# mfathulkr/MA-CJD-Cooperative-Jamming-Decision-Making-via-MARL

Measured on AMD Instinct MI355X. Metric: env-steps/sec (all GPUs; batch_envs=4096/GPU, 3j/4r), higher is better.
Workload: dtype f64; 1 GPU; 3 jammers / 4 radars, batch_envs=4096 per GPU, GRU hidden=64; mode=train, hidden=64, train_batch_episodes=32, updates_per_graph=20, hip_graphs=True, gemm_tuning=True, replay_capacity_episodes=8192, mixer_dtype=fp32, mixer=one MFMA launch per direction (f32)

## Files before the change

include/macjd.h:

```cpp
#ifndef MACJD_H
#define MACJD_H

#include <stddef.h>
#include <stdint.h>

#ifdef __cplusplus
extern "C" {
#endif

#define MACJD_ABI_VERSION 8
#define MACJD_PE_ROWS(R, J) (6 * (R) + 3 * (J) + (J) * (R))
#define MACJD_PE_SCAN_ROWS(R, J) (10 * (R) + (J) * (R))

#define MACJD_OK          0
#define MACJD_EINVAL     -1
#define MACJD_ENOMEM     -2
#define MACJD_EDEVICE    -3
#define MACJD_EUNSUPPORTED -4

#define MACJD_MAX_RADARS  32
#define MACJD_MAX_JAMMERS 32
#define MACJD_MAX_PATTERN_LEVELS 6

#define MACJD_JR_WEAK_DENOM 1u

#define MACJD_STEP_ARITH_F64 1u
#define MACJD_STEP_LANE_KERNEL 2u
#define MACJD_STEP_SLOT_KERNEL 4u

typedef struct macjd_scenario_desc {
    int32_t n_radars;
    int32_t n_jammers;
    int32_t episode_limit;
    int32_t reserved;
    double rp_min, rp_max;
    double pd_A, pd_c1, pd_denB;
    const double* radar_GaPs;
    const double* radar_Pn;
    const double* radar_D;
    const double* radar_pd_no;
    const double* radar_snr_no;
    const double* radar_rd_pen;
    const double* radar_gr;
    const double* jam_pmin;
    const double* jam_pmax;
    const double* jam_gj;
    const double* jr_denom;
    const uint8_t* jr_flags;
} macjd_scenario_desc;

typedef struct macjd_scenario macjd_scenario;

typedef struct macjd_step_io {
    int64_t n_envs;
    int64_t env_offset;
    uint64_t seed;
    uint32_t flags;
    uint32_t reserved;

    const int32_t* T;    int64_t T_se, T_sx;
    const float*   P32;
    const double*  P64;  int64_t P_se, P_sx;

    const double* u;     int64_t u_se, u_sx;
    const int32_t* episode;

    uint8_t* track;      int64_t k_se, k_sx;
    int32_t* step;

    float*   reward;
    float*   r_dpj;
    uint8_t* terminated;
    float*   pd;         int64_t pd_se, pd_sx;
    float*   snr_with;   int64_t sw_se, sw_sx;
    double*  out64;
    double*  pd64;
    double*  snr64;
    double*  prj64;
    const double*  pe_tables;
    const uint8_t* pe_flags;
    int64_t        pe_stride;
    int32_t        pe_tile;
    int32_t        reserved_pe;
    float*   r_dpj_sum;
} macjd_step_io;

typedef struct macjd_scan_desc {
    int32_t n_radars, n_jammers;
    const double* half_beam;
    const double* sweep;
    const double* sweep_mod;
    const uint8_t* full;
    const double* az0;
    const double* bear_tgt;
    const double* bear_jam;
    const double* GaPs_side;
    const double* snr_no;
    const double* snr_no_side;
    const double* pd_no_side;
    const double* gr_side;
} macjd_scan_desc;

typedef struct macjd_scan_pattern_desc {
    int32_t n_radars;
    int32_t n_levels;
    const double* inv_width;
    const double* GaPs_lvl;
    const double* snr_no_lvl;
    const double* pd_no_lvl;
    const double* gr_lvl;
} macjd_scan_pattern_desc;

typedef struct macjd_scan_io {
    double* theta_a;  int64_t a_se, a_sx;
    float*  state;    int64_t st_se;
    int32_t st_col0, st_col_step;
    float*  snr_no;   int64_t sn_se, sn_sx;
} macjd_scan_io;

typedef struct macjd_scan_pe_io {
    const double* tables;
    int64_t stride;
} macjd_scan_pe_io;

int         macjd_abi_version(void);
const char* macjd_last_error(void);
void        macjd_reload_options(void);
int         macjd_device_count(void);

int  macjd_scenario_create(const macjd_scenario_desc* host_desc, macjd_scenario** out);
void macjd_scenario_destroy(macjd_scenario* s);
int  macjd_scenario_dims(const macjd_scenario* s, int32_t* n_radars, int32_t* n_jammers,
                         int32_t* episode_limit);
int  macjd_scenario_is_regular(const macjd_scenario* s);

int macjd_env_reset(const macjd_scenario* s, int64_t n_envs, uint8_t* track, int64_t k_se,
                    int64_t k_sx, int32_t* step, const uint8_t* mask, int32_t* episode,
                    void* hip_stream);

int macjd_env_step(const macjd_scenario* s, const macjd_step_io* io, void* hip_stream);

int macjd_scenario_set_scan(macjd_scenario* s, const macjd_scan_desc* d);
int macjd_scenario_set_scan_pattern(macjd_scenario* s, const macjd_scan_pattern_desc* d);
int macjd_env_step_scan(const macjd_scenario* s, const macjd_step_io* io, const macjd_scan_io* scan, void* hip_stream);
int macjd_env_reset_scan(const macjd_scenario* s, int64_t n_envs, const macjd_scan_io* scan, const uint8_t* mask,
                         void* hip_stream);

int macjd_env_step_scan_pe(const macjd_scenario* s, const macjd_step_io* io, const macjd_scan_io* scan,
                           const macjd_scan_pe_io* scan_pe, void* hip_stream);
int macjd_env_reset_scan_pe(const macjd_scenario* s, int64_t n_envs, const macjd_scan_io* scan, const macjd_scan_pe_io* scan_pe,
                            int32_t pe_tile, const uint8_t* mask, void* hip_stream);

int macjd_env_step_many(const macjd_scenario* s, const macjd_step_io* io, int32_t n_steps, int64_t t_stride,
                        void* hip_stream);

int macjd_env_step_timed(const macjd_scenario* s, const macjd_step_io* io, int iters,
                         void* hip_stream, float* ms_per_launch);

int macjd_env_step_many_timed(const macjd_scenario* s, const macjd_step_io* io, int32_t n_steps, int64_t t_stride,
                              int iters, void* hip_stream, float* ms_per_launch);

#ifdef __cplusplus
}
// ... 3 lines not shown
```

include/macjd_nets.h:

```cpp
#ifndef MACJD_NETS_H
#define MACJD_NETS_H

#include <stdint.h>

#include "macjd.h"

#ifdef __cplusplus
extern "C" {
#endif

typedef struct macjd_qhead_io {
    int64_t n_rows;
    int32_t H, A, n_agents, greedy_only;
    const float* base;  int64_t base_ld;
    const float* P_all; int64_t p_ld;
    const float* W1;    int64_t w1_ld;
    const float* w2;
    const float* b2;
    float* Q;           int64_t q_ld;
    const void* avail;  int32_t avail_elem_size, reserved;
    int64_t av_se, av_sj, av_sa;
    float epsilon;      float reserved2;
    uint64_t seed, counter;
    const float* eps_dev;
    const uint64_t* counter_dev;
    int32_t* T_out32;
    int64_t* T_out64;
    int64_t t32_se, t32_sj, t64_se, t64_sj;
    float* P_out;       int64_t po_se, po_sj;
    int64_t* argmax_out;
    const int64_t* gather_idx;
    float* q_gather_out;
} macjd_qhead_io;

int macjd_qhead_select(const macjd_qhead_io* io, void* hip_stream);

typedef struct macjd_gru_io {
    int32_t n_nets, B, T, J, H, reserved;
    const float* gi[2];
    const float* w_hh[2];
    const float* b_hh[2];
    const float* h0[2];
    float* h_out[2];
    int64_t h0_sb[2];
    const float* obs;      int64_t obs_sb, obs_sj;   int32_t S, reserved2;
    const int64_t* obs_index;
    const float* fc1_w[2]; const float* fc1_b[2];
    const float* w_ih[2];  const float* b_ih[2];
    float* p_out[2];
    const float* act_w[2][3]; const float* act_b[2][3];
    int32_t Ah, A;
} macjd_gru_io;

int macjd_gru_sequence(const macjd_gru_io* io, void* hip_stream);

typedef struct macjd_mixer_io {
    int64_t M;
    int32_t J, Em;
    const float* q;
    const float* w1_raw;
    const float* b1_raw;
    const float* wf_raw;
    const float* v_raw;
    float* y;
    const float* gy;
    float* gq;
    float* gw1_raw;
    float* gb1_raw;
    float* gwf_raw;
    float* gv_raw;
    int64_t b1_ld;
} macjd_mixer_io;

int macjd_mixer_tail_forward(const macjd_mixer_io* io, void* hip_stream);
int macjd_mixer_tail_backward(const macjd_mixer_io* io, void* hip_stream);

typedef struct macjd_tdloss_io {
    int32_t B, Tm1;
    float gamma, reserved;
    const float* y;
    const float* tq;
    int64_t y_sb, tq_sb;
    int64_t gy_sb, gy_cols;
    const float* reward;       int64_t r_sb, r_st;
    const uint8_t* terminated; int64_t t_sb, t_st;
    const uint8_t* filled;     int64_t f_sb, f_st;
    float* stats;
    float* gy;
} macjd_tdloss_io;

int macjd_td_loss(const macjd_tdloss_io* io, void* hip_stream);
int macjd_td_mask_sum(const macjd_tdloss_io* io, float* out, void* hip_stream);

typedef struct macjd_adam_io {
    int64_t n;
    float lr, beta1, beta2, eps, max_norm, reserved;
    float* param; float* grad ; float* exp_avg; float* exp_avg_sq;
    float* step; float* grad_norm; float* partials;
} macjd_adam_io;

int macjd_clip_adam_step(const macjd_adam_io* io, void* hip_stream);

typedef struct macjd_sampler_io {
    int64_t* idx_out;
    int32_t n, reserved;
    const int32_t* n_stored;
    int64_t* counter;
    uint64_t seed;
} macjd_sampler_io;

int macjd_sample_episodes(const macjd_sampler_io* io, void* hip_stream);
int macjd_clip_adam_step_sample(const macjd_adam_io* io, const macjd_sampler_io* next, void* hip_stream);

typedef struct macjd_wgrad_io {
    int64_t K;
    int32_t M, N;
    const float* gout; int64_t gout_ld;
    const float* inp;  int64_t inp_ld;
    float* dW;         int64_t dw_ld;
    float* db;
    float* workspace;
    const float* outer_vec;
    const float* outer_w;
} macjd_wgrad_io;

int64_t macjd_linear_wgrad_workspace_floats(int64_t K, int32_t M, int32_t N);
int macjd_linear_wgrad(const macjd_wgrad_io* io, void* hip_stream);
#define MACJD_WGRAD_MAX_BATCH 8
int macjd_linear_wgrad_many(const macjd_wgrad_io* ios, int32_t n, void* hip_stream);

typedef struct macjd_gather_io {
    int32_t n_tensors, n_rows;
    const int64_t* idx;
    const void* src[8]; void* dst[8]; int64_t row_bytes[8];
    int64_t dst_row_bytes[8];
} macjd_gather_io;

int macjd_gather_rows(const macjd_gather_io* io, void* hip_stream);

typedef struct macjd_prefetch_io {
    macjd_gru_io gru;
    macjd_gather_io gather;
    macjd_sampler_io sampler;
    macjd_tdloss_io mask;
    float* tot_m;
    int32_t no_draw, gather_blocks;
} macjd_prefetch_io;

int macjd_prefetch_batch_supported(int32_t n_nets, int32_t H, int32_t B);
int macjd_prefetch_batch(const macjd_prefetch_io* io, void* hip_stream);

typedef struct macjd_qinput_io {
    int64_t n_rows;
    int32_t H, A;
    const float* h;   int64_t h_ld;
    const void* idx;  int32_t idx_elem_size, reserved;
    const float* P;
    float* out;       int64_t out_ld;
} macjd_qinput_io;

int macjd_qhead_input(const macjd_qinput_io* io, void* hip_stream);

typedef struct macjd_qtaken_io {
    int64_t n_rows;
    int32_t H, A;
    const float* h;   int64_t h_ld;
    const void* idx;  int32_t idx_elem_size, reserved;
    const float* P;
    const float* W1;  int64_t w1_ld;
    const float* b1;  const float* w2;  const float* b2;
    float* x;         int64_t x_ld;
    float* act;       int64_t act_ld;
    float* q;
} macjd_qtaken_io;

int macjd_qhead_taken_supported(int32_t H, int32_t A);
int macjd_qhead_taken(const macjd_qtaken_io* io, void* hip_stream);

typedef struct macjd_layernorm_io {
    int64_t M;
    int32_t S, reserved;
    float eps, reserved2;
    const float* x;  int64_t x_ld;
    const float* gamma;
    const float* beta;
    float* y;        int64_t y_ld;
    float* mean;
    float* rstd;
    float* xhat;     int64_t xhat_ld;
} macjd_layernorm_io;

int macjd_layernorm_forward(const macjd_layernorm_io* io, void* hip_stream);

typedef struct macjd_lnparam_io {
    int32_t C, K;
    const float* W;   int64_t w_ld;
    const float* G;   int64_t g_ld;
    const float* gb;
    float* dgamma;
    float* dbeta;
} macjd_lnparam_io;

int macjd_layernorm_param_grad(const macjd_lnparam_io* io, void* hip_stream);
int macjd_clip_adam_step_ln(const macjd_adam_io* io, const macjd_sampler_io* next, const macjd_lnparam_io* ln,
                            int64_t gamma_off, int64_t beta_off, void* hip_stream);

#define MACJD_ACT_NONE 0
#define MACJD_ACT_RELU 1
#define MACJD_ACT_SIGMOID 2
typedef struct macjd_mlp_io {
    int64_t n_rows;
    int32_t n_layers;
    int32_t dims[4];
    int32_t act[3];
    const float* W[3];
    const float* b[3];
    const float* x;  int64_t x_ld;
    float* y;        int64_t y_ld;
} macjd_mlp_io;

int macjd_mlp_forward(const macjd_mlp_io* io, void* hip_stream);
int macjd_mlp_forward_pair(const macjd_mlp_io* io0, const macjd_mlp_io* io1, void* hip_stream);

typedef struct macjd_splitrelu_bwd_io {
    int64_t M;
    int32_t n_blocks, Cp;
    int32_t width[4];
    const float* g[4];  int64_t g_ld[4];
    const float* g_pass; int64_t gp_ld;
    const float* act;   int64_t act_ld;
    float* gout;        int64_t gout_ld;
    const float* outer_w[4];
} macjd_splitrelu_bwd_io;

int macjd_splitrelu_backward(const macjd_splitrelu_bwd_io* io, void* hip_stream);

typedef struct macjd_rowdot_io {
    int64_t n_rows;
    int32_t K, reserved;
    const float* x;  int64_t x_ld;
    const float* w;
    const float* b;
    float* y;
} macjd_rowdot_io;

int macjd_rowdot(const macjd_rowdot_io* io, void* hip_stream);

typedef struct macjd_grugates_io {
    int64_t n_rows;
    int32_t H, reserved;
    const float* gi;  int64_t gi_ld;
    const float* gh;  int64_t gh_ld;
    const float* h;   int64_t h_ld;
    float* h_out;     int64_t ho_ld;
    float* h_out2;    int64_t ho2_ld;
} macjd_grugates_io;

int macjd_gru_gates(const macjd_grugates_io* io, void* hip_stream);

typedef struct macjd_mixerf_io {
    int64_t M;
    int32_t J, S, Hh, Em;
    int32_t save;
    int32_t operand_dtype;
    float ln_eps;  float reserved_f;
    const float* s;   int64_t s_ld;
    const float* q;
    const float* ln_w; const float* ln_b;
    const float* W1; const float* b1;
    const float* W2; const float* b2;
    const float* Wf2; const float* bf2;
    const float* wV2; const float* bV2;
    float* y;
    float* sn; float* xhat;
    float* act;
    const float* gy;
    float* gq;
    float* gout1;
    float* g_w1raw;
    float* g_wfraw;
    float* g_v;
} macjd_mixerf_io;
// ... 139 lines not shown
```

ma-cjd-cooperative-jamming-decision-making-via-marl_amd/_native.py:

```python
from __future__ import annotations

import ctypes
import os
from typing import Optional

_PKG_DIR = os.path.dirname(os.path.abspath(__file__))
LIB_NAME = "libmacjd_hip.so"
LIB_PATH = os.environ.get("MACJD_LIB") or os.path.join(_PKG_DIR, LIB_NAME)

ABI_VERSION = 8
STEP_ARITH_F64 = 1
STEP_LANE_KERNEL = 2
STEP_SLOT_KERNEL = 4

EXPORTS = [
    "macjd_abi_version", "macjd_last_error", "macjd_reload_options", "macjd_device_count",
    "macjd_scenario_create", "macjd_scenario_destroy", "macjd_scenario_dims", "macjd_scenario_is_regular",
    "macjd_env_reset", "macjd_env_step", "macjd_env_step_timed",
    "macjd_qhead_select", "macjd_gru_sequence", "macjd_mixer_tail_forward", "macjd_mixer_tail_backward",
    "macjd_mlp_forward", "macjd_mlp_forward_pair", "macjd_td_loss", "macjd_clip_adam_step", "macjd_clip_adam_step_sample", "macjd_clip_adam_step_ln", "macjd_sample_episodes", "macjd_gather_rows",
    "macjd_linear_wgrad", "macjd_linear_wgrad_workspace_floats", "macjd_linear_wgrad_many", "macjd_qhead_input", "macjd_layernorm_forward", "macjd_layernorm_param_grad", "macjd_gru_gates", "macjd_rowdot", "macjd_splitrelu_backward",
    "macjd_mixer_fused_supported", "macjd_mixer_fused_forward", "macjd_mixer_fused_backward", "macjd_mixer_fused_backward_td", "macjd_td_mask_sum",
    "macjd_agent_episode_supported", "macjd_agent_episode", "macjd_env_step_many", "macjd_env_step_many_timed",
    "macjd_qhead_double_q_supported", "macjd_qhead_double_q", "macjd_qhead_taken_supported", "macjd_qhead_taken",
    "macjd_qheads_pair", "macjd_mixer_fused_forward_pair", "macjd_mixer_fused_train", "macjd_mixer_fused_train_static",
    "macjd_scenario_set_scan", "macjd_env_step_scan", "macjd_env_reset_scan",
    "macjd_env_step_scan_pe", "macjd_env_reset_scan_pe",
    "macjd_agent_env_episode_scan_supported", "macjd_agent_env_episode_scan",
    "macjd_scenario_set_scan_pattern",
    "macjd_gru_sequence_backward_supported", "macjd_gru_sequence_backward",
    "macjd_prefetch_batch_supported", "macjd_prefetch_batch",
    "macjd_actor_gradient_supported", "macjd_actor_gradient",
]


class NativeLibraryError(RuntimeError):
    pass


class StepIO(ctypes.Structure):
    _fields_ = [
        ("n_envs", ctypes.c_int64), ("env_offset", ctypes.c_int64), ("seed", ctypes.c_uint64),
        ("flags", ctypes.c_uint32), ("reserved", ctypes.c_uint32),
        ("T", ctypes.c_void_p), ("T_se", ctypes.c_int64), ("T_sx", ctypes.c_int64),
        ("P32", ctypes.c_void_p), ("P64", ctypes.c_void_p), ("P_se", ctypes.c_int64), ("P_sx", ctypes.c_int64),
        ("u", ctypes.c_void_p), ("u_se", ctypes.c_int64), ("u_sx", ctypes.c_int64),
        ("episode", ctypes.c_void_p),
        ("track", ctypes.c_void_p), ("k_se", ctypes.c_int64), ("k_sx", ctypes.c_int64),
        ("step", ctypes.c_void_p),
        ("reward", ctypes.c_void_p), ("r_dpj", ctypes.c_void_p), ("terminated", ctypes.c_void_p),
        ("pd", ctypes.c_void_p), ("pd_se", ctypes.c_int64), ("pd_sx", ctypes.c_int64),
        ("snr_with", ctypes.c_void_p), ("sw_se", ctypes.c_int64), ("sw_sx", ctypes.c_int64),
        ("out64", ctypes.c_void_p), ("pd64", ctypes.c_void_p), ("snr64", ctypes.c_void_p),
        ("prj64", ctypes.c_void_p),
        ("pe_tables", ctypes.c_void_p), ("pe_flags", ctypes.c_void_p), ("pe_stride", ctypes.c_int64),
        ("pe_tile", ctypes.c_int32), ("reserved_pe", ctypes.c_int32),
        ("r_dpj_sum", ctypes.c_void_p),
    ]


class ScanDesc(ctypes.Structure):
    _fields_ = [
        ("n_radars", ctypes.c_int32), ("n_jammers", ctypes.c_int32),
        ("half_beam", ctypes.c_void_p), ("sweep", ctypes.c_void_p), ("sweep_mod", ctypes.c_void_p),
        ("full", ctypes.c_void_p), ("az0", ctypes.c_void_p), ("bear_tgt", ctypes.c_void_p), ("bear_jam", ctypes.c_void_p),
        ("GaPs_side", ctypes.c_void_p), ("snr_no", ctypes.c_void_p), ("snr_no_side", ctypes.c_void_p),
        ("pd_no_side", ctypes.c_void_p), ("gr_side", ctypes.c_void_p),
    ]


class ScanPatternDesc(ctypes.Structure):
    _fields_ = [
        ("n_radars", ctypes.c_int32), ("n_levels", ctypes.c_int32),
        ("inv_width", ctypes.c_void_p), ("GaPs_lvl", ctypes.c_void_p), ("snr_no_lvl", ctypes.c_void_p),
        ("pd_no_lvl", ctypes.c_void_p), ("gr_lvl", ctypes.c_void_p),
    ]


class ScanIO(ctypes.Structure):
    _fields_ = [
        ("theta_a", ctypes.c_void_p), ("a_se", ctypes.c_int64), ("a_sx", ctypes.c_int64),
        ("state", ctypes.c_void_p), ("st_se", ctypes.c_int64), ("st_col0", ctypes.c_int32), ("st_col_step", ctypes.c_int32),
        ("snr_no", ctypes.c_void_p), ("sn_se", ctypes.c_int64), ("sn_sx", ctypes.c_int64),
    ]


class ScanPeIO(ctypes.Structure):
    _fields_ = [("tables", ctypes.c_void_p), ("stride", ctypes.c_int64)]


class QheadIO(ctypes.Structure):
    _fields_ = [
        ("n_rows", ctypes.c_int64),
        ("H", ctypes.c_int32), ("A", ctypes.c_int32), ("n_agents", ctypes.c_int32), ("greedy_only", ctypes.c_int32),
        ("base", ctypes.c_void_p), ("base_ld", ctypes.c_int64),
        ("P_all", ctypes.c_void_p), ("p_ld", ctypes.c_int64),
        ("W1", ctypes.c_void_p), ("w1_ld", ctypes.c_int64),
        ("w2", ctypes.c_void_p), ("b2", ctypes.c_void_p),
        ("Q", ctypes.c_void_p), ("q_ld", ctypes.c_int64),
        ("avail", ctypes.c_void_p), ("avail_elem_size", ctypes.c_int32), ("reserved", ctypes.c_int32),
        ("av_se", ctypes.c_int64), ("av_sj", ctypes.c_int64), ("av_sa", ctypes.c_int64),
        ("epsilon", ctypes.c_float), ("reserved2", ctypes.c_float),
        ("seed", ctypes.c_uint64), ("counter", ctypes.c_uint64),
        ("eps_dev", ctypes.c_void_p), ("counter_dev", ctypes.c_void_p),
        ("T_out32", ctypes.c_void_p), ("T_out64", ctypes.c_void_p),
        ("t32_se", ctypes.c_int64), ("t32_sj", ctypes.c_int64), ("t64_se", ctypes.c_int64), ("t64_sj", ctypes.c_int64),
        ("P_out", ctypes.c_void_p), ("po_se", ctypes.c_int64), ("po_sj", ctypes.c_int64),
        ("argmax_out", ctypes.c_void_p), ("gather_idx", ctypes.c_void_p), ("q_gather_out", ctypes.c_void_p),
    ]


class GruIO(ctypes.Structure):
    _fields_ = [
        ("n_nets", ctypes.c_int32), ("B", ctypes.c_int32), ("T", ctypes.c_int32), ("J", ctypes.c_int32),
        ("H", ctypes.c_int32), ("reserved", ctypes.c_int32),
        ("gi", ctypes.c_void_p * 2), ("w_hh", ctypes.c_void_p * 2), ("b_hh", ctypes.c_void_p * 2),
        ("h0", ctypes.c_void_p * 2), ("h_out", ctypes.c_void_p * 2), ("h0_sb", ctypes.c_int64 * 2),
        ("obs", ctypes.c_void_p), ("obs_sb", ctypes.c_int64), ("obs_sj", ctypes.c_int64), ("S", ctypes.c_int32), ("reserved2", ctypes.c_int32),
        ("obs_index", ctypes.c_void_p),
        ("fc1_w", ctypes.c_void_p * 2), ("fc1_b", ctypes.c_void_p * 2), ("w_ih", ctypes.c_void_p * 2), ("b_ih", ctypes.c_void_p * 2),
        ("p_out", ctypes.c_void_p * 2), ("act_w", (ctypes.c_void_p * 3) * 2), ("act_b", (ctypes.c_void_p * 3) * 2),
        ("Ah", ctypes.c_int32), ("A", ctypes.c_int32),
    ]


class GruBwdIO(ctypes.Structure):
    _fields_ = [
        ("B", ctypes.c_int32), ("T", ctypes.c_int32), ("J", ctypes.c_int32), ("H", ctypes.c_int32),
        ("gi", ctypes.c_void_p), ("gh", ctypes.c_void_p), ("h_all", ctypes.c_void_p),
        ("h0", ctypes.c_void_p), ("h0_sb", ctypes.c_int64),
        ("w_hh", ctypes.c_void_p), ("dh_all", ctypes.c_void_p),
        ("dgi", ctypes.c_void_p), ("dgh", ctypes.c_void_p), ("dh0", ctypes.c_void_p),
    ]


class ActorGradIO(ctypes.Structure):
    _fields_ = [
        ("n_rows", ctypes.c_int64),
        ("S", ctypes.c_int32), ("Ha", ctypes.c_int32), ("H", ctypes.c_int32), ("A", ctypes.c_int32),
        ("x", ctypes.c_void_p), ("x_ld", ctypes.c_int64), ("base", ctypes.c_void_p), ("base_ld", ctypes.c_int64),
        ("m", ctypes.c_void_p),
        ("W1a", ctypes.c_void_p), ("b1a", ctypes.c_void_p), ("W2a", ctypes.c_void_p), ("b2a", ctypes.c_void_p),
        ("W3a", ctypes.c_void_p), ("b3a", ctypes.c_void_p),
        ("W1q", ctypes.c_void_p), ("w1_ld", ctypes.c_int64), ("w2q", ctypes.c_void_p), ("b2q", ctypes.c_void_p),
        ("a1", ctypes.c_void_p), ("a2", ctypes.c_void_p), ("g3", ctypes.c_void_p), ("g2", ctypes.c_void_p),
        ("g1", ctypes.c_void_p), ("qsum", ctypes.c_void_p),
    ]


class MixerIO(ctypes.Structure):
    _fields_ = [
        ("M", ctypes.c_int64), ("J", ctypes.c_int32), ("Em", ctypes.c_int32),
        ("q", ctypes.c_void_p), ("w1_raw", ctypes.c_void_p), ("b1_raw", ctypes.c_void_p),
        ("wf_raw", ctypes.c_void_p), ("v_raw", ctypes.c_void_p), ("y", ctypes.c_void_p),
        ("gy", ctypes.c_void_p), ("gq", ctypes.c_void_p), ("gw1_raw", ctypes.c_void_p),
        ("gb1_raw", ctypes.c_void_p), ("gwf_raw", ctypes.c_void_p), ("gv_raw", ctypes.c_void_p),
        ("b1_ld", ctypes.c_int64),
    ]


class MixerFusedIO(ctypes.Structure):
    _fields_ = [
        ("M", ctypes.c_int64), ("J", ctypes.c_int32), ("S", ctypes.c_int32), ("Hh", ctypes.c_int32), ("Em", ctypes.c_int32),
        ("save", ctypes.c_int32), ("operand_dtype", ctypes.c_int32), ("ln_eps", ctypes.c_float), ("reserved_f", ctypes.c_float),
        ("s", ctypes.c_void_p), ("s_ld", ctypes.c_int64), ("q", ctypes.c_void_p),
        ("ln_w", ctypes.c_void_p), ("ln_b", ctypes.c_void_p), ("W1", ctypes.c_void_p), ("b1", ctypes.c_void_p),
        ("W2", ctypes.c_void_p), ("b2", ctypes.c_void_p), ("Wf2", ctypes.c_void_p), ("bf2", ctypes.c_void_p),
        ("wV2", ctypes.c_void_p), ("bV2", ctypes.c_void_p),
        ("y", ctypes.c_void_p), ("sn", ctypes.c_void_p), ("xhat", ctypes.c_void_p), ("act", ctypes.c_void_p),
        ("gy", ctypes.c_void_p), ("gq", ctypes.c_void_p), ("gout1", ctypes.c_void_p), ("g_w1raw", ctypes.c_void_p),
        ("g_wfraw", ctypes.c_void_p), ("g_v", ctypes.c_void_p),
    ]


class MixerStaticIO(ctypes.Structure):
    _fields_ = [
        ("n_tiles", ctypes.c_int64), ("sn", ctypes.c_void_p), ("xhat", ctypes.c_void_p), ("act", ctypes.c_void_p),
        ("gout1_sum", ctypes.c_void_p), ("g_w1raw_sum", ctypes.c_void_p), ("g_wfraw_sum", ctypes.c_void_p),
        ("g_v_sum", ctypes.c_void_p),
    ]


class AgentEpisodeIO(ctypes.Structure):
    _fields_ = [
        ("n_envs", ctypes.c_int64), ("T", ctypes.c_int32), ("J", ctypes.c_int32), ("H", ctypes.c_int32), ("A", ctypes.c_int32),
# ... 18 lines not shown
        ("a1_w", ctypes.c_void_p), ("a1_b", ctypes.c_void_p), ("a2_w", ctypes.c_void_p), ("a2_b", ctypes.c_void_p),
        ("a3_w", ctypes.c_void_p), ("a3_b", ctypes.c_void_p),
        ("W1", ctypes.c_void_p), ("w1_ld", ctypes.c_int64), ("b1", ctypes.c_void_p), ("w2", ctypes.c_void_p), ("b2", ctypes.c_void_p),
        ("avail", ctypes.c_void_p), ("avail_elem_size", ctypes.c_int32), ("reserved", ctypes.c_int32),
        ("av_se", ctypes.c_int64), ("av_sj", ctypes.c_int64), ("av_sa", ctypes.c_int64),
        ("eps", ctypes.c_void_p), ("seed", ctypes.c_uint64), ("counter_base", ctypes.c_void_p),
        ("env_seed", ctypes.c_uint64), ("episode", ctypes.c_void_p),
        ("track", ctypes.c_void_p), ("k_se", ctypes.c_int64), ("k_sx", ctypes.c_int64), ("step", ctypes.c_void_p),
        ("scan", ScanIO), ("pe_tables", ctypes.c_void_p),
        ("hidden", ctypes.c_void_p), ("T_out", ctypes.c_void_p), ("P_out", ctypes.c_void_p), ("h_final", ctypes.c_void_p),
        ("st_state", ctypes.c_void_p), ("st_obs", ctypes.c_void_p), ("reward", ctypes.c_void_p), ("terminated", ctypes.c_void_p),
        ("rdpj_sum", ctypes.c_void_p),
    ]


class DoubleQIO(ctypes.Structure):
    _fields_ = [
        ("n_rows", ctypes.c_int64), ("H", ctypes.c_int32), ("A", ctypes.c_int32),
        ("h_e", ctypes.c_void_p), ("he_ld", ctypes.c_int64), ("h_t", ctypes.c_void_p), ("ht_ld", ctypes.c_int64),
        ("P_e", ctypes.c_void_p), ("pe_ld", ctypes.c_int64), ("P_t", ctypes.c_void_p), ("pt_ld", ctypes.c_int64),
        ("W1_e", ctypes.c_void_p), ("w1e_ld", ctypes.c_int64), ("b1_e", ctypes.c_void_p), ("w2_e", ctypes.c_void_p), ("b2_e", ctypes.c_void_p),
        ("W1_t", ctypes.c_void_p), ("w1t_ld", ctypes.c_int64), ("b1_t", ctypes.c_void_p), ("w2_t", ctypes.c_void_p), ("b2_t", ctypes.c_void_p),
        ("out", ctypes.c_void_p), ("argmax_out", ctypes.c_void_p), ("p_group", ctypes.c_int64), ("p_inner", ctypes.c_int64),
    ]


class QinputIO(ctypes.Structure):
    _fields_ = [
        ("n_rows", ctypes.c_int64), ("H", ctypes.c_int32), ("A", ctypes.c_int32),
        ("h", ctypes.c_void_p), ("h_ld", ctypes.c_int64),
        ("idx", ctypes.c_void_p), ("idx_elem_size", ctypes.c_int32), ("reserved", ctypes.c_int32),
        ("P", ctypes.c_void_p), ("out", ctypes.c_void_p), ("out_ld", ctypes.c_int64),
    ]


class GruGatesIO(ctypes.Structure):
    _fields_ = [
        ("n_rows", ctypes.c_int64), ("H", ctypes.c_int32), ("reserved", ctypes.c_int32),
        ("gi", ctypes.c_void_p), ("gi_ld", ctypes.c_int64), ("gh", ctypes.c_void_p), ("gh_ld", ctypes.c_int64),
        ("h", ctypes.c_void_p), ("h_ld", ctypes.c_int64),
        ("h_out", ctypes.c_void_p), ("ho_ld", ctypes.c_int64), ("h_out2", ctypes.c_void_p), ("ho2_ld", ctypes.c_int64),
    ]


class RowdotIO(ctypes.Structure):
    _fields_ = [
        ("n_rows", ctypes.c_int64), ("K", ctypes.c_int32), ("reserved", ctypes.c_int32),
        ("x", ctypes.c_void_p), ("x_ld", ctypes.c_int64), ("w", ctypes.c_void_p), ("b", ctypes.c_void_p),
        ("y", ctypes.c_void_p),
    ]


class SplitReluBwdIO(ctypes.Structure):
    _fields_ = [
        ("M", ctypes.c_int64), ("n_blocks", ctypes.c_int32), ("Cp", ctypes.c_int32), ("width", ctypes.c_int32 * 4),
        ("g0", ctypes.c_void_p), ("g1", ctypes.c_void_p), ("g2", ctypes.c_void_p), ("g3", ctypes.c_void_p),
        ("g_ld", ctypes.c_int64 * 4),
        ("g_pass", ctypes.c_void_p), ("gp_ld", ctypes.c_int64),
        ("act", ctypes.c_void_p), ("act_ld", ctypes.c_int64), ("gout", ctypes.c_void_p), ("gout_ld", ctypes.c_int64),
        ("ow0", ctypes.c_void_p), ("ow1", ctypes.c_void_p), ("ow2", ctypes.c_void_p), ("ow3", ctypes.c_void_p),
    ]


class LayerNormIO(ctypes.Structure):
    _fields_ = [
        ("M", ctypes.c_int64), ("S", ctypes.c_int32), ("reserved", ctypes.c_int32),
        ("eps", ctypes.c_float), ("reserved2", ctypes.c_float),
        ("x", ctypes.c_void_p), ("x_ld", ctypes.c_int64), ("gamma", ctypes.c_void_p), ("beta", ctypes.c_void_p),
        ("y", ctypes.c_void_p), ("y_ld", ctypes.c_int64), ("mean", ctypes.c_void_p), ("rstd", ctypes.c_void_p),
        ("xhat", ctypes.c_void_p), ("xhat_ld", ctypes.c_int64),
    ]


class LnParamIO(ctypes.Structure):
    _fields_ = [
        ("C", ctypes.c_int32), ("K", ctypes.c_int32),
        ("W", ctypes.c_void_p), ("w_ld", ctypes.c_int64), ("G", ctypes.c_void_p), ("g_ld", ctypes.c_int64),
        ("gb", ctypes.c_void_p), ("dgamma", ctypes.c_void_p), ("dbeta", ctypes.c_void_p),
    ]


class MlpIO(ctypes.Structure):
    _fields_ = [
        ("n_rows", ctypes.c_int64), ("n_layers", ctypes.c_int32), ("dims", ctypes.c_int32 * 4),
        ("act", ctypes.c_int32 * 3), ("W", ctypes.c_void_p * 3), ("b", ctypes.c_void_p * 3),
        ("x", ctypes.c_void_p), ("x_ld", ctypes.c_int64), ("y", ctypes.c_void_p), ("y_ld", ctypes.c_int64),
    ]


class TdLossIO(ctypes.Structure):
    _fields_ = [
        ("B", ctypes.c_int32), ("Tm1", ctypes.c_int32), ("gamma", ctypes.c_float), ("reserved", ctypes.c_float),
        ("y", ctypes.c_void_p), ("tq", ctypes.c_void_p),
        ("y_sb", ctypes.c_int64), ("tq_sb", ctypes.c_int64), ("gy_sb", ctypes.c_int64), ("gy_cols", ctypes.c_int64),
        ("reward", ctypes.c_void_p), ("r_sb", ctypes.c_int64), ("r_st", ctypes.c_int64),
        ("terminated", ctypes.c_void_p), ("t_sb", ctypes.c_int64), ("t_st", ctypes.c_int64),
        ("filled", ctypes.c_void_p), ("f_sb", ctypes.c_int64), ("f_st", ctypes.c_int64),
        ("stats", ctypes.c_void_p), ("gy", ctypes.c_void_p),
    ]


class AdamIO(ctypes.Structure):
    _fields_ = [
        ("n", ctypes.c_int64), ("lr", ctypes.c_float), ("beta1", ctypes.c_float), ("beta2", ctypes.c_float),
        ("eps", ctypes.c_float), ("max_norm", ctypes.c_float), ("reserved", ctypes.c_float),
        ("param", ctypes.c_void_p), ("grad", ctypes.c_void_p), ("exp_avg", ctypes.c_void_p),
        ("exp_avg_sq", ctypes.c_void_p), ("step", ctypes.c_void_p), ("grad_norm", ctypes.c_void_p),
        ("partials", ctypes.c_void_p),
    ]


class QtakenIO(ctypes.Structure):
    _fields_ = [
        ("n_rows", ctypes.c_int64), ("H", ctypes.c_int32), ("A", ctypes.c_int32),
        ("h", ctypes.c_void_p), ("h_ld", ctypes.c_int64),
        ("idx", ctypes.c_void_p), ("idx_elem_size", ctypes.c_int32), ("reserved", ctypes.c_int32),
        ("P", ctypes.c_void_p),
        ("W1", ctypes.c_void_p), ("w1_ld", ctypes.c_int64),
        ("b1", ctypes.c_void_p), ("w2", ctypes.c_void_p), ("b2", ctypes.c_void_p),
        ("x", ctypes.c_void_p), ("x_ld", ctypes.c_int64),
        ("act", ctypes.c_void_p), ("act_ld", ctypes.c_int64),
        ("q", ctypes.c_void_p),
    ]


class SamplerIO(ctypes.Structure):
    _fields_ = [
        ("idx_out", ctypes.c_void_p), ("n", ctypes.c_int32), ("reserved", ctypes.c_int32),
        ("n_stored", ctypes.c_void_p), ("counter", ctypes.c_void_p), ("seed", ctypes.c_uint64),
    ]


class GatherIO(ctypes.Structure):
    _fields_ = [
        ("n_tensors", ctypes.c_int32), ("n_rows", ctypes.c_int32), ("idx", ctypes.c_void_p),
        ("src", ctypes.c_void_p * 8), ("dst", ctypes.c_void_p * 8), ("row_bytes", ctypes.c_int64 * 8),
        ("dst_row_bytes", ctypes.c_int64 * 8),
    ]


class PrefetchIO(ctypes.Structure):
    _fields_ = [
        ("gru", GruIO), ("gather", GatherIO), ("sampler", SamplerIO), ("mask", TdLossIO),
        ("tot_m", ctypes.c_void_p), ("no_draw", ctypes.c_int32), ("gather_blocks", ctypes.c_int32),
    ]


class WgradIO(ctypes.Structure):
    _fields_ = [
        ("K", ctypes.c_int64), ("M", ctypes.c_int32), ("N", ctypes.c_int32),
        ("gout", ctypes.c_void_p), ("gout_ld", ctypes.c_int64), ("inp", ctypes.c_void_p), ("inp_ld", ctypes.c_int64),
        ("dW", ctypes.c_void_p), ("dw_ld", ctypes.c_int64), ("db", ctypes.c_void_p), ("workspace", ctypes.c_void_p),
        ("outer_vec", ctypes.c_void_p), ("outer_w", ctypes.c_void_p),
    ]


_lib: Optional[ctypes.CDLL] = None


def load() -> ctypes.CDLL:
    global _lib
    if _lib is not None:
        return _lib
    if not os.path.exists(LIB_PATH):
        raise NativeLibraryError(
            f"{LIB_PATH} not found. Build it with `python -c 'import __graft_entry__ as g; g.build()'` "
            f"(hipcc --offload-arch=gfx950). There is no CPU fallback for the environment step.")
    try:
        lib = ctypes.CDLL(LIB_PATH)
    except OSError as e:
        raise NativeLibraryError(f"cannot load {LIB_PATH}: {e}") from e
    lib.macjd_abi_version.restype = ctypes.c_int
    lib.macjd_last_error.restype = ctypes.c_char_p
    lib.macjd_device_count.restype = ctypes.c_int
    lib.macjd_reload_options.restype = None
    lib.macjd_scenario_create.restype = ctypes.c_int
    lib.macjd_scenario_create.argtypes = [ctypes.c_void_p, ctypes.POINTER(ctypes.c_void_p)]
    lib.macjd_scenario_destroy.restype = None
    lib.macjd_scenario_destroy.argtypes = [ctypes.c_void_p]
    lib.macjd_scenario_is_regular.restype = ctypes.c_int
    lib.macjd_scenario_is_regular.argtypes = [ctypes.c_void_p]
    lib.macjd_scenario_dims.restype = ctypes.c_int
    lib.macjd_scenario_dims.argtypes = [ctypes.c_void_p] + [ctypes.POINTER(ctypes.c_int32)] * 3
    lib.macjd_env_reset.restype = ctypes.c_int
    lib.macjd_env_reset.argtypes = [ctypes.c_void_p, ctypes.c_int64, ctypes.c_void_p, ctypes.c_int64, ctypes.c_int64,
                                    ctypes.c_void_p, ctypes.c_void_p, ctypes.c_void_p, ctypes.c_void_p]
    lib.macjd_env_step.restype = ctypes.c_int
    lib.macjd_scenario_set_scan.restype = ctypes.c_int
    lib.macjd_scenario_set_scan.argtypes = [ctypes.c_void_p, ctypes.POINTER(ScanDesc)]
    lib.macjd_scenario_set_scan_pattern.restype = ctypes.c_int
    lib.macjd_scenario_set_scan_pattern.argtypes = [ctypes.c_void_p, ctypes.POINTER(ScanPatternDesc)]
    lib.macjd_env_step_scan.restype = ctypes.c_int
    lib.macjd_env_step_scan.argtypes = [ctypes.c_void_p, ctypes.POINTER(StepIO), ctypes.POINTER(ScanIO), ctypes.c_void_p]
    lib.macjd_env_reset_scan.restype = ctypes.c_int
    lib.macjd_env_reset_scan.argtypes = [ctypes.c_void_p, ctypes.c_int64, ctypes.POINTER(ScanIO), ctypes.c_void_p, ctypes.c_void_p]
    lib.macjd_env_step_scan_pe.restype = ctypes.c_int
    lib.macjd_env_step_scan_pe.argtypes = [ctypes.c_void_p, ctypes.POINTER(StepIO), ctypes.POINTER(ScanIO),
                                           ctypes.POINTER(ScanPeIO), ctypes.c_void_p]
    lib.macjd_env_reset_scan_pe.restype = ctypes.c_int
    lib.macjd_env_reset_scan_pe.argtypes = [ctypes.c_void_p, ctypes.c_int64, ctypes.POINTER(ScanIO), ctypes.POINTER(ScanPeIO),
                                            ctypes.c_int32, ctypes.c_void_p, ctypes.c_void_p]
    lib.macjd_env_step.argtypes = [ctypes.c_void_p, ctypes.POINTER(StepIO), ctypes.c_void_p]
    lib.macjd_env_step_timed.restype = ctypes.c_int
    lib.macjd_env_step_timed.argtypes = [ctypes.c_void_p, ctypes.POINTER(StepIO), ctypes.c_int, ctypes.c_void_p,
                                         ctypes.POINTER(ctypes.c_float)]
    lib.macjd_qhead_select.restype = ctypes.c_int
    lib.macjd_qhead_select.argtypes = [ctypes.POINTER(QheadIO), ctypes.c_void_p]
    lib.macjd_gru_sequence.restype = ctypes.c_int
    lib.macjd_gru_sequence.argtypes = [ctypes.POINTER(GruIO), ctypes.c_void_p]
    lib.macjd_gru_sequence_backward_supported.restype = ctypes.c_int
    lib.macjd_gru_sequence_backward_supported.argtypes = [ctypes.c_int32]
    lib.macjd_gru_sequence_backward.restype = ctypes.c_int
    lib.macjd_gru_sequence_backward.argtypes = [ctypes.POINTER(GruBwdIO), ctypes.c_void_p]
    lib.macjd_actor_gradient_supported.restype = ctypes.c_int
    lib.macjd_actor_gradient_supported.argtypes = [ctypes.c_int32] * 4
    lib.macjd_actor_gradient.restype = ctypes.c_int
    lib.macjd_actor_gradient.argtypes = [ctypes.POINTER(ActorGradIO), ctypes.c_void_p]
    for name in ("macjd_mixer_tail_forward", "macjd_mixer_tail_backward"):
        getattr(lib, name).restype = ctypes.c_int
        getattr(lib, name).argtypes = [ctypes.POINTER(MixerIO), ctypes.c_void_p]
    lib.macjd_qhead_double_q_supported.restype = ctypes.c_int
    lib.macjd_qhead_double_q_supported.argtypes = [ctypes.c_int32] * 2
    lib.macjd_qhead_double_q.restype = ctypes.c_int
    lib.macjd_qhead_double_q.argtypes = [ctypes.POINTER(DoubleQIO), ctypes.c_void_p]
    lib.macjd_agent_episode_supported.restype = ctypes.c_int
    lib.macjd_agent_episode_supported.argtypes = [ctypes.c_int32] * 3
    lib.macjd_agent_episode.restype = ctypes.c_int
    lib.macjd_agent_episode.argtypes = [ctypes.POINTER(AgentEpisodeIO), ctypes.c_void_p]
    lib.macjd_agent_env_episode_scan_supported.restype = ctypes.c_int
    lib.macjd_agent_env_episode_scan_supported.argtypes = [ctypes.c_int32] * 4
    lib.macjd_agent_env_episode_scan.restype = ctypes.c_int
    lib.macjd_agent_env_episode_scan.argtypes = [ctypes.c_void_p, ctypes.POINTER(AgentEnvEpisodeScanIO), ctypes.c_void_p]
    lib.macjd_env_step_many.restype = ctypes.c_int
    lib.macjd_env_step_many.argtypes = [ctypes.c_void_p, ctypes.POINTER(StepIO), ctypes.c_int32, ctypes.c_int64, ctypes.c_void_p]
    lib.macjd_env_step_many_timed.restype = ctypes.c_int
    lib.macjd_env_step_many_timed.argtypes = [ctypes.c_void_p, ctypes.POINTER(StepIO), ctypes.c_int32, ctypes.c_int64, ctypes.c_int,
                                              ctypes.c_void_p, ctypes.POINTER(ctypes.c_float)]
    lib.macjd_mixer_fused_supported.restype = ctypes.c_int
    lib.macjd_mixer_fused_supported.argtypes = [ctypes.c_int32] * 4
    for name in ("macjd_mixer_fused_forward", "macjd_mixer_fused_backward"):
        getattr(lib, name).restype = ctypes.c_int
        getattr(lib, name).argtypes = [ctypes.POINTER(MixerFusedIO), ctypes.c_void_p]
    lib.macjd_mixer_fused_backward_td.restype = ctypes.c_int
    lib.macjd_mixer_fused_backward_td.argtypes = [ctypes.POINTER(MixerFusedIO), ctypes.POINTER(TdLossIO), ctypes.c_void_p, ctypes.c_void_p]
    lib.macjd_mixer_fused_train.restype = ctypes.c_int
    lib.macjd_mixer_fused_train.argtypes = [ctypes.POINTER(MixerFusedIO), ctypes.POINTER(MixerFusedIO), ctypes.POINTER(TdLossIO),
                                            ctypes.c_void_p, ctypes.c_void_p]
    lib.macjd_mixer_fused_train_static.restype = ctypes.c_int
    lib.macjd_mixer_fused_train_static.argtypes = [ctypes.POINTER(MixerFusedIO), ctypes.POINTER(MixerFusedIO), ctypes.POINTER(TdLossIO),
                                                   ctypes.c_void_p, ctypes.POINTER(MixerStaticIO), ctypes.c_void_p]
    lib.macjd_td_mask_sum.restype = ctypes.c_int
    lib.macjd_td_mask_sum.argtypes = [ctypes.POINTER(TdLossIO), ctypes.c_void_p, ctypes.c_void_p]
    lib.macjd_qhead_taken_supported.restype = ctypes.c_int
    lib.macjd_qhead_taken_supported.argtypes = [ctypes.c_int32, ctypes.c_int32]
    lib.macjd_qhead_taken.restype = ctypes.c_int
    lib.macjd_qhead_taken.argtypes = [ctypes.POINTER(QtakenIO), ctypes.c_void_p]
    lib.macjd_qheads_pair.restype = ctypes.c_int
    lib.macjd_qheads_pair.argtypes = [ctypes.POINTER(QtakenIO), ctypes.POINTER(DoubleQIO), ctypes.c_void_p]
    lib.macjd_mixer_fused_forward_pair.restype = ctypes.c_int
    lib.macjd_mixer_fused_forward_pair.argtypes = [ctypes.POINTER(MixerFusedIO), ctypes.POINTER(MixerFusedIO), ctypes.c_void_p]
    lib.macjd_qhead_input.restype = ctypes.c_int
    lib.macjd_qhead_input.argtypes = [ctypes.POINTER(QinputIO), ctypes.c_void_p]
    lib.macjd_layernorm_forward.restype = ctypes.c_int
    lib.macjd_layernorm_forward.argtypes = [ctypes.POINTER(LayerNormIO), ctypes.c_void_p]
    lib.macjd_gru_gates.restype = ctypes.c_int
    lib.macjd_gru_gates.argtypes = [ctypes.POINTER(GruGatesIO), ctypes.c_void_p]
    lib.macjd_splitrelu_backward.restype = ctypes.c_int
    lib.macjd_splitrelu_backward.argtypes = [ctypes.POINTER(SplitReluBwdIO), ctypes.c_void_p]
    lib.macjd_layernorm_param_grad.restype = ctypes.c_int
    lib.macjd_layernorm_param_grad.argtypes = [ctypes.POINTER(LnParamIO), ctypes.c_void_p]
    lib.macjd_rowdot.restype = ctypes.c_int
    lib.macjd_rowdot.argtypes = [ctypes.POINTER(RowdotIO), ctypes.c_void_p]
    lib.macjd_mlp_forward_pair.restype = ctypes.c_int
    lib.macjd_mlp_forward_pair.argtypes = [ctypes.POINTER(MlpIO), ctypes.POINTER(MlpIO), ctypes.c_void_p]
    lib.macjd_mlp_forward.restype = ctypes.c_int
    lib.macjd_mlp_forward.argtypes = [ctypes.POINTER(MlpIO), ctypes.c_void_p]
    lib.macjd_td_loss.restype = ctypes.c_int
    lib.macjd_td_loss.argtypes = [ctypes.POINTER(TdLossIO), ctypes.c_void_p]
    lib.macjd_clip_adam_step.restype = ctypes.c_int
    lib.macjd_clip_adam_step.argtypes = [ctypes.POINTER(AdamIO), ctypes.c_void_p]
    lib.macjd_clip_adam_step_sample.restype = ctypes.c_int
    lib.macjd_clip_adam_step_sample.argtypes = [ctypes.POINTER(AdamIO), ctypes.POINTER(SamplerIO), ctypes.c_void_p]
    lib.macjd_clip_adam_step_ln.restype = ctypes.c_int
    lib.macjd_clip_adam_step_ln.argtypes = [ctypes.POINTER(AdamIO), ctypes.POINTER(SamplerIO), ctypes.POINTER(LnParamIO),
                                            ctypes.c_int64, ctypes.c_int64, ctypes.c_void_p]
    lib.macjd_sample_episodes.restype = ctypes.c_int
    lib.macjd_sample_episodes.argtypes = [ctypes.POINTER(SamplerIO), ctypes.c_void_p]
    lib.macjd_prefetch_batch_supported.restype = ctypes.c_int
    lib.macjd_prefetch_batch_supported.argtypes = [ctypes.c_int32] * 3
    lib.macjd_prefetch_batch.restype = ctypes.c_int
    lib.macjd_prefetch_batch.argtypes = [ctypes.POINTER(PrefetchIO), ctypes.c_void_p]
    lib.macjd_gather_rows.restype = ctypes.c_int
    lib.macjd_gather_rows.argtypes = [ctypes.POINTER(GatherIO), ctypes.c_void_p]
    lib.macjd_linear_wgrad.restype = ctypes.c_int
    lib.macjd_linear_wgrad.argtypes = [ctypes.POINTER(WgradIO), ctypes.c_void_p]
    lib.macjd_linear_wgrad_many.restype = ctypes.c_int
    lib.macjd_linear_wgrad_many.argtypes = [ctypes.POINTER(WgradIO), ctypes.c_int32, ctypes.c_void_p]
    lib.macjd_linear_wgrad_workspace_floats.restype = ctypes.c_int64
    lib.macjd_linear_wgrad_workspace_floats.argtypes = [ctypes.c_int64, ctypes.c_int32, ctypes.c_int32]
    if lib.macjd_abi_version() != ABI_VERSION:
        raise NativeLibraryError(f"{LIB_NAME}: ABI version {lib.macjd_abi_version()} != expected {ABI_VERSION}")
    _lib = lib
    return lib


def reload_options() -> None:
    load().macjd_reload_options()


def check(rc: int, what: str) -> None:
    if rc != 0:
        msg = load().macjd_last_error()
        raise NativeLibraryError(f"{what} failed ({rc}): {msg.decode() if msg else ''}")


class ScenarioHandle:

    def __init__(self, scenario):
        lib = load()
        desc, keep = scenario.c_desc()
        h = ctypes.c_void_p()
        check(lib.macjd_scenario_create(ctypes.addressof(desc), ctypes.byref(h)), "macjd_scenario_create")
        del keep
        self._h = h
        self._lib = lib
        if getattr(scenario, "scanning", False):
            sdesc, skeep = scenario.c_scan_desc()
            check(lib.macjd_scenario_set_scan(h, ctypes.byref(sdesc)), "macjd_scenario_set_scan")
            del skeep
            if getattr(scenario, "scan_pattern_levels", 0):
                pdesc, pkeep = scenario.c_scan_pattern_desc()
                check(lib.macjd_scenario_set_scan_pattern(h, ctypes.byref(pdesc)), "macjd_scenario_set_scan_pattern")
                del pkeep

    @property
    def ptr(self):
        return self._h

    def close(self):
        if getattr(self, "_h", None):
            self._lib.macjd_scenario_destroy(self._h)
            self._h = None

    def __del__(self):
        try:
            self.close()
        except Exception:
            pass
```

ma-cjd-cooperative-jamming-decision-making-via-marl_amd/core/qmix.py:

```python
from __future__ import annotations

import copy
import os

import numpy as np
import torch
import torch.nn.functional as F
import torch.optim as optim

from .. import hipgraph, ops, options
from .networks import QMixer


def _to(x, dtype, device):
    if isinstance(x, torch.Tensor):
        return x.to(device=device, dtype=dtype)
    return torch.as_tensor(np.asarray(x), device=device).to(dtype)


class QMixLearner:
    def __init__(self, mac, args):
        self.args = args
        self.mac = mac
        self.n_agents = args.n_agents
        self.n_actions = args.n_actions
        self.state_shape = args.state_shape
        self.obs_shape = args.obs_shape
        self.device = torch.device(args.device if torch.cuda.is_available() and args.use_cuda else "cpu")
        self.train_agent_body = bool(getattr(args, "train_agent_body", False))
        self.train_actor = bool(getattr(args, "train_actor", False))
        self.actor_loss_coef = float(getattr(args, "actor_loss_coef", 1.0))
        self._last_actor_q = None

        self.eval_qmix_net = QMixer(args)
        self.target_mac = copy.deepcopy(mac)
        self.target_qmix_net = QMixer(args)
        self.target_qmix_net.load_state_dict(self.eval_qmix_net.state_dict())
        if args.use_cuda:
            self.cuda()
        print(f"QMix Learner Initialized on device: {self.device}")

        self.agent_params = list(self.mac.parameters())
        self.qmix_params = list(self.eval_qmix_net.parameters())
        self.params = self.agent_params + self.qmix_params
        self.optimizer = optim.Adam(params=self.params, lr=args.lr, capturable=(self.device.type == "cuda"))
        self.last_target_update_step = 0
        self.train_step = 0
        self._flat_grad = None
        self._sample_rng = np.random.default_rng(int(getattr(args, "seed", 0) or 0))
        self.grad_pack_launches = 0
        self._flat_param = None
        if self.device.type == "cuda":
            self._flatten_trainable()
        self._body_versions = None
        self._mark_body_shared()

    @staticmethod
    def _body_params(agent):
        return list(agent.fc1.parameters()) + list(agent.rnn.parameters()) + list(agent.actor.parameters())

    def _mark_body_shared(self):
        pe, pt = self._body_params(self.mac.agent), self._body_params(self.target_mac.agent)
        self._body_versions = [(p, p._version, q, q._version) for p, q in zip(pe, pt)]

    def _verify_body_shared(self):
        pe, pt = self._body_params(self.mac.agent), self._body_params(self.target_mac.agent)
        same = len(pe) == len(pt) and all(p.shape == q.shape and torch.equal(p.detach(), q.detach()) for p, q in zip(pe, pt))
        if same:
            self._mark_body_shared()
        else:
            self._body_versions = None
        return same and self._body_is_shared()

    def _body_is_shared(self):
        if self.train_agent_body or self.train_actor:
            return False
        if not options.on("SHARED_BODY") or not self._body_versions:
            return False
        pe = self._body_params(self.mac.agent)
        if len(pe) != len(self._body_versions):
            return False
        return all(p is p0 and p._version == vp and q._version == vq
                   for p, (p0, vp, q, vq) in zip(pe, self._body_versions))

    def _trainable(self):
        first = self.eval_qmix_net.first_layer_params()
        ids = {id(p) for p in first}
        rest = [p for p in list(self.mac.agent.fc2_q_head.parameters()) + self.qmix_params if id(p) not in ids]
        body = list(self.mac.agent.fc1.parameters()) + list(self.mac.agent.rnn.parameters()) if self.train_agent_body else []
        actor = list(self.mac.agent.actor.parameters()) if self.train_actor else []
        return first + rest + body + actor

    @staticmethod
    def _world_size():
        import torch.distributed as dist
        return dist.get_world_size() if (dist.is_available() and dist.is_initialized()) else 1

    def _flatten_trainable(self):
        tr = self._trainable()
        self._flat_offsets, off = [], 0
        for p in tr:
            self._flat_offsets.append(off)
            off += (p.numel() + 3) // 4 * 4
        flat = torch.zeros(off, dtype=tr[0].dtype, device=tr[0].device)
        for p, o in zip(tr, self._flat_offsets):
            flat[o:o + p.numel()].copy_(p.detach().reshape(-1))
        self._flat_param = flat
        self._flat_exp_avg = torch.zeros_like(flat)
        self._flat_exp_avg_sq = torch.zeros_like(flat)
        self._adam_step = torch.zeros((), dtype=torch.float32, device=flat.device)
        self._grad_norm = torch.zeros((), dtype=torch.float32, device=flat.device)
        self._adam_partials = torch.zeros(256 + 1024, dtype=torch.float32, device=flat.device)
        for p, off in zip(tr, self._flat_offsets):
            n = p.numel()
            p.data = flat[off:off + n].view_as(p)
            self.optimizer.state[p] = {"step": self._adam_step, "exp_avg": self._flat_exp_avg[off:off + n].view_as(p),
                                       "exp_avg_sq": self._flat_exp_avg_sq[off:off + n].view_as(p)}
        self._flat_grad = torch.zeros_like(flat)
        self._grad_dst = {}
        for p, off in zip(tr, self._flat_offsets):
            n = p.numel()
            self._grad_dst[ops.grad_key(p)] = self._flat_grad[off:off + n].view_as(p)
        mx = self.eval_qmix_net
        first = mx.first_layer_params()
        rows, S = sum(p.shape[0] for p in first[:4]), first[0].shape[1]
        assert self._flat_offsets[8] == rows * S + rows, "merged first layer must be contiguous in the flat vector"
        mx._merged_views = (flat[:rows * S].view(rows, S), flat[rows * S:rows * S + rows])
        self._grad_dst[ops.grad_key(mx._merged_views[0])] = self._flat_grad[:rows * S].view(rows, S)
        self._grad_dst[ops.grad_key(mx._merged_views[1])] = self._flat_grad[rows * S:rows * S + rows]
        self.target_qmix_net.enable_first_layer_cache()

    def load_optimizer_state(self, state_dict):
        self.optimizer.load_state_dict(state_dict)
        if self._flat_param is None:
            return
        for p, off in zip(self._trainable(), self._flat_offsets):
            n = p.numel()
            st = self.optimizer.state.get(p, {})
            if "exp_avg" in st:
                self._flat_exp_avg[off:off + n].copy_(st["exp_avg"].reshape(-1))
                self._flat_exp_avg_sq[off:off + n].copy_(st["exp_avg_sq"].reshape(-1))
                self._adam_step.copy_(torch.as_tensor(st["step"], dtype=torch.float32).reshape(()))
            self.optimizer.state[p] = {"step": self._adam_step, "exp_avg": self._flat_exp_avg[off:off + n].view_as(p),
                                       "exp_avg_sq": self._flat_exp_avg_sq[off:off + n].view_as(p)}

    def grad_vector(self):
        if self._flat_grad is not None:
            return self._flat_grad
        return torch.cat([p.grad.reshape(-1) for p in self._trainable()])

    def _flatten_grads(self):
        tr = self._trainable()
        if self._flat_grad is None:
            self._flat_grad = torch.empty(sum(p.numel() for p in tr), dtype=tr[0].dtype, device=tr[0].device)
        for p in tr:
            if p.grad is None:
                p.grad = torch.zeros_like(p)
        offs = getattr(self, "_flat_offsets", None)
        padded = offs is not None
        if not padded:
            offs, off = [], 0
            for p in tr:
                offs.append(off)
                off += p.numel()
        base, esz = self._flat_grad.data_ptr(), self._flat_grad.element_size()
        in_place = sum(int(p.grad.data_ptr() == base + off * esz and p.grad.is_contiguous()) for p, off in zip(tr, offs))
        if in_place == len(tr):
            return
        self.grad_pack_launches += 1
        if padded:
            packed = [p.grad.reshape(-1).clone() for p in tr]
            for g_, off in zip(packed, offs):
                self._flat_grad[off:off + g_.numel()].copy_(g_)
        elif in_place == 0:
            torch.cat([p.grad.reshape(-1) for p in tr], out=self._flat_grad)
        else:
            self._flat_grad.copy_(torch.cat([p.grad.reshape(-1) for p in tr]))
        for p, off in zip(tr, offs):
            p.grad = self._flat_grad[off:off + p.numel()].view_as(p)

    def _ar_capturable(self):
        import torch.distributed as dist
        return dist.is_available() and dist.is_initialized() and dist.get_backend() == "nccl"

    def _allreduce_grads(self, force=False):
        import torch.distributed as dist
        if self._world_size() <= 1 and not (force and self._ar_capturable()):
            return
        if dist.get_backend() == "nccl":
            dist.all_reduce(self._flat_grad, op=dist.ReduceOp.AVG)
        else:
            dist.all_reduce(self._flat_grad, op=dist.ReduceOp.SUM)
            self._flat_grad.div_(dist.get_world_size())

    def _forward_backward(self, batch, T, validate_actions=True):
        dev = self.device
        states = _to(batch["state"], torch.float32, dev)[:, :T]
        obs = _to(batch["obs"], torch.float32, dev)[:, :T]
        actions_discrete = _to(batch["actions_discrete"], torch.long, dev)[:, :T]
        actions_continuous = _to(batch["actions_continuous"], torch.float32, dev)[:, :T]
        rewards = _to(batch["reward"], torch.float32, dev)[:, :T]
        terminated = _to(batch["terminated"], torch.bool, dev)[:, :T]
        filled = _to(batch["filled"], torch.bool, dev)[:, :T]
        hidden_states = _to(batch["hidden_state"], torch.float32, dev)[:, :T + 1]
        B = states.shape[0]

        rollout_hidden = self.mac.hidden_states
        h_eval = self._unroll_eval_body(obs) if self.train_agent_body else None
        with torch.no_grad():
            if h_eval is not None:
                target_q_all = self._all_action_q_multi([self.target_mac], obs)[0]
                eval_q_all = self._all_action_q_from_hidden(self.mac, h_eval.detach(), obs)
            else:
                target_q_all, eval_q_all = self._all_action_q_multi([self.target_mac, self.mac], obs)
            self.mac.hidden_states = rollout_hidden
            next_actions = eval_q_all[:, 1:].argmax(dim=3, keepdim=True)
            target_q_taken = torch.gather(target_q_all[:, 1:], 3, next_actions).squeeze(3)
            target_q_mixer = self.target_qmix_net(target_q_taken, states[:, 1:])

        if T <= 1:
            q_taken = torch.empty((B, 0, self.n_agents), device=dev)
        else:
            n_eff = B * (T - 1) * self.n_agents
            h_taken = hidden_states if h_eval is None else h_eval
            q_taken = self.mac.agent.get_q_value_for_action(
                h_taken[:, :T - 1].reshape(n_eff, self.args.rnn_hidden_dim),
                actions_discrete[:, :T - 1].reshape(n_eff, 1),
                actions_continuous[:, :T - 1].reshape(n_eff, 1), validate=validate_actions).view(B, T - 1, self.n_agents)
        eval_q_mixer = self.eval_qmix_net(q_taken, states[:, :-1])

        loss, eval_mean, target_mean = ops.td_loss(eval_q_mixer, target_q_mixer, rewards[:, :-1], terminated[:, :-1],
                                                   filled[:, :-1], self.args.gamma)

        for p in self.params:
            p.grad = None
        if self.train_actor:
            with ops.deferred_wgrad(grad_dst=getattr(self, "_grad_dst", None)):
                loss.backward()
                self._last_actor_q = self._actor_backward(obs, hidden_states if h_eval is None else h_eval.detach(), filled, T)
        else:
            loss.backward()
        if self._world_size() > 1 or self._flat_param is not None:
            self._flatten_grads()
        return loss.detach(), eval_mean.detach(), target_mean.detach()

    def _actor_backward(self, obs, h_taken, filled, T):
        a = self.mac.agent
        params = list(a.actor.parameters())
        B, J, H, A = obs.shape[0], self.n_agents, self.args.rnn_hidden_dim, self.n_actions
        if T <= 1:
            for p in params:
                p.grad = torch.zeros_like(p)
            return torch.zeros((), dtype=torch.float32, device=obs.device)
        n = B * (T - 1) * J
        with torch.no_grad():
            f = filled[:, :T - 1].reshape(B, T - 1).to(torch.float32)
            tot = f.sum()
            w = torch.where(tot > 0, f / (J * tot), torch.zeros_like(f))
            w = w.unsqueeze(2).expand(B, T - 1, J).reshape(n)
            x = obs[:, :T - 1].reshape(n, -1)
            l1, l2 = a.fc2_q_head[0], a.fc2_q_head[2]
            base = F.linear(h_taken[:, :T - 1].reshape(n, H), l1.weight[:, :H], l1.bias)
            a1, a2, g3, g2, g1, qsum = ops.actor_gradient(x, base, self.actor_loss_coef * w, a.actor_layers(), l1.weight,
                                                           l2.weight, l2.bias, H, A)
            for p, g in zip(params, ops.actor_weight_grads(x, a1, a2, g3, g2, g1, params=params)):
                p.grad = g
            return (w * qsum).sum()

    def _unroll_eval_body(self, obs):
        B, T, J, S = obs.shape
        a = self.mac.agent
        H = a.rnn_hidden_dim
# ... 106 lines not shown
            mixer_static = (mixer_train and obs_static and bool(getattr(self, "_g_state_static", False))
                            and options.on("MIXER_STATIC_STATE"))
            self._g_mixer_static = mixer_static
            train_gy = None
            try:
                with torch.no_grad():
                    bases = scan_chain()
                    p_eval = pre_actor[1]
                    params = [p_eval if shared else pre_actor[0], p_eval]
                    for t_ in list(bases) + [p for p in params if p is not None]:
                        t_.record_stream(origin)
                    tq_agents = double_q(bases, params, paired=True)
                q_taken = self.mac.agent.get_q_value_for_action(
                    st["hidden_state"].view(n, H), st["actions_discrete"].view(n, 1), st["actions_continuous"].view(n, 1),
                    validate=False).view(B, T1, J)
                if after_join is not None:
                    fork_at.record(origin)
                with torch.no_grad():
                    if mixer_train:
                        target_q_tot, train_gy = self.target_qmix_net.forward_paired_with_next_fused(
                            tq_agents, st["state"], td=dict(reward=st["reward"], terminated=st["terminated"], filled=st["filled"],
                                                            gamma=self.args.gamma, Tm1=T - 1, tot_m=tot_m,
                                                            static_rows=mixer_static))
                    else:
                        target_q_tot = self.target_qmix_net.forward_paired_with_next_fused(tq_agents, st["state"])
                eval_q_tot = self.eval_qmix_net(q_taken, st["state"])
                ops.assert_pairs_launched()
            finally:
                ops.clear_pending_pairs()
            return self._finish_update(st, T, eval_q_tot, target_q_tot, tot_m=tot_m, side_work=side_work, sums_in_backward=True,
                                       train_gy=train_gy)
        elif target_beside_head:
            origin = torch.cuda.current_stream(dev)
            ts = self._target_stream
            ts.wait_stream(origin)
            with torch.cuda.stream(ts), torch.no_grad():
                bases = scan_chain()
                p_eval = pre_actor[1]
                params = [p_eval if shared else pre_actor[0], p_eval]
                target_q_tot = self.target_qmix_net(double_q(bases, params), st["state"])
                target_done = torch.cuda.Event()
                target_done.record(ts)
            if after_join is not None:
                after_join(False)
            origin.wait_event(prefetched[0])
            eval_q_tot = eval_forward()
            origin.wait_event(target_done)
            target_q_tot.record_stream(origin)
            return self._finish_update(st, T, eval_q_tot, target_q_tot, tot_m=prefetched[2] if len(prefetched) > 2 else None)
        elif two_streams:
            origin = torch.cuda.current_stream(dev)
            if getattr(self, "_target_stream", None) is None:
                self._target_stream = torch.cuda.Stream(device=dev)
            ts = self._target_stream
            if prefetched is None:
                ts.wait_stream(origin)
                with torch.cuda.stream(ts), torch.no_grad():
                    bases = scan_chain()
                    p_target = None if (shared or pre_actor is not None) else actor_all(macs[0].agent)
            else:
                assert pre_scan is not None and pre_actor is not None
                origin.wait_event(prefetched[0])
                bases, p_target = scan_chain(), None
            if pre_actor is not None:
                p_target, p_eval = (None if shared else pre_actor[0]), pre_actor[1]
            eval_q_tot = eval_forward()
            if pre_actor is None:
                with torch.no_grad():
                    p_eval = actor_all(body)
            with torch.no_grad():
                hyper = None if self.target_qmix_net.fused_available(st["state"]) else self.target_qmix_net.hyper_outputs(st["state"])
                if prefetched is None:
                    origin.wait_stream(ts)
                else:
                    origin.wait_event(prefetched[1])
                if after_join is not None:
                    after_join()
                for t_ in list(bases) + ([p_target] if p_target is not None else []) + ([p_eval] if pre_actor is not None else []):
                    t_.record_stream(origin)
                if pre_actor is not None and not fused_dq:
                    ex = lambda p_: p_.view(B, 1, J, A).expand(B, T1, J, A).reshape(n, A)
                    p_target, p_eval = (None if p_target is None else ex(p_target)), ex(p_eval)
                params = [p_eval if shared else p_target, p_eval]
                target_q_tot = self.target_qmix_net(double_q(bases, params), st["state"], hyper=hyper)
        else:
            with torch.no_grad():
                bases = scan_chain()
                p_eval = actor_all(body)
                params = [p_eval if shared else actor_all(macs[0].agent), p_eval]
                hyper = None if self.target_qmix_net.fused_available(st["state"]) else self.target_qmix_net.hyper_outputs(st["state"])
                target_q_tot = self.target_qmix_net(double_q(bases, params), st["state"], hyper=hyper)
            eval_q_tot = eval_forward()
        return self._finish_update(st, T, eval_q_tot, target_q_tot)

    def _paired_heads_ok(self, st, T):
        B, T1 = st["state"].shape[0], T + 1
        J, H, A = self.n_agents, self.args.rnn_hidden_dim, self.n_actions
        n = B * T1 * J
        head = self.mac.agent.fc2_q_head
        return (st["state"].is_cuda and options.get("UPDATE_STREAMS") != "1" and options.on("PAIRED_HEADS")
                and ops.qhead_double_q_fused_supported(st["obs"].reshape(n, -1), H, A)
                and self.target_qmix_net.fused_available(st["state"]) and self.eval_qmix_net.fused_available(st["state"])
                and ops.qhead_taken_supported(st["hidden_state"].view(n, H), head[0].weight, head[2].weight, A))

    def _finish_update(self, st, T, eval_q_tot, target_q_tot, tot_m=None, side_work=None, sums_in_backward=False,
                       train_gy=None):
        for p in self.params:
            p.grad = None
        if eval_q_tot.is_cuda:
            stats_done = stats_branch = sums_late = None
            if train_gy is not None:
                origin = torch.cuda.current_stream(eval_q_tot.device)
                ts = self._target_stream
                head_done = torch.cuda.Event()
                head_done.record(origin)
                row = self._last_stats4 = torch.empty(4, dtype=torch.float32, device=eval_q_tot.device)
                loss, eval_mean, target_mean = row[0], row[1], row[2]
                gy = train_gy

                def sums_late():
                    ts.wait_event(head_done)
                    with torch.cuda.stream(ts):
                        ops.td_loss_sums_into(row, eval_q_tot, target_q_tot, st["reward"], st["terminated"], st["filled"],
                                              self.args.gamma, T - 1, 1)
                    for t_ in (row, eval_q_tot, target_q_tot):
                        t_.record_stream(ts)
            elif tot_m is not None and ops.fused_mixer_backward_will_run(eval_q_tot):
                origin = torch.cuda.current_stream(eval_q_tot.device)
                ts = self._target_stream
                head_done = torch.cuda.Event()
                if not sums_in_backward:
                    head_done.record(origin)

                def stats_branch():
                    with torch.cuda.stream(ts):
                        ts.wait_event(head_done)
                        out = ops.td_loss_and_grad(eval_q_tot, target_q_tot, st["reward"], st["terminated"], st["filled"],
                                                   self.args.gamma, T - 1, 1)
                        done = torch.cuda.Event()
                        done.record(ts)
                    return out, done

                if not sums_in_backward:
                    (loss, eval_mean, target_mean, _, self._last_stats4), stats_done = stats_branch()
                else:
                    row = self._last_stats4 = torch.empty(4, dtype=torch.float32, device=eval_q_tot.device)
                    loss, eval_mean, target_mean = row[0], row[1], row[2]
                gy = ops.td_grad_in_mixer_backward(eval_q_tot, target_q_tot, st["reward"], st["terminated"], st["filled"],
                                                   self.args.gamma, T - 1, 1, tot_m, stats_row=row if sums_in_backward else None)
            else:
                loss, eval_mean, target_mean, gy, self._last_stats4 = ops.td_loss_and_grad(
                    eval_q_tot, target_q_tot, st["reward"], st["terminated"], st["filled"], self.args.gamma, T - 1, 1)
            hold = self._flat_param is not None and self._world_size() <= 1 and options.on("LN_IN_SQNORM")
            with ops.deferred_wgrad(grad_dst=getattr(self, "_grad_dst", None), hold_lnparam=hold) as dw:
                eval_q_tot.backward(gy)
            assert ops._PENDING_TD is None, "the fused mixer's backward did not take the TD loss's inputs"
            self._held_ln = dw.held
            if side_work is not None:
                side_work()
            if sums_late is not None:
                sums_late()
            if stats_done is not None:
                torch.cuda.current_stream(eval_q_tot.device).wait_event(stats_done)
                for t_ in (self._last_stats4,):
                    t_.record_stream(torch.cuda.current_stream(eval_q_tot.device))
        else:
            loss, eval_mean, target_mean = ops.td_loss_full(eval_q_tot, target_q_tot, st["reward"], st["terminated"],
                                                            st["filled"], self.args.gamma, T - 1, 1)
            loss.backward()
        if self._world_size() > 1 or self._flat_param is not None:
            self._flatten_grads()
        return loss.detach(), eval_mean.detach(), target_mean.detach()

    def _clip_and_step(self, sample_next=None):
        if self._flat_param is not None:
            g = self.optimizer.param_groups[0]
            held, self._held_ln = getattr(self, "_held_ln", None), None
            ops.clip_adam_step(self._flat_param, self._flat_grad, self._flat_exp_avg, self._flat_exp_avg_sq,
                               self._adam_step, self._grad_norm, self._adam_partials, g["lr"], g["betas"], g["eps"],
                               self.args.grad_norm_clip, sample_next=sample_next, lnparam=held)
            return self._grad_norm
        grad_norm = torch.nn.utils.clip_grad_norm_(self.params, self.args.grad_norm_clip)
        self.optimizer.step()
        return grad_norm.detach() if torch.is_tensor(grad_norm) else torch.as_tensor(grad_norm)

    def _after_step(self):
        if (self.train_step - self.last_target_update_step) >= self.args.target_update_interval:
            self._update_targets()
            self.last_target_update_step = self.train_step

    def _pack_stats(self, loss, grad_norm, ev, tg, sync_stats, actor_q=None):
        stats = {"loss": loss, "grad_norm": grad_norm, "eval_qtot_avg": ev, "target_qtot_avg": tg}
        if actor_q is not None:
            stats["actor_q_avg"] = actor_q
        if sync_stats:
            stacked = torch.stack([torch.as_tensor(v, device=self.device, dtype=torch.float32).reshape(())
                                   for v in stats.values()])
            stats = dict(zip(stats.keys(), stacked.tolist()))
        return stats

    def train(self, batch, train_info=None, sync_stats=True):
        self.train_step += 1
        loss, ev, tg = self._forward_backward(batch, int(batch["max_seq_len"]))
        self._allreduce_grads()
        grad_norm = self._clip_and_step()
        if self.train_agent_body or self.train_actor:
            for m in (self.mac, self.target_mac):
                m.invalidate_static_inputs()
        self._after_step()
        if not sync_stats and torch.is_tensor(grad_norm) and grad_norm is self._grad_norm_tensor():
            grad_norm = grad_norm.clone()
        return self._pack_stats(loss, grad_norm, ev, tg, sync_stats, actor_q=self._last_actor_q if self.train_actor else None)

    def _grad_norm_tensor(self):
        return getattr(self, "_grad_norm", None)

    def enable_graphs(self, buffer, batch_size, warmup_iters=3, force_two_graphs=False, updates_per_graph=None,
                      graphed_allreduce=None, prime=True):
        if self.device.type != "cuda":
            raise RuntimeError("enable_graphs needs the learner on a HIP device")
        if self.train_agent_body:
            raise RuntimeError("enable_graphs: train_agent_body is an eager-mode option (the captured, static-observation "
                               "and shared-body updates are built on the frozen agent body); use train()")
        if self.train_actor:
            raise RuntimeError("enable_graphs: train_actor is an eager-mode option (the captured, static-observation and "
                               "shared-body updates are built on the frozen actor); use train()")
        self.release_graphs()
        self._verify_body_shared()
        same_buffer = getattr(self, "_g_buffer", None) is buffer
        self._g_buffer, self._g_B, self._g_T = buffer, int(batch_size), int(buffer.episode_limit)
        self._g_obs_static = bool(getattr(buffer, "obs_static", False)) and options.on("LEARNER_STATIC_OBS")
        self._g_state_static = self._g_obs_static and bool(getattr(buffer, "state_static", False))
        self._g_mixer_static = False
        self._g_actor_in_scan = options.on("ACTOR_IN_SCAN")
        self._g_scan_from_ring = self._g_obs_static and int(buffer.buffers["obs"].shape[-1]) <= 3 * int(self.args.rnn_hidden_dim)
        prev_idx = getattr(self, "_g_idx", None)
        keep_idx = same_buffer and prev_idx is not None and prev_idx.numel() == self._g_B and prev_idx.device == self.device
        self._g_idx = prev_idx if keep_idx else torch.zeros(self._g_B, dtype=torch.int64, device=self.device)
        self._g_dev_sampler = self._flat_param is not None and options.on("DEVICE_SAMPLER")
        if not keep_idx:
            self._g_n_stored = torch.zeros(1, dtype=torch.int32, device=self.device)
        if getattr(self, "_g_draws", None) is None:
            self._g_draws = torch.full((1,), int(getattr(self, "_resume_draws", 0)), dtype=torch.int64, device=self.device)
        if not keep_idx:
            self._g_pop_seen = None
            self._g_idx_fresh = False
        self._g_idx_ring = [(torch.zeros(self._g_B, dtype=torch.int64).pin_memory(), torch.cuda.Event()) for _ in range(8)]
        if buffer.current_size < 1:
            raise RuntimeError("enable_graphs: the replay buffer is empty")

        keys = [k for k in buffer.buffers if k != "avail_actions"]
        srcs = [buffer.buffers[k] for k in keys]
        fused = ops.gather_rows_supported(srcs) and self._g_T >= 2
        if fused:
            T1 = self._g_T + 1
            padded = ("actions_discrete", "actions_continuous")
            stage = {k: torch.zeros((self._g_B, T1 if k in padded else v.shape[1]) + tuple(v.shape[2:]), dtype=v.dtype,
                                    device=v.device) for k, v in zip(keys, srcs)}

        def body_a():
            if fused:
                pre = (None, None)
                if self._g_scan_from_ring and options.get("UPDATE_STREAMS") != "1":
                    pre = self._scan_from_ring_early()
                ops.gather_rows(self._g_idx, srcs, [stage[k] for k in keys])
                return self._forward_backward_full(stage, self._g_T, pre_scan=pre[0], pre_actor=pre[1])
            b = {k: v.index_select(0, self._g_idx) for k, v in zip(keys, srcs)}
            return self._forward_backward(b, self._g_T, validate_actions=False)

        self._graph_body_a = body_a

        was_shared = self._body_is_shared()
        snap_p = [p.detach().clone() for p in self.params]
        snap_o = {id(p): {k: v.clone() for k, v in st.items() if torch.is_tensor(v)}
                  for p, st in self.optimizer.state.items()}
        s = torch.cuda.Stream(device=self.device)
        s.wait_stream(torch.cuda.current_stream(self.device))
        with torch.cuda.stream(s):
            for _ in range(max(1, warmup_iters)):
                body_a()
                self._clip_and_step()
        torch.cuda.current_stream(self.device).wait_stream(s)
        def restore_training_state():
            with torch.no_grad():
                for p, sp in zip(self.params, snap_p):
                    p.copy_(sp)
                for p, st in self.optimizer.state.items():
                    for k, v in st.items():
                        if torch.is_tensor(v):
                            old = snap_o.get(id(p), {}).get(k)
                            v.copy_(old) if old is not None else v.zero_()
            if was_shared:
                self._mark_body_shared()

        restore_training_state()
        self._graph_a, self._graph_b = torch.cuda.CUDAGraph(), torch.cuda.CUDAGraph()
        self._g_graphed_ar = bool(graphed_allreduce if graphed_allreduce is not None
                                  else options.get("GRAPHED_ALLREDUCE") == "1") and self._ar_capturable()
        self._g_single = (self._world_size() <= 1 and not force_two_graphs) or self._g_graphed_ar
        with hipgraph.capture(self._graph_a):
            self._g_out_a = body_a()
            st4 = getattr(self, "_last_stats4", None) if fused else None
            if st4 is not None and st4.numel() == 4:
                self._grad_norm = st4[3]
            self._g_stats4 = st4 if (st4 is not None and st4.numel() == 4) else None
            nxt = (self._g_idx, self._g_n_stored, self._g_draws, self._sampler_seed()) if self._g_dev_sampler else None
            if self._g_single:
                if self._g_graphed_ar:
                    self._allreduce_grads(force=True)
                self._g_out_b = self._clip_and_step(sample_next=nxt)
        if not self._g_single:
            with hipgraph.capture(self._graph_b, pool=self._graph_a.pool()):
                self._g_out_b = self._clip_and_step(sample_next=nxt)
        K = int(updates_per_graph if updates_per_graph is not None else options.get("UPDATES_PER_GRAPH"))
        self._g_multi = None
        self._g_prefetch_launch = False
        if K > 1 and self._g_single and self._g_dev_sampler and fused and self._g_stats4 is not None:
            gm, rows, single_norm = torch.cuda.CUDAGraph(), [], self._grad_norm
            pipelined = (self._g_scan_from_ring and self._g_actor_in_scan and options.get("UPDATE_STREAMS") != "1"
                         and options.on("PIPELINED_GROUP"))
            launch_agents = [self.mac.agent] if self._body_is_shared() else [self.target_mac.agent, self.mac.agent]
            self._g_prefetch_launch = bool(pipelined and options.on("PREFETCH_LAUNCH") and "filled" in keys
                                           and ops.prefetch_batch_supported(launch_agents, self._g_B, srcs))
            stage2 = {k: torch.zeros_like(v) for k, v in stage.items()} if pipelined else None
            stages = [stage, stage2]
            self._g_stages = stages
            origin_dev = self.device

            unwritten = [0]

            def prefetch(dst, fork=True, draw=True):
                origin = torch.cuda.current_stream(origin_dev)
                ts = self._target_stream
                if isinstance(fork, torch.cuda.Event):
                    ts.wait_event(fork)
                elif fork:
                    ts.wait_stream(origin)
                shared = self._body_is_shared()
                agents = [self.mac.agent] if shared else [self.target_mac.agent, self.mac.agent]
                if self._g_prefetch_launch:
                    with torch.cuda.stream(ts), torch.no_grad():
                        h, ps, tot_m = ops.prefetch_batch(
                            buffer.buffers["obs"], agents, self._g_B, self.n_agents, self._g_T + 1,
                            (self._g_idx, self._g_n_stored, self._g_draws, self._sampler_seed()), srcs, [dst[k] for k in keys],
                            buffer.buffers["filled"], self._g_T - 1, offset=unwritten[0], draw=draw)
                        unwritten[0] += 1 if draw else 0
                        ev = torch.cuda.Event()
                        ev.record(ts)
                    return [h[0], h[0]], [ps[0], ps[0]], (ev, ev, tot_m)
                with torch.cuda.stream(ts), torch.no_grad():
                    if draw:
                        ops.sample_episodes(self._g_idx, self._g_n_stored, self._g_draws, self._sampler_seed())
                    ops.gather_rows(self._g_idx, srcs, [dst[k] for k in keys])
                    tot_m = ops.td_mask_sum(dst["filled"], self._g_T - 1)
                    ev_g = torch.cuda.Event()
                    ev_g.record(ts)
                    h, ps = ops.gru_sequence_from_obs(buffer.buffers["obs"], self._g_idx, agents, self._g_B, self.n_agents,
                                                      self._g_T + 1, with_actor=True)
                    ev_s = torch.cuda.Event()
                    ev_s.record(ts)
                return (([h[0], h[0]] if shared else h), ([ps[0], ps[0]] if shared else ps), (ev_g, ev_s, tot_m))

            with hipgraph.capture(gm, pool=self._graph_a.pool()):
                nxt_batch = None
                for k_upd in range(K):
                    last = k_upd == K - 1
                    box = {}
                    hook = (lambda fork=True: box.__setitem__("next", prefetch(stages[(k_upd + 1) % 2], fork))) if (pipelined and not last) else None
                    if pipelined and nxt_batch is not None:
                        h_pre, p_pre, evs = nxt_batch
                        self._forward_backward_full(stages[k_upd % 2], self._g_T, pre_scan=h_pre, pre_actor=p_pre,
                                                    prefetched=evs, after_join=hook)
                    elif pipelined:
                        pre = self._scan_from_ring_early()
                        ops.gather_rows(self._g_idx, srcs, [stage[k] for k in keys])
                        if self._paired_heads_ok(stage, self._g_T):
                            tot_m0 = ops.td_mask_sum(stage["filled"], self._g_T - 1)
                            scan_done = torch.cuda.Event()
                            scan_done.record(self._target_stream)
                            self._forward_backward_full(stage, self._g_T, pre_scan=pre[0], pre_actor=pre[1],
                                                        prefetched=(None, scan_done, tot_m0), after_join=hook)
                        else:
                            self._forward_backward_full(stage, self._g_T, pre_scan=pre[0], pre_actor=pre[1], after_join=hook)
                    else:
                        body_a()
                    nxt_batch = box.get("next")
                    rows.append(self._last_stats4)
                    self._grad_norm = rows[-1][3]
                    if self._g_graphed_ar:
                        self._allreduce_grads(force=True)
                    if nxt_batch is not None:
                        self._clip_and_step(sample_next=None)
                    else:
                        self._clip_and_step(sample_next=nxt + (unwritten[0],))
                        unwritten[0] = 0
                if pipelined:
                    torch.cuda.current_stream(self.device).wait_stream(self._target_stream)
            self._grad_norm = single_norm
            self._g_multi = (K, gm, rows)
            self._g_pipelined = pipelined
        self._g_shared_body = self._body_is_shared()
        assert self._g_obs_static == (bool(getattr(buffer, "obs_static", False)) and options.on("LEARNER_STATIC_OBS"))
        if prime:
            keep = (self._g_draws.clone(), self._g_idx.clone(), self._g_n_stored.clone())
            self._g_n_stored.fill_(int(buffer.current_size))
            self._g_idx.clamp_(0, max(0, int(buffer.current_size) - 1))
            hipgraph.replay(self._graph_a, self.device)
            if not self._g_single:
                self._allreduce_grads()
                hipgraph.replay(self._graph_b, self.device)
            if self._g_multi is not None:
                self._g_idx.clamp_(0, max(0, int(buffer.current_size) - 1))
                hipgraph.replay(self._g_multi[1], self.device)
            torch.cuda.synchronize(self.device)
            restore_training_state()
            self._g_draws.copy_(keep[0]); self._g_idx.copy_(keep[1]); self._g_n_stored.copy_(keep[2])
        self._graphs_ready = True

    def release_graphs(self):
        graphs = []
        m = getattr(self, "_g_multi", None)
        if m is not None:
            graphs.append(m[1])
        graphs += [getattr(self, "_graph_b", None), getattr(self, "_graph_a", None)]
        self._graphs_ready = False
        self._g_multi = self._g_stages = None
        self._graph_a = self._graph_b = None
        self._graph_body_a = None
        self._g_out_a = self._g_out_b = self._g_stats4 = self._last_stats4 = self._held_ln = None
        if self._flat_param is not None and any(g is not None for g in graphs):
            self._grad_norm = torch.zeros((), dtype=torch.float32, device=self._flat_param.device)
        hipgraph.destroy(graphs, self.device)

    def train_from_buffer(self, indices=None, sync_stats=True, stats_row=None):
        buf = self._g_buffer if getattr(self, "_graphs_ready", False) else None
        if buf is None:
            raise RuntimeError("call enable_graphs(buffer, batch_size) first")
        device_draw = False
        if indices is None:
            if buf.current_size < self._g_B:
                return self._snap(self.train(buf.sample(self._g_B), None, sync_stats=sync_stats), stats_row)
            device_draw = self._g_dev_sampler and self._population_full_length(buf)
            if not device_draw:
                indices = self._sample_rng.choice(buf.current_size, self._g_B, replace=False)
        if not device_draw:
            indices = np.asarray(indices, dtype=np.int64)
            if len(indices) != self._g_B or int(buf.episode_lengths[indices].min()) != self._g_T:
                return self._snap(self.train(buf.sample(len(indices), indices=indices), None, sync_stats=sync_stats), stats_row)
        if self._g_obs_static and not buf.obs_static:
            raise RuntimeError("an episode with unknown / changing observations was stored after enable_graphs() captured "
                               "the static-observation update: call enable_graphs() again")
        if self._g_shared_body and not self._body_is_shared():
            raise RuntimeError("the agent body (fc1 / GRU / actor) of one controller changed after enable_graphs() captured "
                               "the shared-body update: call enable_graphs() again")
        self.train_step += 1
        if device_draw:
            self._device_draw_ready(buf)
        else:
            k = self.train_step % len(self._g_idx_ring)
            slot, ev = self._g_idx_ring[k]
            ev.synchronize()
            slot.numpy()[:] = indices
            self._g_idx.copy_(slot, non_blocking=True)
            ev.record()
        hipgraph.replay(self._graph_a, self.device)
        self._g_idx_fresh = self._g_dev_sampler and (buf.store_count, buf.current_size) == self._g_pop_seen
        if not self._g_single:
            self._allreduce_grads()
            hipgraph.replay(self._graph_b, self.device)
        self._after_step()
        loss, ev, tg = self._g_out_a
        if stats_row is not None and not sync_stats and self._g_stats4 is not None:
            stats_row.copy_(self._g_stats4, non_blocking=True)
            return {"loss": stats_row[0], "grad_norm": stats_row[3], "eval_qtot_avg": stats_row[1], "target_qtot_avg": stats_row[2]}
        return self._snap(self._pack_stats(loss, self._g_out_b, ev, tg, sync_stats), stats_row)

    def _device_draw_ready(self, buf):
        pop = (buf.store_count, buf.current_size)
        if pop != self._g_pop_seen:
            self._g_n_stored.fill_(buf.current_size)
            self._g_pop_seen, self._g_idx_fresh = pop, False
        if not self._g_idx_fresh:
            ops.sample_episodes(self._g_idx, self._g_n_stored, self._g_draws, self._sampler_seed())

    def train_from_buffer_many(self, n, stats_out=None):
        buf = self._g_buffer if getattr(self, "_graphs_ready", False) else None
        if buf is None:
            raise RuntimeError("call enable_graphs(buffer, batch_size) first")
        out, done = [], 0
        while done < n:
            m = self._g_multi
            until_sync = self.args.target_update_interval - (self.train_step - self.last_target_update_step)
            if (m is not None and n - done >= m[0] and until_sync >= m[0] and buf.current_size >= self._g_B
                    and self._population_full_length(buf) and (not self._g_obs_static or buf.obs_static)
                    and (not self._g_shared_body or self._body_is_shared())):
                self._device_draw_ready(buf)
                self.train_step += m[0]
                hipgraph.replay(m[1], self.device)
                self._g_idx_fresh = (buf.store_count, buf.current_size) == self._g_pop_seen
                self._after_step()
                if stats_out is not None:
                    torch.stack(m[2], out=stats_out[done:done + m[0]])
                out += m[2]
                done += m[0]
            else:
                row = stats_out[done] if stats_out is not None else torch.empty(4, dtype=torch.float32, device=self.device)
                self.train_from_buffer(sync_stats=False, stats_row=row)
                out.append(row)
                done += 1
        return out if stats_out is None else stats_out

    def _sampler_seed(self):
        return getattr(self, "_sampler_seed_value", int(getattr(self.args, "seed", 0) or 0))

    def _population_full_length(self, buf):
        key = (buf.store_count, buf.current_size)
        if getattr(self, "_g_full_key", None) != key:
            self._g_full_key = key
            self._g_full = bool((buf.episode_lengths[:buf.current_size] == self._g_T).all())
        return self._g_full

    @staticmethod
    def _snap(stats, stats_row):
        if stats_row is None or not torch.is_tensor(stats["loss"]):
            return stats
        order = ("loss", "eval_qtot_avg", "target_qtot_avg", "grad_norm")
        torch.stack([torch.as_tensor(stats[k], device=stats_row.device, dtype=torch.float32).reshape(()) for k in order],
                    out=stats_row)
        return {k: stats_row[i] for i, k in enumerate(order)}

    def _all_action_q_multi(self, macs, obs, keep_final_hidden=True):
        B, T, J, S = obs.shape
        rows = obs.reshape(B * T * J, S)
        shared = len(macs) == 2 and self._body_is_shared() and {id(m) for m in macs} == {id(self.mac), id(self.target_mac)}
        body_macs = [self.mac] if shared else list(macs)
        side = None
        if rows.is_cuda:
            if getattr(self, "_side_stream", None) is None:
                self._side_stream = torch.cuda.Stream(device=rows.device)
            side, main = self._side_stream, torch.cuda.current_stream(rows.device)
            side.wait_stream(main)
            with torch.cuda.stream(side):
                params = [m.agent.actor_forward(rows) for m in body_macs]
        else:
            params = [m.agent.actor_forward(rows) for m in body_macs]
        gis = [m.agent.gru_input_transform(rows).view(B, T, J, 3 * m.agent.rnn_hidden_dim) for m in body_macs]
        h_alls = ops.gru_sequence_multi(gis, [m.agent.rnn.weight_hh for m in body_macs],
                                        [m.agent.rnn.bias_hh for m in body_macs])
        if shared:
            params, h_alls = params * 2, h_alls * 2
        bases = []
        for m, h_all in zip(macs, h_alls):
            a = m.agent
            H = a.rnn_hidden_dim
            if keep_final_hidden:
                m.hidden_states = h_all[:, T - 1].reshape(B * J, H) if T > 0 else None
            l1 = a.fc2_q_head[0]
            bases.append(F.linear(h_all.reshape(B * T * J, H), l1.weight[:, :H], l1.bias))
        if side is not None:
            torch.cuda.current_stream(rows.device).wait_stream(side)
            for p in params:
                p.record_stream(torch.cuda.current_stream(rows.device))
        out = []
        for m, base, params_all in zip(macs, bases, params):
            a = m.agent
            l1, l2 = a.fc2_q_head[0], a.fc2_q_head[2]
            out.append(ops.qhead_all_actions(base, params_all, l1.weight, l2.weight, l2.bias, a.rnn_hidden_dim,
                                             a.n_actions).view(B, T, J, a.n_actions))
        return out

    def _all_action_q(self, mac_controller, obs):
        return self._all_action_q_multi([mac_controller], obs)[0]

    def _get_all_action_q_values_and_params(self, mac_controller, batch, max_seq_len):
        obs = _to(batch["obs"], torch.float32, self.device)[:, :max_seq_len]
        with torch.no_grad():
            q = self._all_action_q(mac_controller, obs)
            B, T, J, S = obs.shape
            params = mac_controller.agent.actor(obs.reshape(-1, S)).view(B, T, J, -1)
        return q, params

    def _update_targets(self):
# ... 25 lines not shown
```

ma-cjd-cooperative-jamming-decision-making-via-marl_amd/csrc/macjd_nets.hip:

```cpp
#include <hip/hip_runtime.h>
#include <math.h>
#include <stdint.h>
#include <stdio.h>
#include <stdlib.h>
#include <string.h>
#include <type_traits>

#include "../../include/macjd.h"
#include "../../include/macjd_nets.h"
#include "macjd_err.h"
#include "macjd_tdloss.h"
#include "macjd_philox.h"
#include "macjd_gru_math.h"

namespace macjd {

static int set_nets_err(int code, const char* msg) { return set_err(code, "%s", msg); }

__device__ __forceinline__ bool avail_at(const macjd_qhead_io& io, int64_t e, int j, int a) {
    if (!io.avail) return true;
    const int64_t off = e * io.av_se + (int64_t)j * io.av_sj + (int64_t)a * io.av_sa;
    return (io.avail_elem_size == 8) ? (((const int64_t*)io.avail)[off] != 0)
                                     : (((const int32_t*)io.avail)[off] != 0);
}
// ... 691 lines not shown
    if (err != hipSuccess) return set_nets_err(MACJD_EDEVICE, hipGetErrorString(err));
    return MACJD_OK;
}

extern "C" int macjd_td_loss(const macjd_tdloss_io* io, void* hip_stream) {
    using namespace macjd;
    if (!io || io->B < 1 || io->Tm1 < 1) return set_nets_err(MACJD_EINVAL, "macjd_td_loss: bad B / Tm1");
    if (!io->y || !io->tq || !io->reward || !io->terminated || !io->filled || !io->stats)
        return set_nets_err(MACJD_EINVAL, "macjd_td_loss: NULL pointer");
    if (io->y_sb < io->Tm1 || io->tq_sb < io->Tm1 || (io->gy && (io->gy_cols < io->Tm1 || io->gy_sb < io->gy_cols)))
        return set_nets_err(MACJD_EINVAL, "macjd_td_loss: bad strides");
    hipLaunchKernelGGL(td_loss_kernel, dim3(1), dim3(1024), 0, (hipStream_t)hip_stream, *io);
    hipError_t err = hipGetLastError();
    if (err != hipSuccess) return set_nets_err(MACJD_EDEVICE, hipGetErrorString(err));
    return MACJD_OK;
}

namespace macjd {

constexpr int ADAM_BLOCKS = 256;

__global__ void __launch_bounds__(256) adam_sqnorm_kernel(const macjd_adam_io io) {
    __shared__ float smem[4];
    float s = 0.0f;
    for (int64_t i = (int64_t)blockIdx.x * blockDim.x + threadIdx.x; i < io.n; i += (int64_t)gridDim.x * blockDim.x) {
        const float g = io.grad[i];
        s = fmaf(g, g, s);
    }
    s = wave_sum(s);
    if ((threadIdx.x & 63) == 0) smem[threadIdx.x >> 6] = s;
    __syncthreads();
    if (threadIdx.x == 0) {
        io.partials[blockIdx.x] = (smem[0] + smem[1]) + (smem[2] + smem[3]);
        if (blockIdx.x == 0) io.step[0] += 1.0f;
    }
}

__global__ void __launch_bounds__(256) adam_sqnorm_ln_kernel(const macjd_adam_io io, const macjd_lnparam_io ln, const int64_t g_off,
                                                             const int64_t b_off, const int nb) {
    __shared__ float smem[8];
    if ((int)blockIdx.x < nb) {
        float s = 0.0f;
        for (int64_t i = (int64_t)blockIdx.x * blockDim.x + threadIdx.x; i < io.n; i += (int64_t)nb * blockDim.x) {
            const bool is_ln = (i >= g_off && i < g_off + ln.K) || (i >= b_off && i < b_off + ln.K);
            const float g = is_ln ? 0.0f : io.grad[i];
            s = fmaf(g, g, s);
        }
        s = wave_sum(s);
        if ((threadIdx.x & 63) == 0) smem[threadIdx.x >> 6] = s;
        __syncthreads();
        if (threadIdx.x == 0) {
            io.partials[blockIdx.x] = (smem[0] + smem[1]) + (smem[2] + smem[3]);
            if (blockIdx.x == 0) io.step[0] += 1.0f;
        }
        return;
    }
    const int k = (int)blockIdx.x - nb;
    float sg = 0.0f, sb = 0.0f;
    for (int c = threadIdx.x; c < ln.C; c += blockDim.x) {
        const float w = ln.W[(int64_t)c * ln.w_ld + k];
        sg = fmaf(w, ln.G[(int64_t)c * ln.g_ld + k], sg);
        sb = fmaf(w, ln.gb[c], sb);
    }
    sg = wave_sum(sg);
    sb = wave_sum(sb);
    if ((threadIdx.x & 63) == 0) { smem[threadIdx.x >> 6] = sg; smem[4 + (threadIdx.x >> 6)] = sb; }
    __syncthreads();
    if (threadIdx.x == 0) {
        const float dg = (smem[0] + smem[1]) + (smem[2] + smem[3]), db = (smem[4] + smem[5]) + (smem[6] + smem[7]);
        ln.dgamma[k] = dg;
        ln.dbeta[k] = db;
        io.partials[nb + k] = fmaf(db, db, dg * dg);
    }
}

__device__ __forceinline__ uint32_t fmix32(uint32_t h) {
    h ^= h >> 16; h *= 0x85ebca6bu; h ^= h >> 13; h *= 0xc2b2ae35u; h ^= h >> 16;
    return h;
}
struct SamplerPerm { uint32_t key[8]; int rb; uint32_t rmask, lmask; };
__device__ __forceinline__ SamplerPerm sampler_perm(const int64_t c, const uint64_t seed, const int64_t N) {
    const Philox4 ka = philox4x32_10((uint32_t)c, (uint32_t)((uint64_t)c >> 32), 0x53414d50u, 0u, (uint32_t)seed, (uint32_t)(seed >> 32));
    const Philox4 kb = philox4x32_10((uint32_t)c, (uint32_t)((uint64_t)c >> 32), 0x53414d50u, 1u, (uint32_t)seed, (uint32_t)(seed >> 32));
    SamplerPerm p;
    p.key[0] = ka.v[0]; p.key[1] = ka.v[1]; p.key[2] = ka.v[2]; p.key[3] = ka.v[3];
    p.key[4] = kb.v[0]; p.key[5] = kb.v[1]; p.key[6] = kb.v[2]; p.key[7] = kb.v[3];
    int k = 2;
    while (((int64_t)1 << k) < N) ++k;
    const int lb = k / 2;
    p.rb = k - k / 2;
    p.rmask = (1u << p.rb) - 1u; p.lmask = (1u << lb) - 1u;
    return p;
}
__device__ __forceinline__ int64_t sampler_index(const SamplerPerm& p, const int64_t N, const int n, const int t) {
    if (N < n) return t % N;
    uint32_t x = (uint32_t)t;
    for (int walk = 0; walk < 64; ++walk) {
        uint32_t L = x >> p.rb, R = x & p.rmask;
#pragma unroll
        for (int r = 0; r < 8; r += 2) {
            L = (L ^ fmix32(R ^ p.key[r])) & p.lmask;
            R = (R ^ fmix32(L ^ p.key[r + 1])) & p.rmask;
        }
        x = (L << p.rb) | R;
        if ((int64_t)x < N) break;
    }
    return ((int64_t)x < N) ? (int64_t)x : (int64_t)(x % (uint32_t)N);
}
__device__ __forceinline__ void sample_episodes_block(const macjd_sampler_io& sp) {
    const int64_t c = *sp.counter + (int64_t)sp.reserved;
    const int64_t N = (int64_t)*sp.n_stored;
    __syncthreads();
    if (threadIdx.x == 0) *sp.counter = c + 1;
    if (N < 1) return;
    const SamplerPerm perm = sampler_perm(c, sp.seed, N);
    for (int t = threadIdx.x; t < sp.n; t += blockDim.x) sp.idx_out[t] = sampler_index(perm, N, sp.n, t);
}

__global__ void __launch_bounds__(256) sample_episodes_kernel(const macjd_sampler_io sp) { sample_episodes_block(sp); }

template <bool SAMPLE>
__global__ void __launch_bounds__(256) adam_update_kernel(const macjd_adam_io io, const int n_partials, const macjd_sampler_io next) {
    __shared__ float s_tot;
    if (threadIdx.x < 64) {
        float s = 0.0f;
        for (int i = threadIdx.x; i < n_partials; i += 64) s += io.partials[i];
        s = wave_sum(s);
        if (threadIdx.x == 0) s_tot = s;
    }
    __syncthreads();
    const float total_norm = sqrtf(s_tot);
    float coef = io.max_norm / (total_norm + 1e-6f);
    coef = coef < 1.0f ? coef : 1.0f;
    const float step = io.step[0];
    const float bc1 = 1.0f - powf(io.beta1, step);
    const float bc2 = 1.0f - powf(io.beta2, step);
    const float step_size = io.lr / bc1;
    const float bc2_sqrt = sqrtf(bc2);
    for (int64_t i = (int64_t)blockIdx.x * blockDim.x + threadIdx.x; i < io.n; i += (int64_t)gridDim.x * blockDim.x) {
        const float g = io.grad[i] * coef;
        io.grad[i] = g;
        float m = io.exp_avg[i], v = io.exp_avg_sq[i];
        m = m + (1.0f - io.beta1) * (g - m);
        v = v * io.beta2 + (1.0f - io.beta2) * g * g;
        io.exp_avg[i] = m;
        io.exp_avg_sq[i] = v;
        const float denom = sqrtf(v) / bc2_sqrt + io.eps;
        io.param[i] -= step_size * (m / denom);
    }
    if (blockIdx.x == 0 && threadIdx.x == 0) io.grad_norm[0] = total_norm;
    if (SAMPLE && blockIdx.x == 0) sample_episodes_block(next);
}

__device__ __forceinline__ void gather_rows_body(const macjd_gather_io& io, const int k, const int row, const int64_t src_row,
                                                 const int part, const int parts) {
    const int64_t words = io.row_bytes[k] >> 2;
    const uint32_t* __restrict__ src = (const uint32_t*)((const char*)io.src[k] + src_row * io.row_bytes[k]);
    const int64_t dpitch = io.dst_row_bytes[k] ? io.dst_row_bytes[k] : io.row_bytes[k];
    uint32_t* __restrict__ dst = (uint32_t*)((char*)io.dst[k] + (int64_t)row * dpitch);
    const bool vec = ((io.row_bytes[k] & 15) == 0) && ((dpitch & 15) == 0) && ((((uintptr_t)io.src[k]) & 15) == 0) &&
                     ((((uintptr_t)io.dst[k]) & 15) == 0);
    if (vec) {
        const int64_t n4 = words >> 2;
        for (int64_t i = (int64_t)part * blockDim.x + threadIdx.x; i < n4; i += (int64_t)parts * blockDim.x)
            ((uint4*)dst)[i] = ((const uint4*)src)[i];
    } else {
        for (int64_t i = (int64_t)part * blockDim.x + threadIdx.x; i < words; i += (int64_t)parts * blockDim.x)
            dst[i] = src[i];
    }
}

__global__ void __launch_bounds__(256) gather_rows_kernel(const macjd_gather_io io) {
    gather_rows_body(io, blockIdx.y, blockIdx.z, io.idx[blockIdx.z], blockIdx.x, gridDim.x);
}

constexpr int PREFETCH_MAX_B = 1024;
constexpr int PREFETCH_ROW_PARTS = 8;

__global__ void __launch_bounds__(256) prefetch_batch_kernel(const macjd_prefetch_io io) {
    __shared__ __attribute__((aligned(16))) float s_h[2][64];
    __shared__ float s_gi[3 * 64];
    __shared__ float s_pro[768];
    __shared__ int64_t s_idx[PREFETCH_MAX_B];
    __shared__ float s_w[16];
    const int B = io.gru.B, BJ = B * io.gru.J, G = io.gather_blocks;
    const int wg = blockIdx.x;
    const int64_t N = (int64_t)*io.sampler.n_stored;
    const bool draw = !io.no_draw && N >= 1;
    SamplerPerm perm = {};
    if (draw) perm = sampler_perm(*io.sampler.counter + (int64_t)io.sampler.reserved, io.sampler.seed, N);
    auto index_of = [&](int t) -> int64_t { return draw ? sampler_index(perm, N, io.sampler.n, t) : io.sampler.idx_out[t]; };
    if (wg < 2 * BJ) {
        const bool actor_only = wg >= BJ;
        const int seq = actor_only ? wg - BJ : wg;
        gru_units_body<true>(io.gru, 0, seq, index_of(seq / io.gru.J), actor_only, false, s_h, s_gi, s_pro);
    } else if (wg < 2 * BJ + G) {
        const int n_parts = PREFETCH_ROW_PARTS * io.gather.n_tensors * B;
        for (int v = wg - 2 * BJ; v < n_parts; v += G) {
            const int part = v % PREFETCH_ROW_PARTS, kr = v / PREFETCH_ROW_PARTS;
            const int k = kr % io.gather.n_tensors, row = kr / io.gather.n_tensors;
            gather_rows_body(io.gather, k, row, index_of(row), part, PREFETCH_ROW_PARTS);
        }
    } else {
        for (int t = threadIdx.x; t < B; t += blockDim.x) {
            const int64_t e = index_of(t);
            s_idx[t] = e;
            if (draw) io.sampler.idx_out[t] = e;
        }
        __syncthreads();
        td_mask_sum_body(io.mask, io.tot_m, s_w, [&](int b) { return s_idx[b]; });
    }
}

}

static int sampler_args_ok(const macjd_sampler_io* sp) {
    return sp && sp->idx_out && sp->n >= 1 && sp->n_stored && sp->counter && sp->reserved >= 0;
}

extern "C" int macjd_sample_episodes(const macjd_sampler_io* io, void* hip_stream) {
    using namespace macjd;
    if (!sampler_args_ok(io)) return set_nets_err(MACJD_EINVAL, "macjd_sample_episodes: bad argument");
    hipLaunchKernelGGL(sample_episodes_kernel, dim3(1), dim3(256), 0, (hipStream_t)hip_stream, *io);
    hipError_t err = hipGetLastError();
    if (err != hipSuccess) return set_nets_err(MACJD_EDEVICE, hipGetErrorString(err));
    return MACJD_OK;
}

extern "C" int macjd_clip_adam_step_sample(const macjd_adam_io* io, const macjd_sampler_io* next, void* hip_stream) {
    using namespace macjd;
    if (!io || io->n < 1 || !io->param || !io->grad || !io->exp_avg || !io->exp_avg_sq || !io->step || !io->grad_norm ||
        !io->partials)
        return set_nets_err(MACJD_EINVAL, "macjd_clip_adam_step: bad argument");
    if (next && !sampler_args_ok(next)) return set_nets_err(MACJD_EINVAL, "macjd_clip_adam_step_sample: bad sampler argument");
    hipStream_t s = (hipStream_t)hip_stream;
    int blocks = (int)((io->n + 255) / 256);
    if (blocks > ADAM_BLOCKS) blocks = ADAM_BLOCKS;
    hipLaunchKernelGGL(adam_sqnorm_kernel, dim3(blocks), dim3(256), 0, s, *io);
    if (next) hipLaunchKernelGGL(adam_update_kernel<true>, dim3(blocks), dim3(256), 0, s, *io, blocks, *next);
    else hipLaunchKernelGGL(adam_update_kernel<false>, dim3(blocks), dim3(256), 0, s, *io, blocks, macjd_sampler_io{});
    hipError_t err = hipGetLastError();
    if (err != hipSuccess) return set_nets_err(MACJD_EDEVICE, hipGetErrorString(err));
    return MACJD_OK;
}

extern "C" int macjd_clip_adam_step(const macjd_adam_io* io, void* hip_stream) {
    return macjd_clip_adam_step_sample(io, nullptr, hip_stream);
}

extern "C" int macjd_clip_adam_step_ln(const macjd_adam_io* io, const macjd_sampler_io* next, const macjd_lnparam_io* ln,
                                       int64_t gamma_off, int64_t beta_off, void* hip_stream) {
    using namespace macjd;
    if (!io || io->n < 1 || !io->param || !io->grad || !io->exp_avg || !io->exp_avg_sq || !io->step || !io->grad_norm ||
        !io->partials)
        return set_nets_err(MACJD_EINVAL, "macjd_clip_adam_step_ln: bad argument");
    if (next && !sampler_args_ok(next)) return set_nets_err(MACJD_EINVAL, "macjd_clip_adam_step_ln: bad sampler argument");
    if (!ln || ln->C < 1 || ln->K < 1 || ln->K > 1024 || !ln->W || !ln->G || !ln->gb || ln->w_ld < ln->K || ln->g_ld < ln->K)
        return set_nets_err(MACJD_EINVAL, "macjd_clip_adam_step_ln: bad LayerNorm argument");
    if (gamma_off < 0 || beta_off < 0 || gamma_off + ln->K > io->n || beta_off + ln->K > io->n ||
        ln->dgamma != io->grad + gamma_off || ln->dbeta != io->grad + beta_off)
        return set_nets_err(MACJD_EINVAL, "macjd_clip_adam_step_ln: dgamma / dbeta must be the named ranges of the gradient vector");
    hipStream_t s = (hipStream_t)hip_stream;
    int blocks = (int)((io->n + 255) / 256);
    if (blocks > ADAM_BLOCKS) blocks = ADAM_BLOCKS;
    hipLaunchKernelGGL(adam_sqnorm_ln_kernel, dim3(blocks + ln->K), dim3(256), 0, s, *io, *ln, gamma_off, beta_off, blocks);
    if (next) hipLaunchKernelGGL(adam_update_kernel<true>, dim3(blocks), dim3(256), 0, s, *io, blocks + ln->K, *next);
    else hipLaunchKernelGGL(adam_update_kernel<false>, dim3(blocks), dim3(256), 0, s, *io, blocks + ln->K, macjd_sampler_io{});
    hipError_t err = hipGetLastError();
    if (err != hipSuccess) return set_nets_err(MACJD_EDEVICE, hipGetErrorString(err));
    return MACJD_OK;
}

static int gather_tensors_ok(const macjd_gather_io* io) {
    if (io->n_tensors < 1 || io->n_tensors > 8) return 0;
    for (int k = 0; k < io->n_tensors; ++k)
        if (!io->src[k] || !io->dst[k] || io->row_bytes[k] < 4 || (io->row_bytes[k] & 3) || (io->dst_row_bytes[k] & 3) ||
            (io->dst_row_bytes[k] && io->dst_row_bytes[k] < io->row_bytes[k]))
            return 0;
    return 1;
}

extern "C" int macjd_gather_rows(const macjd_gather_io* io, void* hip_stream) {
    using namespace macjd;
    if (!io || io->n_tensors < 1 || io->n_tensors > 8 || io->n_rows < 0 || !io->idx)
        return set_nets_err(MACJD_EINVAL, "macjd_gather_rows: bad argument");
    if (!gather_tensors_ok(io))
        return set_nets_err(MACJD_EINVAL, "macjd_gather_rows: bad tensor (row bytes must be a positive multiple of 4)");
    if (io->n_rows == 0) return MACJD_OK;
    hipLaunchKernelGGL(gather_rows_kernel, dim3(8, io->n_tensors, io->n_rows), dim3(256), 0, (hipStream_t)hip_stream, *io);
    hipError_t err = hipGetLastError();
    if (err != hipSuccess) return set_nets_err(MACJD_EDEVICE, hipGetErrorString(err));
    return MACJD_OK;
}

extern "C" int macjd_prefetch_batch_supported(int32_t n_nets, int32_t H, int32_t B) {
    return n_nets == 1 && H == 64 && B >= 1 && B <= macjd::PREFETCH_MAX_B && !macjd::env_options().gru_ksplit;
}

extern "C" int macjd_prefetch_batch(const macjd_prefetch_io* io, void* hip_stream) {
    using namespace macjd;
    if (!io) return set_nets_err(MACJD_EINVAL, "macjd_prefetch_batch: NULL io");
    const macjd_gru_io& g = io->gru;
    if (!macjd_prefetch_batch_supported(g.n_nets, g.H, g.B))
        return set_nets_err(MACJD_EUNSUPPORTED, "macjd_prefetch_batch: needs one network, H = 64, 1 <= B <= 1024, the unit-split scan");
    if (g.T < 1 || g.J < 1 || !g.obs || g.S < 1 || g.S > 256 || !g.w_hh[0] || !g.b_hh[0] || !g.h_out[0] || !g.fc1_w[0] ||
        !g.fc1_b[0] || !g.w_ih[0] || !g.b_ih[0])
        return set_nets_err(MACJD_EINVAL, "macjd_prefetch_batch: bad scan argument");
    if (!g.p_out[0] || g.Ah < 1 || g.Ah > 256 || g.A < 1 || g.A > 64)
        return set_nets_err(MACJD_EINVAL, "macjd_prefetch_batch: needs the in-kernel actor (Ah <= 256, A <= 64)");
    for (int l = 0; l < 3; ++l)
        if (!g.act_w[0][l] || !g.act_b[0][l]) return set_nets_err(MACJD_EINVAL, "macjd_prefetch_batch: needs the actor's three layers");
    if (!sampler_args_ok(&io->sampler) || io->sampler.n != g.B)
        return set_nets_err(MACJD_EINVAL, "macjd_prefetch_batch: bad sampler argument (n must be the batch size)");
    if (io->gather.n_rows != g.B || !gather_tensors_ok(&io->gather))
        return set_nets_err(MACJD_EINVAL, "macjd_prefetch_batch: bad gather argument (n_rows must be the batch size, row bytes "
                                          "positive multiples of 4)");
    if (io->mask.B != g.B || io->mask.Tm1 < 1 || !io->mask.filled || !io->tot_m)
        return set_nets_err(MACJD_EINVAL, "macjd_prefetch_batch: bad mask-sum argument");
    if (io->gather_blocks < 0) return set_nets_err(MACJD_EINVAL, "macjd_prefetch_batch: bad gather_blocks");
    macjd_prefetch_io a = *io;
    const int n_parts = PREFETCH_ROW_PARTS * a.gather.n_tensors * g.B;
    if (a.gather_blocks == 0) a.gather_blocks = 256;
    if (a.gather_blocks > n_parts) a.gather_blocks = n_parts;
    const unsigned grid = 2u * (unsigned)(g.B * g.J) + (unsigned)a.gather_blocks + 1u;
    hipLaunchKernelGGL(prefetch_batch_kernel, dim3(grid), dim3(256), 0, (hipStream_t)hip_stream, a);
    hipError_t err = hipGetLastError();
    if (err != hipSuccess) return set_nets_err(MACJD_EDEVICE, hipGetErrorString(err));
    return MACJD_OK;
}

namespace macjd {

__global__ void __launch_bounds__(256) qhead_input_kernel(const macjd_qinput_io io) {
    const int W = io.H + io.A + 1;
    const int64_t total = io.n_rows * W;
    for (int64_t i = (int64_t)blockIdx.x * blockDim.x + threadIdx.x; i < total; i += (int64_t)gridDim.x * blockDim.x) {
        const int64_t n = i / W;
        const int c = (int)(i - n * W);
        float v;
        if (c < io.H) {
            v = io.h[n * io.h_ld + c];
        } else if (c < io.H + io.A) {
            const int64_t a = (io.idx_elem_size == 8) ? ((const int64_t*)io.idx)[n] : (int64_t)((const int32_t*)io.idx)[n];
            v = (a == (int64_t)(c - io.H)) ? 1.0f : 0.0f;
        } else {
            v = io.P[n];
        }
        io.out[n * io.out_ld + c] = v;
    }
}

__global__ void __launch_bounds__(256) layernorm_forward_kernel(const macjd_layernorm_io io) {
    const int lane = threadIdx.x & 63;
    const int64_t wave = (int64_t)blockIdx.x * (blockDim.x >> 6) + (threadIdx.x >> 6);
    const int64_t n_waves = (int64_t)gridDim.x * (blockDim.x >> 6);
    const int S = io.S;
    const float inv_s = 1.0f / (float)S;
    for (int64_t m = wave; m < io.M; m += n_waves) {
        const float* __restrict__ x = io.x + m * io.x_ld;
        float v[16];
        float sum = 0.0f;
#pragma unroll
        for (int i = 0; i < 16; ++i) {
            const int c = lane + 64 * i;
            v[i] = (c < S) ? x[c] : 0.0f;
            sum += v[i];
        }
#pragma unroll
        for (int o = 32; o > 0; o >>= 1) sum += __shfl_xor(sum, o);
        const float mean = sum * inv_s;
        float sq = 0.0f;
#pragma unroll
        for (int i = 0; i < 16; ++i) {
            const int c = lane + 64 * i;
            const float d = (c < S) ? v[i] - mean : 0.0f;
            sq = fmaf(d, d, sq);
        }
#pragma unroll
        for (int o = 32; o > 0; o >>= 1) sq += __shfl_xor(sq, o);
        const float rstd = rsqrtf(sq * inv_s + io.eps);
        float* __restrict__ y = io.y + m * io.y_ld;
#pragma unroll
        for (int i = 0; i < 16; ++i) {
            const int c = lane + 64 * i;
            if (c < S) {
                const float g = io.gamma ? io.gamma[c] : 1.0f, b = io.beta ? io.beta[c] : 0.0f;
                y[c] = (v[i] - mean) * rstd * g + b;
                if (io.xhat) io.xhat[m * io.xhat_ld + c] = (v[i] - mean) * rstd;
            }
        }
        if (lane == 0) {
            if (io.mean) io.mean[m] = mean;
            if (io.rstd) io.rstd[m] = rstd;
// ... 244 lines not shown
```

ma-cjd-cooperative-jamming-decision-making-via-marl_amd/csrc/macjd_wgrad.hip:

```cpp
#include <hip/hip_runtime.h>
#include <stdint.h>

#include "../../include/macjd.h"
#include "../../include/macjd_nets.h"
#include "macjd_err.h"

namespace macjd {

typedef float f32x4 __attribute__((ext_vector_type(4)));
#ifndef MACJD_WG_KC
#define MACJD_WG_KC 64
#endif
#ifndef MACJD_WG_ABLATE
#define MACJD_WG_ABLATE 0
#endif
#ifndef MACJD_WG_SUB
#define MACJD_WG_SUB 1
#endif
constexpr int WG_BM = 64, WG_BN = 64, WG_KC = MACJD_WG_KC, WG_PITCH = 80, WG_SUB = MACJD_WG_SUB;
constexpr int WG_ROWS = WG_KC * WG_SUB;

__host__ __device__ inline int64_t wg_pad(int64_t v, int64_t m) { return (v + m - 1) / m * m; }

struct WgradProb {
    int64_t K, gout_ld, inp_ld;
    int M, N, Mp, Np, n_chunks;
    const float* gout;
    const float* inp;
    float* workspace;
    bool want_db;
    const float* outer_vec;
    const float* outer_w;
};

__device__ __forceinline__ void wgrad_partial_body(const WgradProb& io, const int tn, const int tm, const int chunk,
                                                   float* __restrict__ sA, float* __restrict__ sB) {
    const int Mp = io.Mp, Np = io.Np;
    const int m0 = tm * WG_BM, n0 = tn * WG_BN;
    const int64_t k0 = (int64_t)chunk * WG_ROWS;
    const int tid = threadIdx.x;
    constexpr int NIT = (WG_KC * 16) / 256;
    float4 va[NIT], vb[NIT];
    auto load_operand = [&](const float* __restrict__ base, const int64_t ld, const int cols, const int c0, const int piece,
                            float4* __restrict__ out) {
        const bool al16 = ((ld & 3) == 0) && ((((uintptr_t)base) & 15) == 0) && (c0 + 64 <= cols);
        const bool al8 = ((ld & 1) == 0) && ((cols & 1) == 0) && ((((uintptr_t)base) & 7) == 0) && cols >= 2;
        const int c4 = (tid & 15) * 4;
        int64_t roff[NIT];
        bool rok[NIT];
#pragma unroll
        for (int it = 0; it < NIT; ++it) {
            const int64_t k = k0 + (int64_t)piece * WG_KC + ((it * 256 + tid) >> 4);
            rok[it] = k < io.K && !(MACJD_WG_ABLATE & 2);
            roff[it] = (k < io.K ? k : io.K - 1) * ld;
        }
        if (al16) {
#pragma unroll
            for (int it = 0; it < NIT; ++it) out[it] = *reinterpret_cast<const float4*>(base + roff[it] + c0 + c4);
        } else if (al8) {
            const int ca = c0 + c4 < cols ? c0 + c4 : cols - 2, cb = c0 + c4 + 2 < cols ? c0 + c4 + 2 : cols - 2;
#pragma unroll
            for (int it = 0; it < NIT; ++it) {
                const float2 lo = *reinterpret_cast<const float2*>(base + roff[it] + ca);
                const float2 hi = *reinterpret_cast<const float2*>(base + roff[it] + cb);
                out[it] = float4{lo.x, lo.y, hi.x, hi.y};
            }
        } else {
            int cc[4];
#pragma unroll
            for (int e = 0; e < 4; ++e) cc[e] = c0 + c4 + e < cols ? c0 + c4 + e : cols - 1;
#pragma unroll
            for (int it = 0; it < NIT; ++it)
                out[it] = float4{base[roff[it] + cc[0]], base[roff[it] + cc[1]], base[roff[it] + cc[2]], base[roff[it] + cc[3]]};
        }
#pragma unroll
        for (int it = 0; it < NIT; ++it) {
            out[it].x = (rok[it] && c0 + c4 + 0 < cols) ? out[it].x : 0.0f;
            out[it].y = (rok[it] && c0 + c4 + 1 < cols) ? out[it].y : 0.0f;
            out[it].z = (rok[it] && c0 + c4 + 2 < cols) ? out[it].z : 0.0f;
            out[it].w = (rok[it] && c0 + c4 + 3 < cols) ? out[it].w : 0.0f;
        }
    };
    auto load_piece = [&](const int piece) {
        load_operand(io.gout, io.gout_ld, io.M, m0, piece, va);
        load_operand(io.inp, io.inp_ld, io.N, n0, piece, vb);
        if (io.outer_vec) {
            const int c4 = (tid & 15) * 4;
            float w4[4];
#pragma unroll
            for (int e = 0; e < 4; ++e) w4[e] = io.outer_w[m0 + c4 + e < io.M ? m0 + c4 + e : io.M - 1];
#pragma unroll
            for (int it = 0; it < NIT; ++it) {
                const int64_t k = k0 + (int64_t)piece * WG_KC + ((it * 256 + tid) >> 4);
                const float gv = io.outer_vec[k < io.K ? k : io.K - 1];
                va[it].x = (va[it].x > 0.0f) ? gv * w4[0] : 0.0f;
                va[it].y = (va[it].y > 0.0f) ? gv * w4[1] : 0.0f;
                va[it].z = (va[it].z > 0.0f) ? gv * w4[2] : 0.0f;
                va[it].w = (va[it].w > 0.0f) ? gv * w4[3] : 0.0f;
            }
        }
    };
    auto store_piece = [&]() {
#pragma unroll
        for (int it = 0; it < NIT; ++it) {
            const int idx = it * 256 + tid;
            const int r = idx >> 4, c4 = (idx & 15) * 4;
            *reinterpret_cast<float4*>(&sA[r * WG_PITCH + c4]) = va[it];
            *reinterpret_cast<float4*>(&sB[r * WG_PITCH + c4]) = vb[it];
        }
    };
    const int wave = tid >> 6, lane = tid & 63, li = lane & 15, lk = lane >> 4;
    const int wm = (wave >> 1) * 32, wn = (wave & 1) * 32;
    f32x4 acc[2][2];
#pragma unroll
    for (int a = 0; a < 2; ++a)
#pragma unroll
        for (int b = 0; b < 2; ++b) acc[a][b] = f32x4{0.f, 0.f, 0.f, 0.f};
    const float* pa = sA + lk * WG_PITCH + wm + li;
    const float* pb = sB + lk * WG_PITCH + wn + li;
    const bool bias_lane = io.want_db && tn == 0 && tid < WG_BM;
    float bias_sum = 0.0f;
    const int n_pieces = (int)((((io.K - k0) < (int64_t)WG_ROWS ? (io.K - k0) : (int64_t)WG_ROWS) + WG_KC - 1) / WG_KC);
    load_piece(0);
    store_piece();
    __syncthreads();
    for (int piece = 0; piece < n_pieces; ++piece) {
        const bool more = piece + 1 < n_pieces;
        if (more) load_piece(piece + 1);
        constexpr int KSTEPS = (MACJD_WG_ABLATE & 1) ? 2 : WG_KC / 4;
        float fa0 = pa[0], fa1 = pa[16], fb0 = pb[0], fb1 = pb[16];
        float ga0, ga1, gb0, gb1;
#pragma unroll 4
        for (int kk = 0; kk < KSTEPS; kk += 2) {
            acc[0][0] = __builtin_amdgcn_mfma_f32_16x16x4f32(fa0, fb0, acc[0][0], 0, 0, 0);
            __builtin_amdgcn_sched_barrier(0);
            ga0 = pa[(kk + 1) * 4 * WG_PITCH]; ga1 = pa[(kk + 1) * 4 * WG_PITCH + 16];
            gb0 = pb[(kk + 1) * 4 * WG_PITCH]; gb1 = pb[(kk + 1) * 4 * WG_PITCH + 16];
            __builtin_amdgcn_sched_barrier(0);
            acc[0][1] = __builtin_amdgcn_mfma_f32_16x16x4f32(fa0, fb1, acc[0][1], 0, 0, 0);
            acc[1][0] = __builtin_amdgcn_mfma_f32_16x16x4f32(fa1, fb0, acc[1][0], 0, 0, 0);
            acc[1][1] = __builtin_amdgcn_mfma_f32_16x16x4f32(fa1, fb1, acc[1][1], 0, 0, 0);
            __builtin_amdgcn_sched_barrier(0);
            acc[0][0] = __builtin_amdgcn_mfma_f32_16x16x4f32(ga0, gb0, acc[0][0], 0, 0, 0);
            __builtin_amdgcn_sched_barrier(0);
            const int kn = (kk + 2 < KSTEPS) ? kk + 2 : KSTEPS - 1;
            fa0 = pa[kn * 4 * WG_PITCH]; fa1 = pa[kn * 4 * WG_PITCH + 16];
            fb0 = pb[kn * 4 * WG_PITCH]; fb1 = pb[kn * 4 * WG_PITCH + 16];
            __builtin_amdgcn_sched_barrier(0);
            acc[0][1] = __builtin_amdgcn_mfma_f32_16x16x4f32(ga0, gb1, acc[0][1], 0, 0, 0);
            acc[1][0] = __builtin_amdgcn_mfma_f32_16x16x4f32(ga1, gb0, acc[1][0], 0, 0, 0);
            acc[1][1] = __builtin_amdgcn_mfma_f32_16x16x4f32(ga1, gb1, acc[1][1], 0, 0, 0);
            __builtin_amdgcn_sched_barrier(0);
        }
        if (bias_lane) {
            float sp = 0.0f;
#pragma unroll 8
            for (int r = 0; r < WG_KC; ++r) sp += sA[r * WG_PITCH + tid];
            bias_sum += sp;
        }
        if (more) {
            __syncthreads();
            store_piece();
            __syncthreads();
        }
    }
    float* ws = io.workspace + (int64_t)chunk * Mp * Np;
#pragma unroll
    for (int a = 0; a < 2; ++a)
#pragma unroll
        for (int b = 0; b < 2; ++b)
#pragma unroll
            for (int r = 0; r < 4; ++r) {
                const int m = m0 + wm + a * 16 + lk * 4 + r;
                const int n = n0 + wn + b * 16 + li;
                if (!(MACJD_WG_ABLATE & 4) || acc[a][b][r] == 12345.678f) ws[(int64_t)m * Np + n] = acc[a][b][r];
            }
    if (bias_lane) io.workspace[(int64_t)io.n_chunks * Mp * Np + (int64_t)chunk * Mp + m0 + tid] = bias_sum;
}

__global__ void __launch_bounds__(256) wgrad_partial_kernel(const macjd_wgrad_io io, const int Mp, const int Np) {
    __shared__ float sA[WG_KC * WG_PITCH];
    __shared__ float sB[WG_KC * WG_PITCH];
    WgradProb p;
    p.K = io.K; p.gout_ld = io.gout_ld; p.inp_ld = io.inp_ld; p.M = io.M; p.N = io.N; p.Mp = Mp; p.Np = Np;
    p.n_chunks = (int)gridDim.z; p.gout = io.gout; p.inp = io.inp; p.workspace = io.workspace; p.want_db = io.db != nullptr;
    p.outer_vec = io.outer_vec; p.outer_w = io.outer_w;
    wgrad_partial_body(p, blockIdx.x, blockIdx.y, blockIdx.z, sA, sB);
}

__device__ __forceinline__ float wgrad_sum_rounds(const float* __restrict__ p, const int64_t stride, const int n_chunks, const int wave) {
    float a[8];
#pragma unroll
    for (int s8 = 0; s8 < 8; ++s8) a[s8] = 0.0f;
    for (int c = 8 * wave; c < n_chunks; c += 32) {
        float v[8];
#pragma unroll
        for (int s8 = 0; s8 < 8; ++s8) {
            const int cc = c + s8 < n_chunks ? c + s8 : n_chunks - 1;
            v[s8] = p[(int64_t)cc * stride];
        }
#pragma unroll
        for (int s8 = 0; s8 < 8; ++s8) a[s8] += (c + s8 < n_chunks) ? v[s8] : 0.0f;
    }
    return ((a[0] + a[1]) + (a[2] + a[3])) + ((a[4] + a[5]) + (a[6] + a[7]));
}

constexpr int WG_RED = 64;

__device__ __forceinline__ float wgrad_meet(float (*part)[WG_RED], const float mine, const int wave, const int lane) {
    part[wave][lane] = mine;
    __syncthreads();
    const float out = (part[0][lane] + part[1][lane]) + (part[2][lane] + part[3][lane]);
    __syncthreads();
    return out;
}

__global__ void __launch_bounds__(256) wgrad_reduce_kernel(const macjd_wgrad_io io, const int Mp, const int Np,
                                                           const int n_chunks) {
    __shared__ float part[4][WG_RED];
    const int lane = threadIdx.x & 63, wave = threadIdx.x >> 6;
    const int64_t total = (int64_t)io.M * io.N, all = total + (io.db ? io.M : 0);
    for (int64_t i0 = (int64_t)blockIdx.x * WG_RED; i0 < all; i0 += (int64_t)gridDim.x * WG_RED) {
        const int64_t i = i0 + lane < all ? i0 + lane : all - 1;
        const float* src;
        int64_t stride;
        float* dst;
        if (i < total) {
            const int m = (int)(i / io.N), n = (int)(i - (int64_t)m * io.N);
            src = io.workspace + (int64_t)m * Np + n; stride = (int64_t)Mp * Np; dst = io.dW + (int64_t)m * io.dw_ld + n;
        } else {
            const int m = (int)(i - total);
            src = io.workspace + (int64_t)n_chunks * Mp * Np + m; stride = Mp; dst = io.db + m;
        }
        const float v = wgrad_meet(part, wgrad_sum_rounds(src, stride, n_chunks, wave), wave, lane);
        if (wave == 0 && i0 + lane < all) *dst = v;
    }
}

struct WgradBatch {
    macjd_wgrad_io io[MACJD_WGRAD_MAX_BATCH];
    int Mp[MACJD_WGRAD_MAX_BATCH], Np[MACJD_WGRAD_MAX_BATCH], chunks[MACJD_WGRAD_MAX_BATCH];
    int tiles_n[MACJD_WGRAD_MAX_BATCH], tiles_m[MACJD_WGRAD_MAX_BATCH];
    int64_t wg_start[MACJD_WGRAD_MAX_BATCH + 1];
    int64_t out_start[MACJD_WGRAD_MAX_BATCH + 1];
    int n;
};

__global__ void __launch_bounds__(256) wgrad_partial_many_kernel(const WgradBatch b) {
    __shared__ float sA[WG_KC * WG_PITCH];
    __shared__ float sB[WG_KC * WG_PITCH];
    const int64_t w = blockIdx.x;
    WgradProb p;
    int tiles_n = b.tiles_n[0], tiles_m = b.tiles_m[0];
    int64_t start = 0;
#define MACJD_PICK(q)                                                                                               \
    p.K = b.io[q].K; p.gout_ld = b.io[q].gout_ld; p.inp_ld = b.io[q].inp_ld; p.M = b.io[q].M; p.N = b.io[q].N;       \
    p.Mp = b.Mp[q]; p.Np = b.Np[q]; p.n_chunks = b.chunks[q]; p.gout = b.io[q].gout; p.inp = b.io[q].inp;            \
    p.workspace = b.io[q].workspace; p.want_db = b.io[q].db != nullptr; tiles_n = b.tiles_n[q]; tiles_m = b.tiles_m[q]; \
    p.outer_vec = b.io[q].outer_vec; p.outer_w = b.io[q].outer_w;                                                    \
    start = b.wg_start[q];
    MACJD_PICK(0)
#pragma unroll
    for (int q = 1; q < MACJD_WGRAD_MAX_BATCH; ++q) {
        if (q < b.n && w >= b.wg_start[q]) { MACJD_PICK(q) }
    }
#undef MACJD_PICK
    const int local = (int)(w - start);
    const int tn = local % tiles_n, rest = local / tiles_n;
    const int tm = rest % tiles_m, chunk = rest / tiles_m;
    wgrad_partial_body(p, tn, tm, chunk, sA, sB);
}

__global__ void __launch_bounds__(256) wgrad_reduce_many_kernel(const WgradBatch b) {
    __shared__ float part[4][WG_RED];
    const int lane = threadIdx.x & 63, wave = threadIdx.x >> 6;
    const int64_t total_all = b.out_start[b.n];
    for (int64_t g0 = (int64_t)blockIdx.x * WG_RED; g0 < total_all; g0 += (int64_t)gridDim.x * WG_RED) {
        const int64_t g = g0 + lane < total_all ? g0 + lane : total_all - 1;
        int M = b.io[0].M, N = b.io[0].N, Mp = b.Mp[0], Np = b.Np[0], n_chunks = b.chunks[0];
        int64_t start = 0, dw_ld = b.io[0].dw_ld;
        const float* workspace = b.io[0].workspace;
        float* dW = b.io[0].dW;
        float* db = b.io[0].db;
#pragma unroll
        for (int q = 1; q < MACJD_WGRAD_MAX_BATCH; ++q) {
            if (q < b.n && g >= b.out_start[q]) {
                M = b.io[q].M; N = b.io[q].N; Mp = b.Mp[q]; Np = b.Np[q]; n_chunks = b.chunks[q];
                start = b.out_start[q]; dw_ld = b.io[q].dw_ld; workspace = b.io[q].workspace; dW = b.io[q].dW; db = b.io[q].db;
            }
        }
        const int64_t i = g - start;
        const int64_t total = (int64_t)M * N;
        const bool is_w = i < total;
        const int m = is_w ? (int)(i / N) : (int)(i - total);
        const int n = is_w ? (int)(i - (int64_t)m * N) : 0;
        const float* src = is_w ? workspace + (int64_t)m * Np + n : workspace + (int64_t)n_chunks * Mp * Np + m;
        const float v = wgrad_meet(part, wgrad_sum_rounds(src, is_w ? (int64_t)Mp * Np : (int64_t)Mp, n_chunks, wave), wave, lane);
        if (wave == 0 && g0 + lane < total_all) {
            if (is_w) dW[(int64_t)m * dw_ld + n] = v;
            else if (db) db[m] = v;
        }
    }
}

}

extern "C" int64_t macjd_linear_wgrad_workspace_floats(int64_t K, int32_t M, int32_t N) {
    using namespace macjd;
    if (K < 1 || M < 1 || N < 1) return -1;
    const int64_t chunks = (K + WG_ROWS - 1) / WG_ROWS, Mp = wg_pad(M, WG_BM), Np = wg_pad(N, WG_BN);
    return chunks * Mp * Np + chunks * Mp;
}

extern "C" int macjd_linear_wgrad(const macjd_wgrad_io* io, void* hip_stream) {
    using namespace macjd;
    if (!io || io->K < 1 || io->M < 1 || io->N < 1 || !io->gout || !io->inp || !io->dW || !io->workspace)
        return set_err(MACJD_EINVAL, "%s", "macjd_linear_wgrad: bad argument");
    if (io->gout_ld < io->M || io->inp_ld < io->N || io->dw_ld < io->N)
        return set_err(MACJD_EINVAL, "%s", "macjd_linear_wgrad: bad leading dimension");
    if ((io->outer_vec == nullptr) != (io->outer_w == nullptr))
        return set_err(MACJD_EINVAL, "%s", "macjd_linear_wgrad: outer_vec and outer_w go together");
    const int Mp = (int)wg_pad(io->M, WG_BM), Np = (int)wg_pad(io->N, WG_BN);
    const int64_t chunks = (io->K + WG_ROWS - 1) / WG_ROWS;
    if (chunks > 65535) return set_err(MACJD_EUNSUPPORTED, "%s", "macjd_linear_wgrad: K too large");
    hipStream_t s = (hipStream_t)hip_stream;
    hipLaunchKernelGGL(wgrad_partial_kernel, dim3(Np / WG_BN, Mp / WG_BM, (unsigned)chunks), dim3(256), 0, s, *io, Mp, Np);
    const int64_t total = (int64_t)io->M * io->N + io->M;
    const unsigned rblocks = (unsigned)((total + WG_RED - 1) / WG_RED < 8192 ? (total + WG_RED - 1) / WG_RED : 8192);
    hipLaunchKernelGGL(wgrad_reduce_kernel, dim3(rblocks), dim3(256), 0, s, *io, Mp, Np, (int)chunks);
    hipError_t err = hipGetLastError();
    if (err != hipSuccess) return set_err(MACJD_EDEVICE, "macjd_linear_wgrad: %s", hipGetErrorString(err));
    return MACJD_OK;
}

extern "C" int macjd_linear_wgrad_many(const macjd_wgrad_io* ios, int32_t n, void* hip_stream) {
    using namespace macjd;
    if (!ios || n < 1 || n > MACJD_WGRAD_MAX_BATCH)
        return set_err(MACJD_EINVAL, "%s", "macjd_linear_wgrad_many: 1..MACJD_WGRAD_MAX_BATCH problems");
    WgradBatch b{};
    b.n = n;
    for (int p = 0; p < n; ++p) {
        const macjd_wgrad_io* io = &ios[p];
        if (io->K < 1 || io->M < 1 || io->N < 1 || !io->gout || !io->inp || !io->dW || !io->workspace)
            return set_err(MACJD_EINVAL, "%s", "macjd_linear_wgrad_many: bad argument");
        if (io->gout_ld < io->M || io->inp_ld < io->N || io->dw_ld < io->N)
            return set_err(MACJD_EINVAL, "%s", "macjd_linear_wgrad_many: bad leading dimension");
        if ((io->outer_vec == nullptr) != (io->outer_w == nullptr))
            return set_err(MACJD_EINVAL, "%s", "macjd_linear_wgrad_many: outer_vec and outer_w go together");
        b.io[p] = *io;
        b.Mp[p] = (int)wg_pad(io->M, WG_BM);
        b.Np[p] = (int)wg_pad(io->N, WG_BN);
        b.chunks[p] = (int)((io->K + WG_ROWS - 1) / WG_ROWS);
        b.tiles_n[p] = b.Np[p] / WG_BN;
        b.tiles_m[p] = b.Mp[p] / WG_BM;
        b.wg_start[p + 1] = b.wg_start[p] + (int64_t)b.tiles_n[p] * b.tiles_m[p] * b.chunks[p];
        b.out_start[p + 1] = b.out_start[p] + (int64_t)io->M * io->N + io->M;
    }
    for (int p = n; p < MACJD_WGRAD_MAX_BATCH; ++p) {
        b.wg_start[p + 1] = b.wg_start[n];
        b.out_start[p + 1] = b.out_start[n];
        b.tiles_n[p] = b.tiles_m[p] = 1;
    }
    if (b.wg_start[n] > 0x7fffffff) return set_err(MACJD_EUNSUPPORTED, "%s", "macjd_linear_wgrad_many: too many work items");
    hipStream_t s = (hipStream_t)hip_stream;
    hipLaunchKernelGGL(wgrad_partial_many_kernel, dim3((unsigned)b.wg_start[n]), dim3(256), 0, s, b);
    const int64_t total = b.out_start[n];
    const unsigned rblocks = (unsigned)((total + WG_RED - 1) / WG_RED < 8192 ? (total + WG_RED - 1) / WG_RED : 8192);
    hipLaunchKernelGGL(wgrad_reduce_many_kernel, dim3(rblocks), dim3(256), 0, s, b);
    hipError_t err = hipGetLastError();
    if (err != hipSuccess) return set_err(MACJD_EDEVICE, "macjd_linear_wgrad_many: %s", hipGetErrorString(err));
    return MACJD_OK;
}
```

ma-cjd-cooperative-jamming-decision-making-via-marl_amd/ops.py:

```python
from __future__ import annotations

import ctypes
import os
from typing import Optional, Tuple

import numpy as np
import torch
import torch.nn.functional as F

from . import _native, options


def _stream(t: torch.Tensor) -> int:
    return torch.cuda.current_stream(t.device).cuda_stream


def _f32c(t: torch.Tensor) -> torch.Tensor:
    if t.dtype != torch.float32:
        t = t.float()
    return t if t.stride(-1) == 1 else t.contiguous()


def _qhead_fill(io: _native.QheadIO, base, P_all, W1, w2, b2, H: int, A: int, n_agents: int):
    io.n_rows, io.H, io.A, io.n_agents = base.shape[0], H, A, n_agents
# ... 907 lines not shown
    io1, y1, _ = _mlp_io(x1, layers1, keep)
    with torch.cuda.device(x0.device):
        _native.check(lib.macjd_mlp_forward_pair(ctypes.byref(io0), ctypes.byref(io1), _stream(x0)), "macjd_mlp_forward_pair")
    return y0, y1


def td_loss_reference(y, tq, reward, terminated, filled, gamma):
    targets = reward + gamma * (1 - terminated.float()) * tq
    m = filled.float()
    td = (y - targets.detach()) * m
    return (td ** 2).sum() / m.sum(), y.detach().mean(), targets.mean()


class _TdLossHip(torch.autograd.Function):

    @staticmethod
    def forward(ctx, y_full, tq_full, reward, terminated, filled, gamma, Tm1, tq_off):
        lib = _native.load()
        B, Ty = y_full.shape[0], y_full.shape[1]
        yc, tqc = y_full.detach().float().contiguous(), tq_full.detach().float().contiguous()
        stats = torch.empty(4, dtype=torch.float32, device=yc.device)
        gy = torch.empty((B, Ty, 1), dtype=torch.float32, device=yc.device)
        io = _native.TdLossIO()
        io.B, io.Tm1, io.gamma = B, int(Tm1), float(gamma)
        io.y, io.y_sb = yc.data_ptr(), Ty
        io.tq, io.tq_sb = tqc.data_ptr() + 4 * int(tq_off), tqc.shape[1]
        io.gy, io.gy_sb, io.gy_cols = gy.data_ptr(), Ty, Ty
        io.reward, io.r_sb, io.r_st = reward.data_ptr(), reward.stride(0), reward.stride(1)
        io.terminated, io.t_sb, io.t_st = terminated.data_ptr(), terminated.stride(0), terminated.stride(1)
        io.filled, io.f_sb, io.f_st = filled.data_ptr(), filled.stride(0), filled.stride(1)
        io.stats = stats.data_ptr()
        with torch.cuda.device(yc.device):
            _native.check(lib.macjd_td_loss(ctypes.byref(io), _stream(yc)), "macjd_td_loss")
        ctx.save_for_backward(gy)
        ctx.mark_non_differentiable(stats)
        stats.saved_gy = gy
        return stats[0], stats

    @staticmethod
    def backward(ctx, g_loss, _g_stats):
        (gy,) = ctx.saved_tensors
        return gy * g_loss, None, None, None, None, None, None, None


def td_loss_full(y_full, tq_full, reward, terminated, filled, gamma, Tm1, tq_off):
    loss, stats = _TdLossHip.apply(y_full, tq_full, reward, terminated, filled, gamma, Tm1, tq_off)
    return loss, stats[1], stats[2]


def td_loss_and_grad(y_full, tq_full, reward, terminated, filled, gamma, Tm1, tq_off):
    with torch.no_grad():
        _, stats = _TdLossHip.apply(y_full, tq_full, reward, terminated, filled, gamma, Tm1, tq_off)
    return stats[0], stats[1], stats[2], stats.saved_gy, stats


def td_loss_sums_into(row, y_full, tq_full, reward, terminated, filled, gamma, Tm1, tq_off):
    lib = _native.load()
    io, keep = _tdloss_sums_io(row, y_full, tq_full, reward, terminated, filled, gamma, Tm1, tq_off)
    with torch.cuda.device(row.device):
        _native.check(lib.macjd_td_loss(ctypes.byref(io), _stream(row)), "macjd_td_loss")
    return row


def _tdloss_sums_io(row, y_full, tq_full, reward, terminated, filled, gamma, Tm1, tq_off):
    B, Ty = y_full.shape[0], y_full.shape[1]
    yc, tqc = y_full.detach(), tq_full.detach()
    assert yc.dtype == torch.float32 and tqc.dtype == torch.float32 and yc.is_contiguous() and tqc.is_contiguous()
    assert row.dtype == torch.float32 and row.numel() >= 3 and row.is_contiguous()
    io = _native.TdLossIO()
    io.B, io.Tm1, io.gamma = B, int(Tm1), float(gamma)
    io.y, io.y_sb = yc.data_ptr(), Ty
    io.tq, io.tq_sb = tqc.data_ptr() + 4 * int(tq_off), tqc.shape[1]
    io.reward, io.r_sb, io.r_st = reward.data_ptr(), reward.stride(0), reward.stride(1)
    io.terminated, io.t_sb, io.t_st = terminated.data_ptr(), terminated.stride(0), terminated.stride(1)
    io.filled, io.f_sb, io.f_st = filled.data_ptr(), filled.stride(0), filled.stride(1)
    io.stats, io.gy = row.data_ptr(), None
    return io, (row, yc, tqc, reward, terminated, filled)


def td_mask_sum(filled, Tm1):
    lib = _native.load()
    out = torch.empty(1, dtype=torch.float32, device=filled.device)
    io = _native.TdLossIO()
    io.B, io.Tm1 = filled.shape[0], int(Tm1)
    io.filled, io.f_sb, io.f_st = filled.data_ptr(), filled.stride(0), filled.stride(1)
    with torch.cuda.device(filled.device):
        _native.check(lib.macjd_td_mask_sum(ctypes.byref(io), out.data_ptr(), _stream(filled)), "macjd_td_mask_sum")
    return out


_PENDING_TD = None


def fused_mixer_backward_will_run(y_full) -> bool:
    fn = getattr(y_full, "grad_fn", None)
    for _ in range(4):
        if fn is None:
            return False
        if type(fn).__name__.startswith("_FusedMixer"):
            return True
        nxt = [f for f, _ in fn.next_functions if f is not None]
        if len(nxt) != 1:
            return False
        fn = nxt[0]
    return False


def td_grad_in_mixer_backward(y_full, tq_full, reward, terminated, filled, gamma, Tm1, tq_off, tot_m, stats_row=None):
    global _PENDING_TD
    B, Ty = y_full.shape[0], y_full.shape[1]
    yc, tqc = y_full.detach().float().contiguous(), tq_full.detach().float().contiguous()
    io = _native.TdLossIO()
    io.B, io.Tm1, io.gamma = B, int(Tm1), float(gamma)
    io.y, io.y_sb = yc.data_ptr(), Ty
    io.tq, io.tq_sb = tqc.data_ptr() + 4 * int(tq_off), tqc.shape[1]
    io.gy, io.gy_sb, io.gy_cols = None, Ty, Ty
    io.reward, io.r_sb, io.r_st = reward.data_ptr(), reward.stride(0), reward.stride(1)
    io.terminated, io.t_sb, io.t_st = terminated.data_ptr(), terminated.stride(0), terminated.stride(1)
    io.filled, io.f_sb, io.f_st = filled.data_ptr(), filled.stride(0), filled.stride(1)
    if stats_row is not None:
        assert stats_row.dtype == torch.float32 and stats_row.numel() >= 3 and stats_row.is_contiguous()
        io.stats = stats_row.data_ptr()
    _PENDING_TD = (io, (yc, tqc, reward, terminated, filled, tot_m, stats_row), B * Ty, tot_m)
    return torch.empty((B, Ty, 1), dtype=torch.float32, device=yc.device)


def td_loss(y, tq, reward, terminated, filled, gamma):
    ok = (y.is_cuda and reward.dtype == torch.float32 and terminated.dtype == torch.bool and filled.dtype == torch.bool
          and y.shape[1] > 0)
    if not ok:
        return td_loss_reference(y, tq, reward, terminated, filled, gamma)
    loss, stats = _TdLossHip.apply(y, tq, reward, terminated, filled, gamma, y.shape[1], 0)
    return loss, stats[1], stats[2]


def _sampler_io(idx_out, n_stored, counter, seed, offset=0):
    assert idx_out.dtype == torch.int64 and idx_out.is_contiguous() and n_stored.dtype == torch.int32 and counter.dtype == torch.int64
    assert idx_out.is_cuda and n_stored.device == idx_out.device and counter.device == idx_out.device
    sp = _native.SamplerIO()
    sp.idx_out, sp.n, sp.n_stored, sp.counter = idx_out.data_ptr(), idx_out.numel(), n_stored.data_ptr(), counter.data_ptr()
    sp.seed = int(seed) & 0xFFFFFFFFFFFFFFFF
    sp.reserved = int(offset)
    return sp


def sample_episodes(idx_out, n_stored, counter, seed, offset=0):
    lib = _native.load()
    sp = _sampler_io(idx_out, n_stored, counter, seed, offset)
    with torch.cuda.device(idx_out.device):
        _native.check(lib.macjd_sample_episodes(ctypes.byref(sp), _stream(idx_out)), "macjd_sample_episodes")


def clip_adam_step(param, grad, exp_avg, exp_avg_sq, step, grad_norm, partials, lr, betas, eps, max_norm, sample_next=None,
                   lnparam=None):
    lib = _native.load()
    io = _native.AdamIO()
    io.n, io.lr, io.beta1, io.beta2, io.eps, io.max_norm = param.numel(), lr, betas[0], betas[1], eps, max_norm
    io.param, io.grad, io.exp_avg, io.exp_avg_sq = param.data_ptr(), grad.data_ptr(), exp_avg.data_ptr(), exp_avg_sq.data_ptr()
    io.step, io.grad_norm, io.partials = step.data_ptr(), grad_norm.data_ptr(), partials.data_ptr()
    sp = _sampler_io(*sample_next) if sample_next is not None else None
    spp = ctypes.byref(sp) if sp is not None else None
    held = list(lnparam or [])
    fuse = None
    if len(held) == 1:
        lio, esz, base = held[0].lnparam, grad.element_size(), grad.data_ptr()
        g_off, b_off = (lio.dgamma - base) // esz, (lio.dbeta - base) // esz
        if ((lio.dgamma - base) % esz == 0 and (lio.dbeta - base) % esz == 0 and 0 <= g_off <= grad.numel() - lio.K
                and 0 <= b_off <= grad.numel() - lio.K and partials.numel() >= 256 + lio.K):
            fuse = (lio, int(g_off), int(b_off))
    with torch.cuda.device(param.device):
        if fuse is not None:
            _native.check(lib.macjd_clip_adam_step_ln(ctypes.byref(io), spp, ctypes.byref(fuse[0]), fuse[1], fuse[2],
                                                      _stream(param)), "macjd_clip_adam_step_ln")
            return
        for fn in held:
            fn()
        _native.check(lib.macjd_clip_adam_step_sample(ctypes.byref(io), spp, _stream(param)), "macjd_clip_adam_step")


def gather_rows_supported(srcs) -> bool:
    return len(srcs) <= 8 and all(s.is_cuda and s.is_contiguous() and (s[0].numel() * s.element_size()) % 4 == 0
                                  for s in srcs)


def _gather_io(n_rows, srcs, dsts):
    io = _native.GatherIO()
    io.n_tensors, io.n_rows = len(srcs), int(n_rows)
    for k, (s_, d_) in enumerate(zip(srcs, dsts)):
        assert d_.is_contiguous() and d_.dtype == s_.dtype and d_.shape[0] == n_rows and d_[0].numel() >= s_[0].numel()
        io.src[k], io.dst[k], io.row_bytes[k] = s_.data_ptr(), d_.data_ptr(), s_[0].numel() * s_.element_size()
        io.dst_row_bytes[k] = d_.stride(0) * d_.element_size()
    return io


def gather_rows(idx, srcs, dsts):
    lib = _native.load()
    io = _gather_io(idx.numel(), srcs, dsts)
    io.idx = idx.data_ptr()
    with torch.cuda.device(idx.device):
        _native.check(lib.macjd_gather_rows(ctypes.byref(io), _stream(idx)), "macjd_gather_rows")


def prefetch_batch_supported(agents, B: int, srcs) -> bool:
    return (len(agents) == 1 and gather_rows_supported(srcs)
            and bool(_native.load().macjd_prefetch_batch_supported(len(agents), int(agents[0].rnn_hidden_dim), int(B))))


def prefetch_batch(obs, agents, B: int, J: int, n_steps: int, sampler, srcs, dsts, filled, Tm1: int, offset: int = 0,
                   draw: bool = True, gather_blocks: int = 0):
    lib = _native.load()
    if not prefetch_batch_supported(agents, B, srcs):
        raise _native.NativeLibraryError("macjd_prefetch_batch: unsupported shape (one agent body, rnn_hidden_dim 64, B <= 1024)")
    gio, outs, pouts, _keep = _gru_from_obs_io(obs, None, agents, B, J, n_steps, True)
    assert sampler[0].numel() == B and filled.dtype == torch.bool and filled.device == obs.device and filled.shape[1] >= Tm1
    io = _native.PrefetchIO()
    io.gru, io.gather, io.sampler = gio, _gather_io(B, srcs, dsts), _sampler_io(*sampler[:4], offset)
    io.mask.B, io.mask.Tm1 = int(B), int(Tm1)
    io.mask.filled, io.mask.f_sb, io.mask.f_st = filled.data_ptr(), filled.stride(0), filled.stride(1)
    tot_m = torch.empty(1, dtype=torch.float32, device=obs.device)
    io.tot_m, io.no_draw, io.gather_blocks = tot_m.data_ptr(), 0 if draw else 1, int(gather_blocks)
    with torch.cuda.device(obs.device):
        _native.check(lib.macjd_prefetch_batch(ctypes.byref(io), _stream(obs)), "macjd_prefetch_batch")
    return outs, pouts, tot_m


_DEFERRED_WGRAD = None
_DEFERRED_POST = None
_GRAD_DST = None
_DEFERRED_SEEN = None


def grad_key(t):
    return None if t is None else (t.data_ptr(), t.numel())


def _grad_dst(key, shape):
    if not _GRAD_DST or key is None:
        return None
    dst = _GRAD_DST.get(key)
    if dst is None or dst.numel() != int(np.prod(shape)) or not dst.is_contiguous():
        return None
    del _GRAD_DST[key]
    return dst.view(shape)


class deferred_wgrad:

    def __init__(self, grad_dst=None, hold_lnparam=False):
        self._grad_dst = grad_dst
        self._hold, self.held = bool(hold_lnparam), []

    def __enter__(self):
        global _DEFERRED_WGRAD, _DEFERRED_POST, _GRAD_DST, _DEFERRED_SEEN
        self._prev, _DEFERRED_WGRAD = _DEFERRED_WGRAD, []
        self._prev_post, _DEFERRED_POST = _DEFERRED_POST, []
        self._prev_dst, _GRAD_DST = _GRAD_DST, (dict(self._grad_dst) if self._grad_dst else None)
        self._prev_seen, _DEFERRED_SEEN = _DEFERRED_SEEN, set()
        return self

    def __exit__(self, *exc):
        global _DEFERRED_WGRAD, _DEFERRED_POST, _GRAD_DST, _DEFERRED_SEEN
        pending, _DEFERRED_WGRAD = _DEFERRED_WGRAD, self._prev
        post, _DEFERRED_POST = _DEFERRED_POST, self._prev_post
        _GRAD_DST, _DEFERRED_SEEN = self._prev_dst, self._prev_seen
        self._flush(exc, pending)
        if exc[0] is None:
            for fn in post:
                if self._hold and hasattr(fn, "lnparam"):
                    self.held.append(fn)
                else:
                    fn()
        return False

    @staticmethod
    def _flush(exc, pending):
        if exc[0] is None and pending:
            lib = _native.load()
            dev = pending[0][1][0].device
            for lo in range(0, len(pending), 8):
                part = pending[lo:lo + 8]
                arr = (_native.WgradIO * len(part))(*[io for io, _ in part])
                with torch.cuda.device(dev):
                    _native.check(lib.macjd_linear_wgrad_many(arr, len(part), _stream(part[0][1][0])),
                                  "macjd_linear_wgrad_many")


def linear_wgrad(gout, inp, want_bias=True, w_key=None, b_key=None, need=(True, True), outer=None):
    lib = _native.load()
    gout, inp = _f32c(gout), _f32c(inp)
    K, M = gout.shape
    N = inp.shape[1]
    if outer is not None:
        o_vec, o_w = _f32c(outer[0]).reshape(-1).contiguous(), _f32c(outer[1]).reshape(-1).contiguous()
        assert o_vec.numel() == K and o_w.numel() == M
    dW = _grad_dst(w_key, (M, N))
    if dW is None:
        dW = torch.empty((M, N), dtype=torch.float32, device=gout.device)
    db = None
    if want_bias:
        db = _grad_dst(b_key, (M,))
        if db is None:
            db = torch.empty((M,), dtype=torch.float32, device=gout.device)
    ws = torch.empty(int(lib.macjd_linear_wgrad_workspace_floats(K, M, N)), dtype=torch.float32, device=gout.device)
    io = _native.WgradIO()
    io.K, io.M, io.N = K, M, N
    io.gout, io.gout_ld, io.inp, io.inp_ld = gout.data_ptr(), gout.stride(0), inp.data_ptr(), inp.stride(0)
    io.dW, io.dw_ld, io.db, io.workspace = dW.data_ptr(), dW.stride(0), (db.data_ptr() if want_bias else None), ws.data_ptr()
    if outer is not None:
        io.outer_vec, io.outer_w = o_vec.data_ptr(), o_w.data_ptr()
    if _DEFERRED_WGRAD is not None and any(k is not None and k in _DEFERRED_SEEN for k in (w_key, b_key)):
        pending, posts = list(_DEFERRED_WGRAD), list(_DEFERRED_POST)
        del _DEFERRED_WGRAD[:], _DEFERRED_POST[:]
        deferred_wgrad._flush((None, None, None), pending)
        for fn in posts:
            fn()
    elif _DEFERRED_WGRAD is not None:
        _DEFERRED_SEEN.update(k for k in (w_key, b_key) if k is not None)
        unowned = tuple(t for t, n in ((dW, need[0]), (db, need[1])) if t is not None and not n)
        _DEFERRED_WGRAD.append((io, (ws, gout, inp) + unowned + ((o_vec, o_w) if outer is not None else ())))
        return dW, db
    with torch.cuda.device(gout.device):
        _native.check(lib.macjd_linear_wgrad(ctypes.byref(io), _stream(gout)), "macjd_linear_wgrad")
    return dW, db


class _LinearSplitK(torch.autograd.Function):

    @staticmethod
    def forward(ctx, x, weight, bias):
        ctx.save_for_backward(x, weight)
        ctx.has_bias, ctx.b_key = bias is not None, grad_key(bias)
        return F.linear(x, weight, bias)

    @staticmethod
    def backward(ctx, gy):
        x, weight = ctx.saved_tensors
        gx = gy.matmul(weight) if ctx.needs_input_grad[0] else None
        gW = gb = None
        if ctx.needs_input_grad[1] or (ctx.has_bias and ctx.needs_input_grad[2]):
            gW, gb = linear_wgrad(gy.reshape(-1, gy.shape[-1]), x.reshape(-1, x.shape[-1]), want_bias=ctx.has_bias,
                                  w_key=grad_key(weight), b_key=ctx.b_key,
                                  need=(ctx.needs_input_grad[1], ctx.has_bias and ctx.needs_input_grad[2]))
        return gx, gW, (gb if ctx.has_bias else None)


class _MergedLinear(torch.autograd.Function):

    @staticmethod
    def forward(ctx, x, w_cat, b_cat, *params):
        ctx.save_for_backward(x, w_cat)
        ctx.sizes, ctx.b_key = [p.shape[0] for p in params[:len(params) // 2]], grad_key(b_cat)
        return F.linear(x, w_cat, b_cat)

    @staticmethod
    def backward(ctx, gy):
        x, w_cat = ctx.saved_tensors
        gx = gy.matmul(w_cat) if ctx.needs_input_grad[0] else None
        gW, gb = linear_wgrad(gy, x, want_bias=True, w_key=grad_key(w_cat), b_key=ctx.b_key)
        return (gx, None, None) + tuple(gW.split(ctx.sizes, 0)) + tuple(gb.split(ctx.sizes, 0))


def merged_linear(x, w_cat, b_cat, params):
    return _MergedLinear.apply(x, w_cat, b_cat, *params)


def _layernorm_launch(x, weight, bias, eps, want_xhat):
    lib = _native.load()
    x = _f32c(x.detach())
    M, S = x.shape
    y = torch.empty((M, S), dtype=torch.float32, device=x.device)
    mean = torch.empty((M, 1), dtype=torch.float32, device=x.device)
    rstd = torch.empty((M, 1), dtype=torch.float32, device=x.device)
    xhat = torch.empty((M, S), dtype=torch.float32, device=x.device) if want_xhat else None
    io = _native.LayerNormIO()
    io.M, io.S, io.eps = M, S, float(eps)
    io.x, io.x_ld, io.y, io.y_ld = x.data_ptr(), x.stride(0), y.data_ptr(), y.stride(0)
    io.gamma = weight.data_ptr() if weight is not None else None
    io.beta = bias.data_ptr() if bias is not None else None
    io.mean, io.rstd = mean.data_ptr(), rstd.data_ptr()
    if want_xhat:
        io.xhat, io.xhat_ld = xhat.data_ptr(), xhat.stride(0)
    with torch.cuda.device(x.device):
        _native.check(lib.macjd_layernorm_forward(ctypes.byref(io), _stream(x)), "macjd_layernorm_forward")
    return x, y, mean, rstd, xhat


class _NormMergedLinear(torch.autograd.Function):

    @staticmethod
    def forward(ctx, x, gamma, beta, eps, w_cat, b_cat, *params):
        _, s_, _, _, xhat = _layernorm_launch(x, gamma, beta, eps, want_xhat=True)
        ctx.save_for_backward(s_, xhat, w_cat)
        ctx.sizes = [p.shape[0] for p in params[:len(params) // 2]]
        ctx.keys = (grad_key(b_cat), grad_key(gamma), grad_key(beta))
        return F.linear(s_, w_cat, b_cat)

    @staticmethod
    def backward(ctx, gy):
        s_, xhat, w_cat = ctx.saved_tensors
        assert not ctx.needs_input_grad[0], "norm_merged_linear is for inputs that need no gradient"
        gW, gb = linear_wgrad(gy, s_, want_bias=True, w_key=grad_key(w_cat), b_key=ctx.keys[0])
        G, _ = linear_wgrad(gy, xhat, want_bias=False)
        K = w_cat.shape[1]
        dgamma, dbeta = _grad_dst(ctx.keys[1], (K,)), _grad_dst(ctx.keys[2], (K,))
        if dgamma is None:
            dgamma = torch.empty(K, dtype=torch.float32, device=gy.device)
        if dbeta is None:
            dbeta = torch.empty(K, dtype=torch.float32, device=gy.device)
        io = _native.LnParamIO()
        io.C, io.K = w_cat.shape[0], K
        io.W, io.w_ld, io.G, io.g_ld = w_cat.data_ptr(), w_cat.stride(0), G.data_ptr(), G.stride(0)
        io.gb, io.dgamma, io.dbeta = gb.data_ptr(), dgamma.data_ptr(), dbeta.data_ptr()
        dev, stream = gy.device, _stream(gy)

        def post(io=io, keep=(G, w_cat), dev=dev, stream=stream):
            with torch.cuda.device(dev):
                _native.check(_native.load().macjd_layernorm_param_grad(ctypes.byref(io), stream), "macjd_layernorm_param_grad")

        post.lnparam = io
        if _DEFERRED_WGRAD is not None:
            _DEFERRED_POST.append(post)
        else:
            post()
        return (None, dgamma, dbeta, None, None, None) + tuple(gW.split(ctx.sizes, 0)) + tuple(gb.split(ctx.sizes, 0))


def norm_merged_linear(x, gamma, beta, eps, w_cat, b_cat, params):
    return _NormMergedLinear.apply(x, gamma, beta, eps, w_cat, b_cat, *params)


def deferred_wgrad_active() -> bool:
    return _DEFERRED_WGRAD is not None


def qhead_input(h, idx, P, n_actions: int):
    n, H = h.shape
    if not h.is_cuda:
# ... 367 lines not shown
```

ma-cjd-cooperative-jamming-decision-making-via-marl_amd/options.py:

```python
from __future__ import annotations

import os

_DEFAULTS = {
    "UPDATE_STREAMS": "2", "UPDATES_PER_GRAPH": "1", "PIPELINED_GROUP": "1", "SHARED_BODY": "1",
    "LEARNER_STATIC_OBS": "1", "ACTOR_IN_SCAN": "1", "DEVICE_SAMPLER": "1", "LN_IN_SQNORM": "1", "WGRAD_OUTER": "1",
    "QHEAD_TAKEN": "1", "QHEAD_DOUBLE_Q": "1", "QHEAD_DOUBLE_Q_H128": "0", "PAIRED_HEADS": "1", "MIXER_TRAIN": "1", "MIXER_STATIC_STATE": "1", "GRAPHED_ALLREDUCE": "0",
    "PREFETCH_LAUNCH": "1",
    "CLOSED_LOOP_ROLLOUT": "0",
}
_values = None


def reload() -> None:
    global _values
    _values = {k: os.environ.get("MACJD_" + k, d) for k, d in _DEFAULTS.items()}


def get(name: str) -> str:
    if _values is None:
        reload()
    return _values[name]


def on(name: str) -> bool:
    return get(name) != "0"
```

Measured before the change: 37.30 million env-steps/s.

## Fold grad-norm partials and LayerNorm grad contraction into batched wgrad reduce

Adds a batched weight-gradient path that writes squared-norm partials during its reduce pass and contracts the LayerNorm gamma/beta gradients inside the partial kernel. Adam then only sums those partials, which removes the separate sqnorm launch and the full pass over the flat gradient. A Python planner checks that the written gradient regions cover every trainable parameter before it takes this path, and otherwise falls back to the old one. This adds complexity and a coverage condition that can silently disable the path.

```diff
diff --git a/include/macjd.h b/include/macjd.h
--- a/include/macjd.h
+++ b/include/macjd.h
@@ -8,7 +8,7 @@
 extern "C" {
 #endif
 
-#define MACJD_ABI_VERSION 8
+#define MACJD_ABI_VERSION 9
 #define MACJD_PE_ROWS(R, J) (6 * (R) + 3 * (J) + (J) * (R))
 #define MACJD_PE_SCAN_ROWS(R, J) (10 * (R) + (J) * (R))
 
diff --git a/include/macjd_nets.h b/include/macjd_nets.h
--- a/include/macjd_nets.h
+++ b/include/macjd_nets.h
@@ -128,6 +128,19 @@
 int macjd_linear_wgrad(const macjd_wgrad_io* io, void* hip_stream);
 #define MACJD_WGRAD_MAX_BATCH 8
 int macjd_linear_wgrad_many(const macjd_wgrad_io* ios, int32_t n, void* hip_stream);
+
+typedef struct macjd_wgrad_norm_io {
+    int32_t ln_problem, partials_cap;
+    const float* W; int64_t w_ld;
+    float* dgamma; float* dbeta;
+    float* partials;
+    float* step;
+} macjd_wgrad_norm_io;
+
+int32_t macjd_linear_wgrad_many_norm_partials(const macjd_wgrad_io* ios, int32_t n, int32_t ln_problem);
+int macjd_linear_wgrad_many_norm(const macjd_wgrad_io* ios, int32_t n, const macjd_wgrad_norm_io* norm, void* hip_stream);
+
+int macjd_clip_adam_step_reduced(const macjd_adam_io* io, int32_t n_partials, const macjd_sampler_io* next, void* hip_stream);
 
 typedef struct macjd_gather_io {
     int32_t n_tensors, n_rows;
diff --git a/ma-cjd-cooperative-jamming-decision-making-via-marl_amd/_native.py b/ma-cjd-cooperative-jamming-decision-making-via-marl_amd/_native.py
--- a/ma-cjd-cooperative-jamming-decision-making-via-marl_amd/_native.py
+++ b/ma-cjd-cooperative-jamming-decision-making-via-marl_amd/_native.py
@@ -8,7 +8,7 @@
 LIB_NAME = "libmacjd_hip.so"
 LIB_PATH = os.environ.get("MACJD_LIB") or os.path.join(_PKG_DIR, LIB_NAME)
 
-ABI_VERSION = 8
+ABI_VERSION = 9
 STEP_ARITH_F64 = 1
 STEP_LANE_KERNEL = 2
 STEP_SLOT_KERNEL = 4
@@ -31,6 +31,7 @@
     "macjd_gru_sequence_backward_supported", "macjd_gru_sequence_backward",
     "macjd_prefetch_batch_supported", "macjd_prefetch_batch",
     "macjd_actor_gradient_supported", "macjd_actor_gradient",
+    "macjd_linear_wgrad_many_norm", "macjd_linear_wgrad_many_norm_partials", "macjd_clip_adam_step_reduced",
 ]
 
 
@@ -355,6 +356,14 @@
         ("gout", ctypes.c_void_p), ("gout_ld", ctypes.c_int64), ("inp", ctypes.c_void_p), ("inp_ld", ctypes.c_int64),
         ("dW", ctypes.c_void_p), ("dw_ld", ctypes.c_int64), ("db", ctypes.c_void_p), ("workspace", ctypes.c_void_p),
         ("outer_vec", ctypes.c_void_p), ("outer_w", ctypes.c_void_p),
+    ]
+
+
+class WgradNormIO(ctypes.Structure):
+    _fields_ = [
+        ("ln_problem", ctypes.c_int32), ("partials_cap", ctypes.c_int32),
+        ("W", ctypes.c_void_p), ("w_ld", ctypes.c_int64), ("dgamma", ctypes.c_void_p), ("dbeta", ctypes.c_void_p),
+        ("partials", ctypes.c_void_p), ("step", ctypes.c_void_p),
     ]
 
 
@@ -497,6 +506,12 @@
     lib.macjd_gather_rows.argtypes = [ctypes.POINTER(GatherIO), ctypes.c_void_p]
     lib.macjd_linear_wgrad.restype = ctypes.c_int
     lib.macjd_linear_wgrad.argtypes = [ctypes.POINTER(WgradIO), ctypes.c_void_p]
+    lib.macjd_linear_wgrad_many_norm.restype = ctypes.c_int
+    lib.macjd_linear_wgrad_many_norm.argtypes = [ctypes.POINTER(WgradIO), ctypes.c_int32, ctypes.POINTER(WgradNormIO), ctypes.c_void_p]
+    lib.macjd_linear_wgrad_many_norm_partials.restype = ctypes.c_int32
+    lib.macjd_linear_wgrad_many_norm_partials.argtypes = [ctypes.POINTER(WgradIO), ctypes.c_int32, ctypes.c_int32]
+    lib.macjd_clip_adam_step_reduced.restype = ctypes.c_int
+    lib.macjd_clip_adam_step_reduced.argtypes = [ctypes.POINTER(AdamIO), ctypes.c_int32, ctypes.POINTER(SamplerIO), ctypes.c_void_p]
     lib.macjd_linear_wgrad_many.restype = ctypes.c_int
     lib.macjd_linear_wgrad_many.argtypes = [ctypes.POINTER(WgradIO), ctypes.c_int32, ctypes.c_void_p]
     lib.macjd_linear_wgrad_workspace_floats.restype = ctypes.c_int64
diff --git a/ma-cjd-cooperative-jamming-decision-making-via-marl_amd/core/qmix.py b/ma-cjd-cooperative-jamming-decision-making-via-marl_amd/core/qmix.py
--- a/ma-cjd-cooperative-jamming-decision-making-via-marl_amd/core/qmix.py
+++ b/ma-cjd-cooperative-jamming-decision-making-via-marl_amd/core/qmix.py
@@ -96,6 +96,10 @@
         import torch.distributed as dist
         return dist.get_world_size() if (dist.is_available() and dist.is_initialized()) else 1
 
+    def _norm_in_reduce(self):
+        return (self._flat_param is not None and self._world_size() <= 1 and not self.train_agent_body
+                and not self.train_actor and options.on("NORM_IN_REDUCE"))
+
     def _flatten_trainable(self):
         tr = self._trainable()
         self._flat_offsets, off = [], 0
@@ -110,7 +114,7 @@
         self._flat_exp_avg_sq = torch.zeros_like(flat)
         self._adam_step = torch.zeros((), dtype=torch.float32, device=flat.device)
         self._grad_norm = torch.zeros((), dtype=torch.float32, device=flat.device)
-        self._adam_partials = torch.zeros(256 + 1024, dtype=torch.float32, device=flat.device)
+        self._adam_partials = torch.zeros(8192, dtype=torch.float32, device=flat.device)
         for p, off in zip(tr, self._flat_offsets):
             n = p.numel()
             p.data = flat[off:off + n].view_as(p)
@@ -118,6 +122,8 @@
                                        "exp_avg_sq": self._flat_exp_avg_sq[off:off + n].view_as(p)}
         self._flat_grad = torch.zeros_like(flat)
         self._grad_dst = {}
+        esz = self._flat_grad.element_size()
+        self._grad_cover = [(self._flat_grad.data_ptr() + off * esz, p.numel() * esz) for p, off in zip(tr, self._flat_offsets)]
         for p, off in zip(tr, self._flat_offsets):
             n = p.numel()
             self._grad_dst[ops.grad_key(p)] = self._flat_grad[off:off + n].view_as(p)
@@ -530,10 +536,11 @@
                 loss, eval_mean, target_mean, gy, self._last_stats4 = ops.td_loss_and_grad(
                     eval_q_tot, target_q_tot, st["reward"], st["terminated"], st["filled"], self.args.gamma, T - 1, 1)
             hold = self._flat_param is not None and self._world_size() <= 1 and options.on("LN_IN_SQNORM")
-            with ops.deferred_wgrad(grad_dst=getattr(self, "_grad_dst", None), hold_lnparam=hold) as dw:
+            norm = (self._adam_partials, self._adam_step, self._grad_cover) if self._norm_in_reduce() else None
+            with ops.deferred_wgrad(grad_dst=getattr(self, "_grad_dst", None), hold_lnparam=hold, norm=norm) as dw:
                 eval_q_tot.backward(gy)
             assert ops._PENDING_TD is None, "the fused mixer's backward did not take the TD loss's inputs"
-            self._held_ln = dw.held
+            self._held_ln, self._norm_partials = dw.held, dw.norm_partials
             if side_work is not None:
                 side_work()
             if sums_late is not None:
@@ -554,9 +561,10 @@
         if self._flat_param is not None:
             g = self.optimizer.param_groups[0]
             held, self._held_ln = getattr(self, "_held_ln", None), None
+            reduced, self._norm_partials = getattr(self, "_norm_partials", None), None
             ops.clip_adam_step(self._flat_param, self._flat_grad, self._flat_exp_avg, self._flat_exp_avg_sq,
                                self._adam_step, self._grad_norm, self._adam_partials, g["lr"], g["betas"], g["eps"],
-                               self.args.grad_norm_clip, sample_next=sample_next, lnparam=held)
+                               self.args.grad_norm_clip, sample_next=sample_next, lnparam=held, reduced=reduced)
             return self._grad_norm
         grad_norm = torch.nn.utils.clip_grad_norm_(self.params, self.args.grad_norm_clip)
         self.optimizer.step()
@@ -805,7 +813,7 @@
         self._g_multi = self._g_stages = None
         self._graph_a = self._graph_b = None
         self._graph_body_a = None
-        self._g_out_a = self._g_out_b = self._g_stats4 = self._last_stats4 = self._held_ln = None
+        self._g_out_a = self._g_out_b = self._g_stats4 = self._last_stats4 = self._held_ln = self._norm_partials = None
         if self._flat_param is not None and any(g is not None for g in graphs):
             self._grad_norm = torch.zeros((), dtype=torch.float32, device=self._flat_param.device)
         hipgraph.destroy(graphs, self.device)
diff --git a/ma-cjd-cooperative-jamming-decision-making-via-marl_amd/csrc/macjd_nets.hip b/ma-cjd-cooperative-jamming-decision-making-via-marl_amd/csrc/macjd_nets.hip
--- a/ma-cjd-cooperative-jamming-decision-making-via-marl_amd/csrc/macjd_nets.hip
+++ b/ma-cjd-cooperative-jamming-decision-making-via-marl_amd/csrc/macjd_nets.hip
@@ -867,6 +867,50 @@
     if (SAMPLE && blockIdx.x == 0) sample_episodes_block(next);
 }
 
+template <bool SAMPLE>
+__device__ __forceinline__ void adam_apply(const macjd_adam_io& io, const float total_norm, const macjd_sampler_io& next) {
+    float coef = io.max_norm / (total_norm + 1e-6f);
+    coef = coef < 1.0f ? coef : 1.0f;
+    const float step = io.step[0];
+    const float bc1 = 1.0f - powf(io.beta1, step);
+    const float bc2 = 1.0f - powf(io.beta2, step);
+    const float step_size = io.lr / bc1;
+    const float bc2_sqrt = sqrtf(bc2);
+    for (int64_t i = (int64_t)blockIdx.x * blockDim.x + threadIdx.x; i < io.n; i += (int64_t)gridDim.x * blockDim.x) {
+        const float g = io.grad[i] * coef;
+        io.grad[i] = g;
+        float m = io.exp_avg[i], v = io.exp_avg_sq[i];
+        m = m + (1.0f - io.beta1) * (g - m);
+        v = v * io.beta2 + (1.0f - io.beta2) * g * g;
+        io.exp_avg[i] = m;
+        io.exp_avg_sq[i] = v;
+        const float denom = sqrtf(v) / bc2_sqrt + io.eps;
+        io.param[i] -= step_size * (m / denom);
+    }
+    if (blockIdx.x == 0 && threadIdx.x == 0) io.grad_norm[0] = total_norm;
+    if (SAMPLE && blockIdx.x == 0) sample_episodes_block(next);
+}
+
+template <bool SAMPLE>
+__global__ void __launch_bounds__(256) adam_update_reduced_kernel(const macjd_adam_io io, const int n_partials, const macjd_sampler_io next) {
+    __shared__ float s_w[4];
+    float s = 0.0f;
+    for (int base = 0; base < n_partials; base += 8 * 256) {
+        float v[8];
+#pragma unroll
+        for (int j = 0; j < 8; ++j) {
+            const int i = base + j * 256 + (int)threadIdx.x;
+            v[j] = io.partials[i < n_partials ? i : n_partials - 1];
+        }
+#pragma unroll
+        for (int j = 0; j < 8; ++j) s += (base + j * 256 + (int)threadIdx.x < n_partials) ? v[j] : 0.0f;
+    }
+    s = wave_sum(s);
+    if ((threadIdx.x & 63) == 0) s_w[threadIdx.x >> 6] = s;
+    __syncthreads();
+    adam_apply<SAMPLE>(io, sqrtf((s_w[0] + s_w[1]) + (s_w[2] + s_w[3])), next);
+}
+
 __device__ __forceinline__ void gather_rows_body(const macjd_gather_io& io, const int k, const int row, const int64_t src_row,
                                                  const int part, const int parts) {
     const int64_t words = io.row_bytes[k] >> 2;
@@ -954,6 +998,22 @@
     hipLaunchKernelGGL(adam_sqnorm_kernel, dim3(blocks), dim3(256), 0, s, *io);
     if (next) hipLaunchKernelGGL(adam_update_kernel<true>, dim3(blocks), dim3(256), 0, s, *io, blocks, *next);
     else hipLaunchKernelGGL(adam_update_kernel<false>, dim3(blocks), dim3(256), 0, s, *io, blocks, macjd_sampler_io{});
+    hipError_t err = hipGetLastError();
+    if (err != hipSuccess) return set_nets_err(MACJD_EDEVICE, hipGetErrorString(err));
+    return MACJD_OK;
+}
+
+extern "C" int macjd_clip_adam_step_reduced(const macjd_adam_io* io, int32_t n_partials, const macjd_sampler_io* next, void* hip_stream) {
+    using namespace macjd;
+    if (!io || io->n < 1 || !io->param || !io->grad || !io->exp_avg || !io->exp_avg_sq || !io->step || !io->grad_norm ||
+        !io->partials || n_partials < 1)
+        return set_nets_err(MACJD_EINVAL, "macjd_clip_adam_step_reduced: bad argument");
+    if (next && !sampler_args_ok(next)) return set_nets_err(MACJD_EINVAL, "macjd_clip_adam_step_reduced: bad sampler argument");
+    hipStream_t s = (hipStream_t)hip_stream;
+    int blocks = (int)((io->n + 255) / 256);
+    if (blocks > ADAM_BLOCKS) blocks = ADAM_BLOCKS;
+    if (next) hipLaunchKernelGGL(adam_update_reduced_kernel<true>, dim3(blocks), dim3(256), 0, s, *io, n_partials, *next);
+    else hipLaunchKernelGGL(adam_update_reduced_kernel<false>, dim3(blocks), dim3(256), 0, s, *io, n_partials, macjd_sampler_io{});
     hipError_t err = hipGetLastError();
     if (err != hipSuccess) return set_nets_err(MACJD_EDEVICE, hipGetErrorString(err));
     return MACJD_OK;
diff --git a/ma-cjd-cooperative-jamming-decision-making-via-marl_amd/csrc/macjd_wgrad.hip b/ma-cjd-cooperative-jamming-decision-making-via-marl_amd/csrc/macjd_wgrad.hip
--- a/ma-cjd-cooperative-jamming-decision-making-via-marl_amd/csrc/macjd_wgrad.hip
+++ b/ma-cjd-cooperative-jamming-decision-making-via-marl_amd/csrc/macjd_wgrad.hip
@@ -31,8 +31,11 @@
     bool want_db;
     const float* outer_vec;
     const float* outer_w;
+    const float* ln_W;
+    int64_t ln_ld;
 };
 
+template <bool LN>
 __device__ __forceinline__ void wgrad_partial_body(const WgradProb& io, const int tn, const int tm, const int chunk,
                                                    float* __restrict__ sA, float* __restrict__ sB) {
     const int Mp = io.Mp, Np = io.Np;
@@ -118,9 +121,28 @@
         for (int b = 0; b < 2; ++b) acc[a][b] = f32x4{0.f, 0.f, 0.f, 0.f};
     const float* pa = sA + lk * WG_PITCH + wm + li;
     const float* pb = sB + lk * WG_PITCH + wn + li;
-    const bool bias_lane = io.want_db && tn == 0 && tid < WG_BM;
+    bool contract = false;
+    if constexpr (LN) contract = io.ln_W != nullptr;
+    const bool bias_lane = (io.want_db || contract) && tn == 0 && tid < WG_BM;
     float bias_sum = 0.0f;
-    const int n_pieces = (int)((((io.K - k0) < (int64_t)WG_ROWS ? (io.K - k0) : (int64_t)WG_ROWS) + WG_KC - 1) / WG_KC);
+    float wl[2][2][4];
+    if constexpr (LN) {
+        const float* wbase = contract ? io.ln_W : io.gout;
+        const int64_t wld = contract ? io.ln_ld : 0;
+#pragma unroll
+        for (int a = 0; a < 2; ++a)
+#pragma unroll
+            for (int b = 0; b < 2; ++b)
+#pragma unroll
+                for (int r = 0; r < 4; ++r) {
+                    const int m = m0 + wm + a * 16 + lk * 4 + r, n = n0 + wn + b * 16 + li;
+                    const int mc = m < io.M ? m : io.M - 1, nc = n < io.N ? n : io.N - 1;
+                    const float v = wbase[(int64_t)mc * wld + (contract ? nc : 0)];
+                    wl[a][b][r] = (contract && m < io.M && n < io.N) ? v : 0.0f;
+                }
+    }
+    const int n_pieces = (LN && WG_SUB == 1) ? 1
+        : (int)((((io.K - k0) < (int64_t)WG_ROWS ? (io.K - k0) : (int64_t)WG_ROWS) + WG_KC - 1) / WG_KC);
     load_piece(0);
     store_piece();
     __syncthreads();
@@ -164,6 +186,39 @@
             __syncthreads();
         }
     }
+    if constexpr (LN) {
+        if (contract) {
+            __syncthreads();
+            float* gbs = sA;
+            float* red = sB;
+            if (tid < WG_BM) gbs[tid] = bias_sum;
+            __syncthreads();
+#pragma unroll
+            for (int b = 0; b < 2; ++b) {
+                float sg = 0.0f, sb = 0.0f;
+#pragma unroll
+                for (int a = 0; a < 2; ++a)
+#pragma unroll
+                    for (int r = 0; r < 4; ++r) {
+                        sg = fmaf(wl[a][b][r], acc[a][b][r], sg);
+                        sb = fmaf(wl[a][b][r], gbs[wm + a * 16 + lk * 4 + r], sb);
+                    }
+                sg += __shfl_xor(sg, 16, 64); sg += __shfl_xor(sg, 32, 64);
+                sb += __shfl_xor(sb, 16, 64); sb += __shfl_xor(sb, 32, 64);
+                if (lk == 0) {
+                    red[((wave >> 1) * 2 + 0) * WG_BN + wn + b * 16 + li] = sg;
+                    red[((wave >> 1) * 2 + 1) * WG_BN + wn + b * 16 + li] = sb;
+                }
+            }
+            __syncthreads();
+            if (tid < 2 * WG_BN) {
+                const int which = tid >> 6, n = tid & 63;
+                const float v = red[which * WG_BN + n] + red[(2 + which) * WG_BN + n];
+                if (n < io.N) io.workspace[((int64_t)tm * io.n_chunks + chunk) * 2 * io.N + which * io.N + n] = v;
+            }
+            return;
+        }
+    }
     float* ws = io.workspace + (int64_t)chunk * Mp * Np;
 #pragma unroll
     for (int a = 0; a < 2; ++a)
@@ -176,6 +231,12 @@
                 if (!(MACJD_WG_ABLATE & 4) || acc[a][b][r] == 12345.678f) ws[(int64_t)m * Np + n] = acc[a][b][r];
             }
     if (bias_lane) io.workspace[(int64_t)io.n_chunks * Mp * Np + (int64_t)chunk * Mp + m0 + tid] = bias_sum;
+}
+
+__device__ __forceinline__ float wgrad_wave_sum(float x) {
+#pragma unroll
+    for (int off = 32; off > 0; off >>= 1) x += __shfl_xor(x, off, 64);
+    return x;
 }
 
 __global__ void __launch_bounds__(256) wgrad_partial_kernel(const macjd_wgrad_io io, const int Mp, const int Np) {
@@ -185,7 +246,7 @@
     p.K = io.K; p.gout_ld = io.gout_ld; p.inp_ld = io.inp_ld; p.M = io.M; p.N = io.N; p.Mp = Mp; p.Np = Np;
     p.n_chunks = (int)gridDim.z; p.gout = io.gout; p.inp = io.inp; p.workspace = io.workspace; p.want_db = io.db != nullptr;
     p.outer_vec = io.outer_vec; p.outer_w = io.outer_w;
-    wgrad_partial_body(p, blockIdx.x, blockIdx.y, blockIdx.z, sA, sB);
+    wgrad_partial_body<false>(p, blockIdx.x, blockIdx.y, blockIdx.z, sA, sB);
 }
 
 __device__ __forceinline__ float wgrad_sum_rounds(const float* __restrict__ p, const int64_t stride, const int n_chunks, const int wave) {
@@ -264,11 +325,10 @@
     for (int q = 1; q < MACJD_WGRAD_MAX_BATCH; ++q) {
         if (q < b.n && w >= b.wg_start[q]) { MACJD_PICK(q) }
     }
-#undef MACJD_PICK
     const int local = (int)(w - start);
     const int tn = local % tiles_n, rest = local / tiles_n;
     const int tm = rest % tiles_m, chunk = rest / tiles_m;
-    wgrad_partial_body(p, tn, tm, chunk, sA, sB);
+    wgrad_partial_body<false>(p, tn, tm, chunk, sA, sB);
 }
 
 __global__ void __launch_bounds__(256) wgrad_reduce_many_kernel(const WgradBatch b) {
@@ -299,6 +359,80 @@
         if (wave == 0 && g0 + lane < total_all) {
             if (is_w) dW[(int64_t)m * dw_ld + n] = v;
             else if (db) db[m] = v;
+        }
+    }
+}
+
+struct WgradNorm {
+    int problem;
+    int slots;
+    const float* W; int64_t w_ld;
+    float* dgamma; float* dbeta;
+    float* partials; float* step;
+};
+
+__global__ void __launch_bounds__(256) wgrad_partial_many_norm_kernel(const WgradBatch b, const WgradNorm ln) {
+    __shared__ float sA[WG_KC * WG_PITCH];
+    __shared__ float sB[WG_KC * WG_PITCH];
+    const int64_t w = blockIdx.x;
+    WgradProb p;
+    int tiles_n = b.tiles_n[0], tiles_m = b.tiles_m[0];
+    int64_t start = 0;
+    MACJD_PICK(0)
+    p.ln_W = ln.problem == 0 ? ln.W : nullptr;
+#pragma unroll
+    for (int q = 1; q < MACJD_WGRAD_MAX_BATCH; ++q) {
+        if (q < b.n && w >= b.wg_start[q]) { MACJD_PICK(q) p.ln_W = ln.problem == q ? ln.W : nullptr; }
+    }
+    p.ln_ld = ln.w_ld;
+    const int local = (int)(w - start);
+    const int tn = local % tiles_n, rest = local / tiles_n;
+    const int tm = rest % tiles_m, chunk = rest / tiles_m;
+    wgrad_partial_body<true>(p, tn, tm, chunk, sA, sB);
+}
+#undef MACJD_PICK
+
+__global__ void __launch_bounds__(256) wgrad_reduce_many_norm_kernel(const WgradBatch b, const WgradNorm ln) {
+    __shared__ float part[4][WG_RED];
+    const int lane = threadIdx.x & 63, wave = threadIdx.x >> 6;
+    const int64_t total_all = b.out_start[b.n];
+    float sq = 0.0f;
+    for (int64_t g0 = (int64_t)blockIdx.x * WG_RED; g0 < total_all; g0 += (int64_t)gridDim.x * WG_RED) {
+        const int64_t g = g0 + lane < total_all ? g0 + lane : total_all - 1;
+        int M = b.io[0].M, N = b.io[0].N, Mp = b.Mp[0], Np = b.Np[0], n_chunks = b.chunks[0], prob = 0;
+        int64_t start = 0, dw_ld = b.io[0].dw_ld;
+        const float* workspace = b.io[0].workspace;
+        float* dW = b.io[0].dW;
+        float* db = b.io[0].db;
+#pragma unroll
+        for (int q = 1; q < MACJD_WGRAD_MAX_BATCH; ++q) {
+            if (q < b.n && g >= b.out_start[q]) {
+                M = b.io[q].M; N = b.io[q].N; Mp = b.Mp[q]; Np = b.Np[q]; n_chunks = b.chunks[q]; prob = q;
+                start = b.out_start[q]; dw_ld = b.io[q].dw_ld; workspace = b.io[q].workspace; dW = b.io[q].dW; db = b.io[q].db;
+            }
+        }
+        const int64_t i = g - start;
+        const int64_t total = (int64_t)M * N;
+        const bool is_ln = prob == ln.problem;
+        const bool is_w = i < total;
+        const int m = is_w ? (int)(i / N) : (int)(i - total);
+        const int n = is_w ? (int)(i - (int64_t)m * N) : 0;
+        const float* src = is_ln ? workspace + i : is_w ? workspace + (int64_t)m * Np + n : workspace + (int64_t)n_chunks * Mp * Np + m;
+        const int64_t stride = is_ln ? (int64_t)2 * N : is_w ? (int64_t)Mp * Np : (int64_t)Mp;
+        const float v = wgrad_meet(part, wgrad_sum_rounds(src, stride, is_ln ? ln.slots : n_chunks, wave), wave, lane);
+        if (wave == 0 && g0 + lane < total_all) {
+            float* dst = is_ln ? (i < N ? ln.dgamma + i : ln.dbeta + (i - N)) : is_w ? dW + (int64_t)m * dw_ld + n : db ? db + m : nullptr;
+            if (dst) {
+                *dst = v;
+                sq = fmaf(v, v, sq);
+            }
+        }
+    }
+    if (wave == 0) {
+        sq = wgrad_wave_sum(sq);
+        if (lane == 0) {
+            ln.partials[blockIdx.x] = sq;
+            if (blockIdx.x == 0) ln.step[0] += 1.0f;
         }
     }
 }
@@ -371,3 +505,76 @@
     if (err != hipSuccess) return set_err(MACJD_EDEVICE, "macjd_linear_wgrad_many: %s", hipGetErrorString(err));
     return MACJD_OK;
 }
+
+static int wgrad_norm_batch(const macjd_wgrad_io* ios, int32_t n, int32_t ln_problem, macjd::WgradBatch* out, const char* who) {
+    using namespace macjd;
+    if (!ios || n < 1 || n > MACJD_WGRAD_MAX_BATCH || ln_problem < -1 || ln_problem >= n)
+        return set_err(MACJD_EINVAL, "%s: 1..MACJD_WGRAD_MAX_BATCH problems, ln_problem -1 or one of them", who);
+    WgradBatch& b = *out;
+    b = WgradBatch{};
+    b.n = n;
+    for (int p = 0; p < n; ++p) {
+        const macjd_wgrad_io* io = &ios[p];
+        const bool is_ln = p == ln_problem;
+        if (io->K < 1 || io->M < 1 || io->N < 1 || !io->gout || !io->inp || (!io->dW && !is_ln) || !io->workspace)
+            return set_err(MACJD_EINVAL, "%s: bad argument", who);
+        if (io->gout_ld < io->M || io->inp_ld < io->N || (!is_ln && io->dw_ld < io->N))
+            return set_err(MACJD_EINVAL, "%s: bad leading dimension", who);
+        if ((io->outer_vec == nullptr) != (io->outer_w == nullptr))
+            return set_err(MACJD_EINVAL, "%s: outer_vec and outer_w go together", who);
+        if (is_ln && (io->N > WG_BN || io->db))
+            return set_err(MACJD_EUNSUPPORTED, "%s: the contracted problem has N <= 64 and no bias output", who);
+        b.io[p] = *io;
+        b.Mp[p] = (int)wg_pad(io->M, WG_BM);
+        b.Np[p] = (int)wg_pad(io->N, WG_BN);
+        b.chunks[p] = (int)((io->K + WG_ROWS - 1) / WG_ROWS);
+        b.tiles_n[p] = b.Np[p] / WG_BN;
+        b.tiles_m[p] = b.Mp[p] / WG_BM;
+        b.wg_start[p + 1] = b.wg_start[p] + (int64_t)b.tiles_n[p] * b.tiles_m[p] * b.chunks[p];
+        b.out_start[p + 1] = b.out_start[p] + (is_ln ? (int64_t)2 * io->N : (int64_t)io->M * io->N + io->M);
+    }
+    for (int p = n; p < MACJD_WGRAD_MAX_BATCH; ++p) {
+        b.wg_start[p + 1] = b.wg_start[n];
+        b.out_start[p + 1] = b.out_start[n];
+        b.tiles_n[p] = b.tiles_m[p] = 1;
+    }
+    if (b.wg_start[n] > 0x7fffffff) return set_err(MACJD_EUNSUPPORTED, "%s: too many work items", who);
+    return MACJD_OK;
+}
+
+static unsigned wgrad_reduce_blocks(int64_t total) {
+    using namespace macjd;
+    return (unsigned)((total + WG_RED - 1) / WG_RED < 8192 ? (total + WG_RED - 1) / WG_RED : 8192);
+}
+
+extern "C" int32_t macjd_linear_wgrad_many_norm_partials(const macjd_wgrad_io* ios, int32_t n, int32_t ln_problem) {
+    macjd::WgradBatch b;
+    if (wgrad_norm_batch(ios, n, ln_problem, &b, "macjd_linear_wgrad_many_norm_partials") != MACJD_OK) return -1;
+    return (int32_t)wgrad_reduce_blocks(b.out_start[n]);
+}
+
+extern "C" int macjd_linear_wgrad_many_norm(const macjd_wgrad_io* ios, int32_t n, const macjd_wgrad_norm_io* norm, void* hip_stream) {
+    using namespace macjd;
+    const char* who = "macjd_linear_wgrad_many_norm";
+    if (!norm || !norm->partials || !norm->step) return set_err(MACJD_EINVAL, "%s: bad argument", who);
+    WgradBatch b;
+    const int rc = wgrad_norm_batch(ios, n, norm->ln_problem, &b, who);
+    if (rc != MACJD_OK) return rc;
+    WgradNorm ln{};
+    ln.problem = norm->ln_problem;
+    ln.partials = norm->partials; ln.step = norm->step;
+    if (ln.problem >= 0) {
+        if (!norm->W || !norm->dgamma || !norm->dbeta || norm->w_ld < ios[ln.problem].N)
+            return set_err(MACJD_EINVAL, "%s: bad LayerNorm argument", who);
+        ln.W = norm->W; ln.w_ld = norm->w_ld; ln.dgamma = norm->dgamma; ln.dbeta = norm->dbeta;
+        ln.slots = b.tiles_m[ln.problem] * b.chunks[ln.problem];
+    }
+    const unsigned rblocks = wgrad_reduce_blocks(b.out_start[n]);
+    if ((int64_t)rblocks > (int64_t)norm->partials_cap) return set_err(MACJD_EINVAL, "%s: partials_cap too small", who);
+    hipStream_t s = (hipStream_t)hip_stream;
+    hipLaunchKernelGGL(wgrad_partial_many_norm_kernel, dim3((unsigned)b.wg_start[n]), dim3(256), 0, s, b, ln);
+    hipLaunchKernelGGL(wgrad_reduce_many_norm_kernel, dim3(rblocks), dim3(256), 0, s, b, ln);
+    hipError_t err = hipGetLastError();
+    if (err != hipSuccess) return set_err(MACJD_EDEVICE, "macjd_linear_wgrad_many_norm: %s", hipGetErrorString(err));
+    return MACJD_OK;
+}
diff --git a/ma-cjd-cooperative-jamming-decision-making-via-marl_amd/ops.py b/ma-cjd-cooperative-jamming-decision-making-via-marl_amd/ops.py
--- a/ma-cjd-cooperative-jamming-decision-making-via-marl_amd/ops.py
+++ b/ma-cjd-cooperative-jamming-decision-making-via-marl_amd/ops.py
@@ -1083,7 +1083,7 @@
 
 
 def clip_adam_step(param, grad, exp_avg, exp_avg_sq, step, grad_norm, partials, lr, betas, eps, max_norm, sample_next=None,
-                   lnparam=None):
+                   lnparam=None, reduced=None):
     lib = _native.load()
     io = _native.AdamIO()
     io.n, io.lr, io.beta1, io.beta2, io.eps, io.max_norm = param.numel(), lr, betas[0], betas[1], eps, max_norm
@@ -1100,6 +1100,11 @@
                 and 0 <= b_off <= grad.numel() - lio.K and partials.numel() >= 256 + lio.K):
             fuse = (lio, int(g_off), int(b_off))
     with torch.cuda.device(param.device):
+        if reduced is not None:
+            assert not held, "clip_adam_step: the reduce launch already formed the LayerNorm gradients"
+            _native.check(lib.macjd_clip_adam_step_reduced(ctypes.byref(io), int(reduced), spp, _stream(param)),
+                          "macjd_clip_adam_step_reduced")
+            return
         if fuse is not None:
             _native.check(lib.macjd_clip_adam_step_ln(ctypes.byref(io), spp, ctypes.byref(fuse[0]), fuse[1], fuse[2],
                                                       _stream(param)), "macjd_clip_adam_step_ln")
@@ -1177,9 +1182,10 @@
 
 class deferred_wgrad:
 
-    def __init__(self, grad_dst=None, hold_lnparam=False):
+    def __init__(self, grad_dst=None, hold_lnparam=False, norm=None):
         self._grad_dst = grad_dst
         self._hold, self.held = bool(hold_lnparam), []
+        self._norm, self.norm_partials = norm, None
 
     def __enter__(self):
         global _DEFERRED_WGRAD, _DEFERRED_POST, _GRAD_DST, _DEFERRED_SEEN
@@ -1194,6 +1200,13 @@
         pending, _DEFERRED_WGRAD = _DEFERRED_WGRAD, self._prev
         post, _DEFERRED_POST = _DEFERRED_POST, self._prev_post
         _GRAD_DST, _DEFERRED_SEEN = self._prev_dst, self._prev_seen
+        if exc[0] is None and self._norm is not None and pending:
+            partials, step, cover = self._norm
+            lns = [fn.lnparam for fn in post if hasattr(fn, "lnparam")]
+            q = norm_in_reduce_plan([io for io, _ in pending], lns, cover) if len(lns) == len(post) else None
+            if q is not None:
+                self.norm_partials = self._flush_norm(pending, q, lns[0], partials, step)
+                return False
         self._flush(exc, pending)
         if exc[0] is None:
             for fn in post:
@@ -1214,6 +1227,58 @@
                 with torch.cuda.device(dev):
                     _native.check(lib.macjd_linear_wgrad_many(arr, len(part), _stream(part[0][1][0])),
                                   "macjd_linear_wgrad_many")
+
+    @staticmethod
+    def _flush_norm(pending, q, lio, partials, step):
+        lib = _native.load()
+        arr = (_native.WgradIO * len(pending))(*[io for io, _ in pending])
+        n_partials = int(lib.macjd_linear_wgrad_many_norm_partials(arr, len(pending), q))
+        if n_partials < 1 or n_partials > partials.numel():
+            raise _native.NativeLibraryError("macjd_linear_wgrad_many_norm: partials buffer too small or bad problem set")
+        nio = _native.WgradNormIO()
+        nio.ln_problem, nio.partials_cap = q, partials.numel()
+        nio.W, nio.w_ld, nio.dgamma, nio.dbeta = lio.W, lio.w_ld, lio.dgamma, lio.dbeta
+        nio.partials, nio.step = partials.data_ptr(), step.data_ptr()
+        t0 = pending[0][1][0]
+        with torch.cuda.device(t0.device):
+            _native.check(lib.macjd_linear_wgrad_many_norm(arr, len(pending), ctypes.byref(nio), _stream(t0)),
+                          "macjd_linear_wgrad_many_norm")
+        return n_partials
+
+
+def norm_in_reduce_plan(ios, lns, cover):
+    if not ios or len(ios) > 8 or len(lns) != 1:
+        return None
+    ln = lns[0]
+    qs = [k for k, io in enumerate(ios) if io.dW == ln.G and not io.db]
+    if len(qs) != 1:
+        return None
+    q = qs[0]
+    g = ios[q]
+    if g.N > 64 or g.M != ln.C or g.N != ln.K or g.dw_ld != ln.g_ld or not ln.W or ln.w_ld < ln.K:
+        return None
+    same_operand = [io for k, io in enumerate(ios) if k != q and io.db and io.db == ln.gb and
+                    (io.gout, io.gout_ld, io.K, io.M, io.outer_vec, io.outer_w) == (g.gout, g.gout_ld, g.K, g.M, g.outer_vec, g.outer_w)]
+    if not same_operand:
+        return None
+    written = [(ln.dgamma, 4 * ln.K), (ln.dbeta, 4 * ln.K)]
+    for k, io in enumerate(ios):
+        if k == q:
+            continue
+        if io.dw_ld == io.N:
+            written.append((io.dW, 4 * io.M * io.N))
+        if io.db:
+            written.append((io.db, 4 * io.M))
+    merged = []
+    for lo, nb in sorted(written):
+        if merged and lo <= merged[-1][1]:
+            merged[-1][1] = max(merged[-1][1], lo + nb)
+        else:
+            merged.append([lo, lo + nb])
+    for lo, nb in cover:
+        if not any(a <= lo and lo + nb <= b for a, b in merged):
+            return None
+    return q
 
 
 def linear_wgrad(gout, inp, want_bias=True, w_key=None, b_key=None, need=(True, True), outer=None):
diff --git a/ma-cjd-cooperative-jamming-decision-making-via-marl_amd/options.py b/ma-cjd-cooperative-jamming-decision-making-via-marl_amd/options.py
--- a/ma-cjd-cooperative-jamming-decision-making-via-marl_amd/options.py
+++ b/ma-cjd-cooperative-jamming-decision-making-via-marl_amd/options.py
@@ -4,7 +4,7 @@
 
 _DEFAULTS = {
     "UPDATE_STREAMS": "2", "UPDATES_PER_GRAPH": "1", "PIPELINED_GROUP": "1", "SHARED_BODY": "1",
-    "LEARNER_STATIC_OBS": "1", "ACTOR_IN_SCAN": "1", "DEVICE_SAMPLER": "1", "LN_IN_SQNORM": "1", "WGRAD_OUTER": "1",
+    "LEARNER_STATIC_OBS": "1", "ACTOR_IN_SCAN": "1", "DEVICE_SAMPLER": "1", "LN_IN_SQNORM": "1", "NORM_IN_REDUCE": "1", "WGRAD_OUTER": "1",
     "QHEAD_TAKEN": "1", "QHEAD_DOUBLE_Q": "1", "QHEAD_DOUBLE_Q_H128": "0", "PAIRED_HEADS": "1", "MIXER_TRAIN": "1", "MIXER_STATIC_STATE": "1", "GRAPHED_ALLREDUCE": "0",
     "PREFETCH_LAUNCH": "1",
     "CLOSED_LOOP_ROLLOUT": "0",
```

After: 37.81 million env-steps/s (median of 6 runs). +1.4%, better.
